# clementinboittiaux/sucre

Measured on AMD Instinct MI355X. Metric: restored Mpixels/sec/GPU at 1080p, 64 neighbour views; % HBM roofline, higher is better.
Workload: dtype f32

## Files before the change

### include/sucre_hip.h

```cpp
#ifndef SUCRE_HIP_H
#define SUCRE_HIP_H

#include <stddef.h>
#include <stdint.h>

#ifdef __cplusplus
extern "C" {
#endif

#define SUCRE_ABI_VERSION 2

#define SUCRE_OK 0
#define SUCRE_ERR_ARG (-1)
#define SUCRE_ERR_RANGE (-2)
#define SUCRE_ERR_LAUNCH (-3)

#define SUCRE_FIT_CLOSED_FORM 1u
#define SUCRE_FIT_OBS_U16MM 2u
#define SUCRE_FIT_KEEP_J 8u

#define SUCRE_OBS_F32 0
#define SUCRE_OBS_U16MM 1
#define SUCRE_OBS_F32_PLAIN 2
#define SUCRE_OBS_F32_Z26 3

#define SUCRE_EXT_POINTS 1
#define SUCRE_EXT_COLOUR 2
#define SUCRE_EXT_POINTS_COLOUR 3
#define SUCRE_FIT_EXT_COLOUR 4u
#define SUCRE_FIT_EXT_BOTH 16u

typedef struct sucre_view {
    const float *depth;
    const uint8_t *rgb;
    int32_t H, W;
    float K[9];
    float Kinv[9];
    float R[9];
    float t[3];
    float Rinv[9];
    float tinv[3];
} sucre_view_t;

enum {
    SUCRE_WS_VIEW_COUNT = 0,
    SUCRE_WS_VIEW_KEEP = 1,
    SUCRE_WS_N_OBS = 2,
    SUCRE_WS_PARAMS = 3,
    SUCRE_WS_SUMS = 4,
    SUCRE_WS_N_OBS_TOTAL = 5,
    SUCRE_WS_STORE_FORMAT = 6
};

int sucre_version(void);
const char *sucre_last_error(void);

size_t sucre_workspace_bytes(int H, int W, int n_views);
int64_t sucre_ws_offset(int H, int W, int n_views, int region);

int sucre_match_views(void *ws, int H, int W, int n_views, const sucre_view_t *target,
                      const sucre_view_t *views_dev, int k0, int k1, void *stream);

int sucre_match_map(int H, int W, int n_views, const sucre_view_t *target, const sucre_view_t *views_dev, int k,
                    int32_t *map_dev, void *stream);

int sucre_pack_view(const float *depth_dev, const uint8_t *rgb_dev, int H, int W, void *packed_dev, void *stream);
int sucre_pack_views(const float *const *depth_dev, const uint8_t *const *rgb_dev, void *const *packed_dev, int n, int H, int W,
                     void *stream);

int sucre_project_points(const sucre_view_t *view, const float *wP_dev, int64_t n, int32_t *pix_dev, void *stream);

int sucre_import_view(void *ws, int H, int W, int n_views, int k, const int16_t *u1_dev, const int16_t *v1_dev,
                      const float *z_dev, const uint8_t *rgb_dev, int64_t n, void *stream);

int sucre_finalize_matches(void *ws, int H, int W, int n_views, double min_cover, void *stream);
int sucre_finalize_matches_fmt(void *ws, int H, int W, int n_views, double min_cover, int obs_format, void *stream);

int sucre_fit_init(void *ws, int H, int W, int n_views, const uint8_t *rgb1_dev, const float *depth1_dev,
                   const float *params0, const float *J0_dev, void *stream);

int sucre_fit_run(void *ws, int H, int W, int n_views, int t0, int T, double lr, double beta1, double beta2,
                  double eps, unsigned flags, double *trace_dev, void *stream);

int sucre_fit_grad(void *ws, int H, int W, int n_views, int step, double lr, double beta1, double beta2,
                   double eps, unsigned flags, void *stream);
int sucre_fit_step(void *ws, int H, int W, int n_views, int step, double lr, double beta1, double beta2,
                   double eps, double *trace_row_dev, void *stream);
int sucre_set_n_obs_total(void *ws, int H, int W, int n_views, uint64_t n_obs_total, void *stream);

typedef struct sucre_group_image {
    void *ws;
    int32_t H, W, n_views;
    int32_t reserved;
} sucre_group_image_t;
size_t sucre_group_bytes(int n_images);
int64_t sucre_group_sums_offset(void);
int sucre_group_init(void *group_dev, int n_images, const sucre_group_image_t *images, const float *params0, void *stream);
int sucre_group_iter(void *group_dev, int n_images, int step, double lr, double beta1, double beta2, double eps, unsigned flags,
                     uint64_t n_obs_total, double *trace_dev, void *stream);
int sucre_group_finish(void *group_dev, int n_images, int step, double lr, double beta1, double beta2, double eps,
                       uint64_t n_obs_total, double *trace_dev, void *stream);

size_t sucre_batch_bytes(int n_images);
int sucre_fit_run_batch(void *batch_dev, int n_images, void *const *ws, double *const *trace_dev, int H, int W, const int *n_views,
                        int t0, int T, double lr, double beta1, double beta2, double eps, unsigned flags, void *stream);

int sucre_update_J(void *ws, int H, int W, int n_views, void *stream);
int sucre_update_J_fmt(void *ws, int H, int W, int n_views, int obs_format, void *stream);

int sucre_export_J(const void *ws, int H, int W, int n_views, float *J_dev, void *stream);

size_t sucre_select_scratch_bytes(void);
int sucre_select_ranks(const float *J_dev, int H, int W, int n_ranks, const uint64_t *ranks, float *out_dev, void *scratch_dev,
                       void *stream);

int sucre_count_valid(const float *J_dev, int H, int W, uint64_t *count_dev, void *stream);

int sucre_plot_stretch(const float *J_dev, int H, int W, const float *lo, const float *hi, uint8_t *out_dev, void *stream);

typedef struct sucre_pool_image {
    const float *J;
    int64_t n_px;
} sucre_pool_image_t;
size_t sucre_pool_select_bytes(void);
size_t sucre_pool_table_bytes(int n_images);
int sucre_pool_select_begin(void *state_dev, void *stream);
int sucre_pool_select_pass(void *state_dev, int pass, void *table_dev, int n_images, const sucre_pool_image_t *images, int n_ranks,
                           void *stream);
int sucre_pool_select_locate(void *state_dev, int pass, int n_ranks, const uint64_t *ranks, float *out_dev, void *stream);

int sucre_check_store(const void *ws, int H, int W, int n_views, uint32_t *verdict_dev, uint64_t *scratch_dev,
                      void *stream);

int sucre_export_view(const void *ws, int H, int W, int n_views, int k, float *z_dev, uint8_t *rgb_dev,
                      void *stream);

size_t sucre_light_workspace_bytes(int H, int W, int n_views);
int64_t sucre_light_params_offset(int H, int W, int n_views);
int sucre_match_views_light(void *ws, void *lws, int H, int W, int n_views, const sucre_view_t *target,
                            const sucre_view_t *views_dev, int k0, int k1, void *stream);
int sucre_match_views_fcolour(void *ws, void *lws, int H, int W, int n_views, const sucre_view_t *target,
                              const sucre_view_t *views_dev, int k0, int k1, void *stream);
size_t sucre_light_workspace_bytes_ext(int H, int W, int n_views, int ext_mode);
int sucre_match_views_light_fcolour(void *ws, void *lws, int H, int W, int n_views, const sucre_view_t *target,
                                    const sucre_view_t *views_dev, int k0, int k1, void *stream);
int sucre_finalize_matches_ext(void *ws, void *lws, int H, int W, int n_views, double min_cover, int ext_mode, void *stream);
int sucre_import_view_ext(void *ws, void *lws, int H, int W, int n_views, int k, const int16_t *u1_dev, const int16_t *v1_dev,
                          const float *z_dev, const uint8_t *rgb_dev, const float *ext_dev, int64_t n, int ext_mode, void *stream);
int sucre_export_view_ext(const void *ws, const void *lws, int H, int W, int n_views, int k, float *planes_dev, void *stream);
int sucre_export_view_ext2(const void *ws, const void *lws, int H, int W, int n_views, int k, float *planes_dev, void *stream);
int sucre_finalize_matches_light(void *ws, void *lws, int H, int W, int n_views, double min_cover, void *stream);
int sucre_fit_init_light(void *ws, void *lws, int H, int W, int n_views, const uint8_t *rgb1_dev, const float *depth1_dev,
                         const float *params0, const float *J0_dev, void *stream);
int sucre_update_J_light(void *ws, void *lws, int H, int W, int n_views, void *stream);
int sucre_update_J_ext(void *ws, void *lws, int H, int W, int n_views, unsigned flags, void *stream);
int sucre_fit_run_light(void *ws, void *lws, int H, int W, int n_views, int t0, int T, double lr, double beta1,
                        double beta2, double eps, unsigned flags , double *trace_dev,
                        void *stream);

size_t sucre_residual_scratch_bytes(int H, int W, int n_views);
int sucre_fit_residuals(const void *ws, int H, int W, int n_views, int obs_format, int32_t *count_dev, float *ssr_dev,
                        double *view_stats_dev, void *scratch_dev, void *stream);
int sucre_fit_residuals_ext(const void *ws, const void *lws, int H, int W, int n_views, unsigned flags ,
                            int32_t *count_dev, float *ssr_dev, double *view_stats_dev, void *scratch_dev, void *stream);

size_t sucre_trim_scratch_bytes(int H, int W, int n_views);
int sucre_trim_outliers(void *ws, int H, int W, int n_views, int obs_format, double k_sigma, const double *view_stats_dev,
                        int32_t *dropped_dev, int64_t *view_dropped_dev, float *thresholds_dev, void *scratch_dev, void *stream);
int sucre_trim_outliers_ext(void *ws, const void *lws, int H, int W, int n_views, unsigned flags ,
                            double k_sigma, const double *view_stats_dev, int32_t *dropped_dev, int64_t *view_dropped_dev,
                            float *thresholds_dev, void *scratch_dev, void *stream);

size_t sucre_gain_scratch_bytes(int H, int W, int n_views);
int sucre_view_gains(const void *ws, int H, int W, int n_views, int obs_format, double limit, double *gains_dev, float *inv_dev,
                     double *sums_dev, void *scratch_dev, void *stream);
int sucre_view_gains_ext(const void *ws, const void *lws, int H, int W, int n_views, unsigned flags ,
                         double limit, double *gains_dev, float *inv_dev, double *sums_dev, void *scratch_dev, void *stream);
int sucre_apply_view_gains(void *ws, int H, int W, int n_views, const float *inv_dev, int64_t *view_clipped_dev, void *scratch_dev,
                           void *stream);
int sucre_apply_view_gains_ext(void *ws, void *lws, int H, int W, int n_views, unsigned flags ,
                               const float *inv_dev, int64_t *view_clipped_dev, void *scratch_dev, void *stream);

#define SUCRE_INVERT_LIGHT 1u
#define SUCRE_INVERT_FLOAT_COLOUR 2u
typedef struct sucre_invert_image {
    const float *depth;
    const void *rgb;
    float *J;
    int32_t H, W;
    float Kinv[9];
    int32_t reserved;
} sucre_invert_image_t;
size_t sucre_invert_bytes(int n_images);
int sucre_invert_images(void *table_dev, int n_images, const sucre_invert_image_t *images, const float *params, unsigned flags,
                        void *stream);

typedef struct sucre_light_group_image {
    void *ws;
    void *lws;
    int32_t H, W, n_views;
    int32_t reserved;
} sucre_light_group_image_t;
size_t sucre_light_group_bytes(int n_images);
int64_t sucre_light_group_sums_offset(void);
// ... 12 lines not shown
```

### sucre_amd/_lib.py

```python
from __future__ import annotations

import ctypes as C
import os
from pathlib import Path

ABI_VERSION = 2
LIB_PATH = Path(os.environ.get('SUCRE_HIP_LIB', Path(__file__).resolve().parent / 'libsucre_hip.so'))

FIT_CLOSED_FORM = 1
FIT_OBS_U16MM = 2
FIT_EXT_COLOUR = 4
FIT_EXT_BOTH = 16
FIT_KEEP_J = 8
OBS_F32, OBS_U16MM, OBS_F32_PLAIN, OBS_F32_Z26 = 0, 1, 2, 3
EXT_POINTS, EXT_COLOUR, EXT_POINTS_COLOUR = 1, 2, 3
OBS_FORMATS = {'f32': OBS_F32, 'u16mm': OBS_U16MM, 'f32plain': OBS_F32_PLAIN, 'f32z26': OBS_F32_Z26}
WS_VIEW_COUNT, WS_VIEW_KEEP, WS_N_OBS, WS_PARAMS, WS_SUMS, WS_N_OBS_TOTAL, WS_STORE_FORMAT = range(7)
INVERT_LIGHT, INVERT_FLOAT_COLOUR = 1, 2
INVERT_MAX_IMAGES = 4096
POOL_MAX_IMAGES = 4096
POOL_MAX_RANKS = 8
POOL_HIST_WORDS = 3 * 8 * 256
STORE_F32, STORE_U16MM, STORE_Z24, STORE_Z26 = 0, 1, 2, 3


class SucreView(C.Structure):
    _fields_ = [('depth', C.c_void_p), ('rgb', C.c_void_p), ('H', C.c_int32), ('W', C.c_int32),
                ('K', C.c_float * 9), ('Kinv', C.c_float * 9), ('R', C.c_float * 9), ('t', C.c_float * 3),
                ('Rinv', C.c_float * 9), ('tinv', C.c_float * 3)]


assert C.sizeof(SucreView) == 192


class GroupImage(C.Structure):
    _fields_ = [('ws', C.c_void_p), ('H', C.c_int32), ('W', C.c_int32), ('n_views', C.c_int32), ('reserved', C.c_int32)]

class LightGroupImage(C.Structure):
    _fields_ = [('ws', C.c_void_p), ('lws', C.c_void_p), ('H', C.c_int32), ('W', C.c_int32), ('n_views', C.c_int32),
                ('reserved', C.c_int32)]


class InvertImage(C.Structure):
    _fields_ = [('depth', C.c_void_p), ('rgb', C.c_void_p), ('J', C.c_void_p), ('H', C.c_int32), ('W', C.c_int32),
                ('Kinv', C.c_float * 9), ('reserved', C.c_int32)]


assert C.sizeof(InvertImage) == 72


class PoolImage(C.Structure):
    _fields_ = [('J', C.c_void_p), ('n_px', C.c_int64)]


assert C.sizeof(PoolImage) == 16


_i, _vp, _d, _u64 = C.c_int, C.c_void_p, C.c_double, C.c_uint64
SIGNATURES = {
    'sucre_version': (_i, []),
    'sucre_last_error': (C.c_char_p, []),
    'sucre_workspace_bytes': (C.c_size_t, [_i, _i, _i]),
    'sucre_ws_offset': (C.c_int64, [_i, _i, _i, _i]),
    'sucre_match_views': (_i, [_vp, _i, _i, _i, C.POINTER(SucreView), _vp, _i, _i, _vp]),
    'sucre_match_map': (_i, [_i, _i, _i, C.POINTER(SucreView), _vp, _i, _vp, _vp]),
    'sucre_pack_view': (_i, [_vp, _vp, _i, _i, _vp, _vp]),
    'sucre_pack_views': (_i, [C.POINTER(_vp), C.POINTER(_vp), C.POINTER(_vp), _i, _i, _i, _vp]),
    'sucre_project_points': (_i, [C.POINTER(SucreView), _vp, C.c_int64, _vp, _vp]),
    'sucre_import_view': (_i, [_vp, _i, _i, _i, _i, _vp, _vp, _vp, _vp, C.c_int64, _vp]),
    'sucre_finalize_matches': (_i, [_vp, _i, _i, _i, _d, _vp]),
    'sucre_finalize_matches_fmt': (_i, [_vp, _i, _i, _i, _d, _i, _vp]),
    'sucre_fit_init': (_i, [_vp, _i, _i, _i, _vp, _vp, C.POINTER(C.c_float), _vp, _vp]),
    'sucre_fit_run': (_i, [_vp, _i, _i, _i, _i, _i, _d, _d, _d, _d, C.c_uint, _vp, _vp]),
    'sucre_fit_grad': (_i, [_vp, _i, _i, _i, _i, _d, _d, _d, _d, C.c_uint, _vp]),
    'sucre_fit_step': (_i, [_vp, _i, _i, _i, _i, _d, _d, _d, _d, _vp, _vp]),
    'sucre_set_n_obs_total': (_i, [_vp, _i, _i, _i, _u64, _vp]),
    'sucre_group_bytes': (C.c_size_t, [_i]),
    'sucre_group_sums_offset': (C.c_int64, []),
    'sucre_group_init': (_i, [_vp, _i, C.POINTER(GroupImage), C.POINTER(C.c_float), _vp]),
    'sucre_group_iter': (_i, [_vp, _i, _i, _d, _d, _d, _d, C.c_uint, _u64, _vp, _vp]),
    'sucre_group_finish': (_i, [_vp, _i, _i, _d, _d, _d, _d, _u64, _vp, _vp]),
    'sucre_batch_bytes': (C.c_size_t, [_i]),
    'sucre_fit_run_batch': (_i, [_vp, _i, C.POINTER(_vp), C.POINTER(_vp), _i, _i, C.POINTER(_i), _i, _i, _d, _d, _d, _d, C.c_uint, _vp]),
    'sucre_update_J': (_i, [_vp, _i, _i, _i, _vp]),
    'sucre_update_J_fmt': (_i, [_vp, _i, _i, _i, _i, _vp]),
    'sucre_export_J': (_i, [_vp, _i, _i, _i, _vp, _vp]),
    'sucre_select_scratch_bytes': (C.c_size_t, []),
    'sucre_select_ranks': (_i, [_vp, _i, _i, _i, C.POINTER(C.c_uint64), _vp, _vp, _vp]),
    'sucre_count_valid': (_i, [_vp, _i, _i, _vp, _vp]),
    'sucre_plot_stretch': (_i, [_vp, _i, _i, C.POINTER(C.c_float), C.POINTER(C.c_float), _vp, _vp]),
    'sucre_pool_select_bytes': (C.c_size_t, []),
    'sucre_pool_table_bytes': (C.c_size_t, [_i]),
    'sucre_pool_select_begin': (_i, [_vp, _vp]),
    'sucre_pool_select_pass': (_i, [_vp, _i, _vp, _i, C.POINTER(PoolImage), _i, _vp]),
    'sucre_pool_select_locate': (_i, [_vp, _i, _i, C.POINTER(C.c_uint64), _vp, _vp]),
    'sucre_check_store': (_i, [_vp, _i, _i, _i, _vp, _vp, _vp]),
    'sucre_export_view': (_i, [_vp, _i, _i, _i, _i, _vp, _vp, _vp]),
    'sucre_light_workspace_bytes': (C.c_size_t, [_i, _i, _i]),
    'sucre_light_params_offset': (C.c_int64, [_i, _i, _i]),
    'sucre_match_views_light': (_i, [_vp, _vp, _i, _i, _i, C.POINTER(SucreView), _vp, _i, _i, _vp]),
    'sucre_match_views_fcolour': (_i, [_vp, _vp, _i, _i, _i, C.POINTER(SucreView), _vp, _i, _i, _vp]),
    'sucre_light_workspace_bytes_ext': (C.c_size_t, [_i, _i, _i, _i]),
    'sucre_match_views_light_fcolour': (_i, [_vp, _vp, _i, _i, _i, C.POINTER(SucreView), _vp, _i, _i, _vp]),
    'sucre_finalize_matches_ext': (_i, [_vp, _vp, _i, _i, _i, _d, _i, _vp]),
    'sucre_import_view_ext': (_i, [_vp, _vp, _i, _i, _i, _i, _vp, _vp, _vp, _vp, _vp, C.c_int64, _i, _vp]),
    'sucre_export_view_ext': (_i, [_vp, _vp, _i, _i, _i, _i, _vp, _vp]),
    'sucre_export_view_ext2': (_i, [_vp, _vp, _i, _i, _i, _i, _vp, _vp]),
    'sucre_finalize_matches_light': (_i, [_vp, _vp, _i, _i, _i, _d, _vp]),
    'sucre_fit_init_light': (_i, [_vp, _vp, _i, _i, _i, _vp, _vp, C.POINTER(C.c_float), _vp, _vp]),
    'sucre_update_J_light': (_i, [_vp, _vp, _i, _i, _i, _vp]),
    'sucre_update_J_ext': (_i, [_vp, _vp, _i, _i, _i, C.c_uint, _vp]),
    'sucre_fit_run_light': (_i, [_vp, _vp, _i, _i, _i, _i, _i, _d, _d, _d, _d, C.c_uint, _vp, _vp]),
    'sucre_residual_scratch_bytes': (C.c_size_t, [_i, _i, _i]),
    'sucre_fit_residuals': (_i, [_vp, _i, _i, _i, _i, _vp, _vp, _vp, _vp, _vp]),
    'sucre_fit_residuals_ext': (_i, [_vp, _vp, _i, _i, _i, C.c_uint, _vp, _vp, _vp, _vp, _vp]),
    'sucre_trim_scratch_bytes': (C.c_size_t, [_i, _i, _i]),
    'sucre_trim_outliers': (_i, [_vp, _i, _i, _i, _i, _d, _vp, _vp, _vp, _vp, _vp, _vp]),
    'sucre_trim_outliers_ext': (_i, [_vp, _vp, _i, _i, _i, C.c_uint, _d, _vp, _vp, _vp, _vp, _vp, _vp]),
    'sucre_gain_scratch_bytes': (C.c_size_t, [_i, _i, _i]),
    'sucre_view_gains': (_i, [_vp, _i, _i, _i, _i, _d, _vp, _vp, _vp, _vp, _vp]),
    'sucre_view_gains_ext': (_i, [_vp, _vp, _i, _i, _i, C.c_uint, _d, _vp, _vp, _vp, _vp, _vp]),
    'sucre_apply_view_gains': (_i, [_vp, _i, _i, _i, _vp, _vp, _vp, _vp]),
    'sucre_apply_view_gains_ext': (_i, [_vp, _vp, _i, _i, _i, C.c_uint, _vp, _vp, _vp, _vp]),
    'sucre_invert_bytes': (C.c_size_t, [_i]),
    'sucre_invert_images': (_i, [_vp, _i, C.POINTER(InvertImage), C.POINTER(C.c_float), C.c_uint, _vp]),
    'sucre_light_group_bytes': (C.c_size_t, [_i]),
    'sucre_light_group_sums_offset': (C.c_int64, []),
    'sucre_light_group_init': (_i, [_vp, _i, C.POINTER(LightGroupImage), C.POINTER(C.c_float), _vp]),
    'sucre_light_group_iter': (_i, [_vp, _i, _i, _d, _d, _d, _d, C.c_uint, _u64, _vp, _vp]),
    'sucre_light_group_finish': (_i, [_vp, _i, _i, _d, _d, _d, _d, C.c_uint, _u64, _vp, _vp]),
}

_lib = None


class SucreError(RuntimeError):
    pass


def load() -> C.CDLL:
    global _lib
    if _lib is not None:
        return _lib
    if not LIB_PATH.exists():
        raise SucreError(f'{LIB_PATH} is missing: build the gfx950 HIP library first '
                         f'(make -C {LIB_PATH.parent / "csrc"}); there is no fallback path')
    import torch
    lib = C.CDLL(str(LIB_PATH))
    for name, (res, args) in SIGNATURES.items():
        fn = getattr(lib, name)
        fn.restype, fn.argtypes = res, args
    if lib.sucre_version() != ABI_VERSION:
        raise SucreError(f'libsucre_hip.so has ABI {lib.sucre_version()}, expected {ABI_VERSION}: rebuild it')
    _lib = lib
    return lib


def check(rc: int) -> None:
    if rc != 0:
        raise SucreError(f'libsucre_hip error {rc}: {load().sucre_last_error().decode()}')
```

### sucre_amd/csrc/abi.hip

```cpp
#include <cmath>
#include <cstdarg>
#include <cstdio>
#include <map>
#include <mutex>
#include <vector>

#include "invert.h"
#include "launch.h"
#include "pool.h"

namespace sucre {

static thread_local char g_err[512] = "";

static int fail(int code, const char *fmt, ...) {
    va_list ap;
    va_start(ap, fmt);
    vsnprintf(g_err, sizeof(g_err), fmt, ap);
    va_end(ap);
    return code;
}

static int check_hip(hipError_t e, const char *what) {
    if (e == hipSuccess) return SUCRE_OK;
    return fail(SUCRE_ERR_LAUNCH, "%s: %s", what, hipGetErrorString(e));
}

static bool aligned(const void *p, size_t a) { return (reinterpret_cast<uintptr_t>(p) % a) == 0; }

static int check_ws(const void *ws, int H, int W, int n_views, Layout *L) {
    if (!make_layout(H, W, n_views, L))
        return fail(SUCRE_ERR_ARG, "invalid geometry H=%d W=%d n_views=%d (need 1..32767, 1..%d views)", H, W, n_views,
                    kMaxViews);
    if (!ws) return fail(SUCRE_ERR_ARG, "workspace is NULL");
    if (!aligned(ws, 256)) return fail(SUCRE_ERR_ARG, "workspace must be 256-byte aligned");
    return SUCRE_OK;
}

AdamCoef adam_coef(int step, double lr, double beta1, double beta2, double eps) {
    AdamCoef c;
    const double bc1 = 1.0 - std::pow(beta1, (double)step);
    const double bc2 = 1.0 - std::pow(beta2, (double)step);
    c.w1 = (float)(1.0 - beta1);
    c.beta2 = (float)beta2;
    c.w2 = (float)(1.0 - beta2);
    c.step_size_neg = (float)(-(lr / bc1));
    c.bc2_sqrt = (float)std::sqrt(bc2);
    c.eps = (float)eps;
    return c;
}

static int check_adam(int step, double lr, double beta1, double beta2, double eps) {
    if (step < 1) return fail(SUCRE_ERR_RANGE, "Adam step must be >= 1 (got %d)", step);
    if (!(lr >= 0.0) || !(beta1 >= 0.0 && beta1 < 1.0) || !(beta2 >= 0.0 && beta2 < 1.0) || !(eps >= 0.0))
        return fail(SUCRE_ERR_ARG, "invalid Adam hyper-parameters lr=%g betas=(%g,%g) eps=%g", lr, beta1, beta2, eps);
    return SUCRE_OK;
}

}

using namespace sucre;

extern "C" {

int sucre_version(void) { return SUCRE_ABI_VERSION; }

const char *sucre_last_error(void) { return g_err; }

size_t sucre_workspace_bytes(int H, int W, int n_views) {
    Layout L;
    if (!make_layout(H, W, n_views, &L)) {
        fail(SUCRE_ERR_ARG, "invalid geometry H=%d W=%d n_views=%d", H, W, n_views);
        return 0;
    }
    return L.total;
}

int64_t sucre_ws_offset(int H, int W, int n_views, int region) {
    Layout L;
    if (!make_layout(H, W, n_views, &L)) return fail(SUCRE_ERR_ARG, "invalid geometry H=%d W=%d n_views=%d", H, W, n_views);
    switch (region) {
        case SUCRE_WS_VIEW_COUNT: return (int64_t)L.off_view_count;
        case SUCRE_WS_VIEW_KEEP: return (int64_t)L.off_view_keep;
        case SUCRE_WS_N_OBS: return (int64_t)L.off_n_obs;
        case SUCRE_WS_PARAMS: return (int64_t)L.off_params;
        case SUCRE_WS_SUMS: return (int64_t)L.off_sums;
        case SUCRE_WS_N_OBS_TOTAL: return (int64_t)L.off_n_obs_total;
        case SUCRE_WS_STORE_FORMAT: return (int64_t)off_store_format(L);
        default: return fail(SUCRE_ERR_RANGE, "unknown workspace region %d", region);
    }
}

int sucre_match_views(void *ws, int H, int W, int n_views, const sucre_view_t *target,
                      const sucre_view_t *views_dev, int k0, int k1, void *stream) {
    Layout L;
    if (int rc = check_ws(ws, H, W, n_views, &L)) return rc;
    if (!target || !views_dev) return fail(SUCRE_ERR_ARG, "target / views_dev is NULL");
    if (!target->depth) return fail(SUCRE_ERR_ARG, "target depth map is NULL");
    if (target->H != H || target->W != W)
        return fail(SUCRE_ERR_ARG, "target is %dx%d but the workspace is laid out for %dx%d", target->W, target->H, W, H);
    if (!aligned(views_dev, 8)) return fail(SUCRE_ERR_ARG, "views_dev must be 8-byte aligned");
    if (k0 < 0 || k1 > n_views || k0 >= k1) return fail(SUCRE_ERR_RANGE, "view range [%d,%d) outside [0,%d)", k0, k1, n_views);
    return check_hip(launch_match(L, static_cast<uint8_t *>(ws), *target, views_dev, k0, k1,
                                  static_cast<hipStream_t>(stream)), "sucre_match_views");
}

int sucre_match_map(int H, int W, int n_views, const sucre_view_t *target, const sucre_view_t *views_dev, int k,
                    int32_t *map_dev, void *stream) {
    Layout L;
    if (!make_layout(H, W, n_views, &L)) return fail(SUCRE_ERR_ARG, "invalid geometry H=%d W=%d n_views=%d", H, W, n_views);
    if (!target || !views_dev || !map_dev) return fail(SUCRE_ERR_ARG, "target / views_dev / map_dev is NULL");
    if (!target->depth) return fail(SUCRE_ERR_ARG, "target depth map is NULL");
    if (target->H != H || target->W != W) return fail(SUCRE_ERR_ARG, "target is %dx%d, expected %dx%d", target->W, target->H, W, H);
    if (k < 0 || k >= n_views) return fail(SUCRE_ERR_RANGE, "view %d outside [0,%d)", k, n_views);
    return check_hip(launch_match_map(L, *target, views_dev, k, map_dev, static_cast<hipStream_t>(stream)), "sucre_match_map");
}

int sucre_pack_view(const float *depth_dev, const uint8_t *rgb_dev, int H, int W, void *packed_dev, void *stream) {
    if (H <= 0 || W <= 0 || H > 32767 || W > 32767) return fail(SUCRE_ERR_ARG, "invalid image size %dx%d", W, H);
    if (!depth_dev || !rgb_dev || !packed_dev) return fail(SUCRE_ERR_ARG, "depth_dev / rgb_dev / packed_dev is NULL");
    if (!aligned(packed_dev, 8)) return fail(SUCRE_ERR_ARG, "packed_dev must be 8-byte aligned");
    return check_hip(launch_pack_view(depth_dev, rgb_dev, H, W, packed_dev, static_cast<hipStream_t>(stream)), "sucre_pack_view");
}

int sucre_pack_views(const float *const *depth_dev, const uint8_t *const *rgb_dev, void *const *packed_dev, int n, int H, int W,
                     void *stream) {
    if (H <= 0 || W <= 0 || H > 32767 || W > 32767) return fail(SUCRE_ERR_ARG, "invalid image size %dx%d", W, H);
    if (n < 0) return fail(SUCRE_ERR_RANGE, "negative view count %d", n);
    if (n == 0) return SUCRE_OK;
    if (!depth_dev || !rgb_dev || !packed_dev) return fail(SUCRE_ERR_ARG, "depth_dev / rgb_dev / packed_dev is NULL");
    for (int k = 0; k < n; ++k) {
        if (!depth_dev[k] || !rgb_dev[k] || !packed_dev[k]) return fail(SUCRE_ERR_ARG, "view %d: depth / rgb / packed pointer is NULL", k);
        if (!aligned(packed_dev[k], 8)) return fail(SUCRE_ERR_ARG, "view %d: packed_dev must be 8-byte aligned", k);
    }
    return check_hip(launch_pack_views(depth_dev, rgb_dev, packed_dev, n, H, W, static_cast<hipStream_t>(stream)), "sucre_pack_views");
}

int sucre_project_points(const sucre_view_t *view, const float *wP_dev, int64_t n, int32_t *pix_dev, void *stream) {
    if (!view) return fail(SUCRE_ERR_ARG, "view is NULL");
    if (view->H <= 0 || view->W <= 0 || view->H > 32767 || view->W > 32767)
        return fail(SUCRE_ERR_ARG, "invalid sensor size %dx%d", view->W, view->H);
    if (n < 0) return fail(SUCRE_ERR_RANGE, "negative point count %lld", (long long)n);
    if (n == 0) return SUCRE_OK;
    if (!wP_dev || !pix_dev) return fail(SUCRE_ERR_ARG, "wP_dev / pix_dev is NULL");
    return check_hip(launch_project_points(*view, wP_dev, (long long)n, pix_dev, static_cast<hipStream_t>(stream)),
                     "sucre_project_points");
}

int sucre_import_view(void *ws, int H, int W, int n_views, int k, const int16_t *u1_dev, const int16_t *v1_dev,
                      const float *z_dev, const uint8_t *rgb_dev, int64_t n, void *stream) {
    Layout L;
    if (int rc = check_ws(ws, H, W, n_views, &L)) return rc;
    if (k < 0 || k >= n_views) return fail(SUCRE_ERR_RANGE, "view %d outside [0,%d)", k, n_views);
    if (n < 0) return fail(SUCRE_ERR_RANGE, "negative observation count %lld", (long long)n);
    if (n > 0 && (!u1_dev || !v1_dev || !z_dev || !rgb_dev)) return fail(SUCRE_ERR_ARG, "NULL match list");
    return check_hip(launch_import_view(L, static_cast<uint8_t *>(ws), k, u1_dev, v1_dev, z_dev, rgb_dev, (long long)n,
                                        static_cast<hipStream_t>(stream)), "sucre_import_view");
}

int sucre_finalize_matches(void *ws, int H, int W, int n_views, double min_cover, void *stream) {
    Layout L;
    if (int rc = check_ws(ws, H, W, n_views, &L)) return rc;
    if (std::isnan(min_cover)) return fail(SUCRE_ERR_ARG, "min_cover is NaN");
    return check_hip(launch_finalize(L, static_cast<uint8_t *>(ws), min_cover, static_cast<hipStream_t>(stream)),
                     "sucre_finalize_matches");
}

int sucre_finalize_matches_fmt(void *ws, int H, int W, int n_views, double min_cover, int obs_format, void *stream) {
    Layout L;
    if (int rc = check_ws(ws, H, W, n_views, &L)) return rc;
    if (std::isnan(min_cover)) return fail(SUCRE_ERR_ARG, "min_cover is NaN");
    if (obs_format != SUCRE_OBS_F32 && obs_format != SUCRE_OBS_U16MM && obs_format != SUCRE_OBS_F32_PLAIN && obs_format != SUCRE_OBS_F32_Z26)
        return fail(SUCRE_ERR_ARG, "unknown observation format %d", obs_format);
    return check_hip(launch_finalize(L, static_cast<uint8_t *>(ws), min_cover, static_cast<hipStream_t>(stream),
                                     nullptr, nullptr, obs_format), "sucre_finalize_matches_fmt");
}

int sucre_fit_init(void *ws, int H, int W, int n_views, const uint8_t *rgb1_dev, const float *depth1_dev,
                   const float *params0, const float *J0_dev, void *stream) {
    Layout L;
    if (int rc = check_ws(ws, H, W, n_views, &L)) return rc;
    if (!depth1_dev || !params0) return fail(SUCRE_ERR_ARG, "depth1_dev / params0 is NULL");
    if (!rgb1_dev && !J0_dev) return fail(SUCRE_ERR_ARG, "need rgb1_dev or J0_dev");
    return check_hip(launch_fit_init(L, static_cast<uint8_t *>(ws), rgb1_dev, depth1_dev, params0, J0_dev,
                                     static_cast<hipStream_t>(stream)), "sucre_fit_init");
}

int sucre_fit_grad(void *ws, int H, int W, int n_views, int step, double lr, double beta1, double beta2,
                   double eps, unsigned flags, void *stream) {
    Layout L;
    if (int rc = check_ws(ws, H, W, n_views, &L)) return rc;
    if (int rc = check_adam(step, lr, beta1, beta2, eps)) return rc;
    if (flags & ~(SUCRE_FIT_CLOSED_FORM | SUCRE_FIT_OBS_U16MM)) return fail(SUCRE_ERR_ARG, "unknown fit flags 0x%x", flags);
    if ((flags & SUCRE_FIT_CLOSED_FORM) && step == 1)
        if (int rc = check_hip(launch_update_J(L, static_cast<uint8_t *>(ws), (flags & SUCRE_FIT_OBS_U16MM) ? SUCRE_OBS_U16MM : SUCRE_OBS_F32,
                                               static_cast<hipStream_t>(stream)), "sucre_fit_grad/update_J")) return rc;
    return check_hip(launch_fit_grad(L, static_cast<uint8_t *>(ws), adam_coef(step, lr, beta1, beta2, eps), flags,
                                     static_cast<hipStream_t>(stream)), "sucre_fit_grad");
}

int sucre_fit_step(void *ws, int H, int W, int n_views, int step, double lr, double beta1, double beta2,
                   double eps, double *trace_row_dev, void *stream) {
    Layout L;
    if (int rc = check_ws(ws, H, W, n_views, &L)) return rc;
    if (int rc = check_adam(step, lr, beta1, beta2, eps)) return rc;
    if (trace_row_dev && !aligned(trace_row_dev, 8)) return fail(SUCRE_ERR_ARG, "trace must be 8-byte aligned");
    return check_hip(launch_fit_step(L, static_cast<uint8_t *>(ws), adam_coef(step, lr, beta1, beta2, eps),
                                     trace_row_dev, static_cast<hipStream_t>(stream)), "sucre_fit_step");
}

int sucre_fit_run(void *ws, int H, int W, int n_views, int t0, int T, double lr, double beta1, double beta2,
                  double eps, unsigned flags, double *trace_dev, void *stream) {
    Layout L;
    if (int rc = check_ws(ws, H, W, n_views, &L)) return rc;
    if (t0 < 0 || T < 0) return fail(SUCRE_ERR_RANGE, "t0=%d T=%d must be >= 0", t0, T);
    if (int rc = check_adam(t0 + 1, lr, beta1, beta2, eps)) return rc;
    if (flags & ~(SUCRE_FIT_CLOSED_FORM | SUCRE_FIT_OBS_U16MM | SUCRE_FIT_KEEP_J)) return fail(SUCRE_ERR_ARG, "unknown fit flags 0x%x", flags);
    if (trace_dev && !aligned(trace_dev, 8)) return fail(SUCRE_ERR_ARG, "trace must be 8-byte aligned");
    auto *w = static_cast<uint8_t *>(ws);
    auto s = static_cast<hipStream_t>(stream);
    const int fmt = (flags & SUCRE_FIT_OBS_U16MM) ? SUCRE_OBS_U16MM : SUCRE_OBS_F32;
    if ((flags & SUCRE_FIT_CLOSED_FORM) && t0 == 0 && T > 0)
        if (int rc = check_hip(launch_update_J(L, w, fmt, s), "sucre_fit_run/initial update_J")) return rc;
    for (int it = 0; it < T; ++it) {
        const AdamCoef co = adam_coef(t0 + it + 1, lr, beta1, beta2, eps);
        if (int rc = check_hip(launch_fit_iter_fused(L, w, co, flags, trace_dev ? trace_dev + (size_t)it * 10 : nullptr, s),
                               "sucre_fit_run")) return rc;
    }
    if ((flags & SUCRE_FIT_CLOSED_FORM) && !(flags & SUCRE_FIT_KEEP_J))
        return check_hip(launch_update_J(L, w, fmt, s), "sucre_fit_run/update_J");
    return SUCRE_OK;
}

int sucre_set_n_obs_total(void *ws, int H, int W, int n_views, uint64_t n_obs_total, void *stream) {
    Layout L;
    if (int rc = check_ws(ws, H, W, n_views, &L)) return rc;
    if (n_obs_total == 0) return fail(SUCRE_ERR_RANGE, "n_obs_total must be > 0");
    return check_hip(launch_set_n_obs_total(L, static_cast<uint8_t *>(ws), n_obs_total,
                                            static_cast<hipStream_t>(stream)), "sucre_set_n_obs_total");
}

int sucre_update_J(void *ws, int H, int W, int n_views, void *stream) {
    return sucre_update_J_fmt(ws, H, W, n_views, SUCRE_OBS_F32, stream);
}

int sucre_update_J_fmt(void *ws, int H, int W, int n_views, int obs_format, void *stream) {
    Layout L;
    if (int rc = check_ws(ws, H, W, n_views, &L)) return rc;
    if (obs_format != SUCRE_OBS_F32 && obs_format != SUCRE_OBS_U16MM && obs_format != SUCRE_OBS_F32_PLAIN && obs_format != SUCRE_OBS_F32_Z26)
        return fail(SUCRE_ERR_ARG, "unknown observation format %d", obs_format);
    return check_hip(launch_update_J(L, static_cast<uint8_t *>(ws), obs_format == SUCRE_OBS_U16MM ? SUCRE_OBS_U16MM : SUCRE_OBS_F32,
                                     static_cast<hipStream_t>(stream)),
                     "sucre_update_J");
}

int sucre_export_J(const void *ws, int H, int W, int n_views, float *J_dev, void *stream) {
    Layout L;
    if (int rc = check_ws(ws, H, W, n_views, &L)) return rc;
    if (!J_dev) return fail(SUCRE_ERR_ARG, "J_dev is NULL");
    return check_hip(launch_export_J(L, static_cast<const uint8_t *>(ws), J_dev, static_cast<hipStream_t>(stream)),
                     "sucre_export_J");
}

int sucre_export_view(const void *ws, int H, int W, int n_views, int k, float *z_dev, uint8_t *rgb_dev,
                      void *stream) {
    Layout L;
    if (int rc = check_ws(ws, H, W, n_views, &L)) return rc;
    if (k < 0 || k >= n_views) return fail(SUCRE_ERR_RANGE, "view %d outside [0,%d)", k, n_views);
    if (!z_dev && !rgb_dev) return fail(SUCRE_ERR_ARG, "both outputs are NULL");
    return check_hip(launch_export_view(L, static_cast<const uint8_t *>(ws), k, z_dev, rgb_dev,
                                        static_cast<hipStream_t>(stream)), "sucre_export_view");
}

int sucre_check_store(const void *ws, int H, int W, int n_views, uint32_t *verdict_dev, uint64_t *scratch_dev,
                      void *stream) {
    Layout L;
    if (int rc = check_ws(ws, H, W, n_views, &L)) return rc;
    if (!verdict_dev || !scratch_dev) return fail(SUCRE_ERR_ARG, "verdict_dev / scratch_dev is NULL");
    if (!aligned(verdict_dev, 4) || !aligned(scratch_dev, 8)) return fail(SUCRE_ERR_ARG, "outputs must be 4 / 8-byte aligned");
    return check_hip(launch_check_store(L, static_cast<const uint8_t *>(ws), verdict_dev, scratch_dev,
                                        static_cast<hipStream_t>(stream)), "sucre_check_store");
}


size_t sucre_group_bytes(int n_images) { return n_images > 0 ? group_bytes(n_images) : 0; }

int64_t sucre_group_sums_offset(void) { return group_sums_offset(); }

int sucre_group_init(void *group_dev, int n_images, const sucre_group_image_t *images, const float *params0, void *stream) {
    if (!group_dev || !aligned(group_dev, 256)) return fail(SUCRE_ERR_ARG, "group buffer is NULL or not 256-byte aligned");
    if (n_images < 1 || !images || !params0) return fail(SUCRE_ERR_ARG, "need at least one image and params0");
    auto s = static_cast<hipStream_t>(stream);
    if (int rc = check_hip(launch_group_init(group_dev, params0, s), "sucre_group_init")) return rc;
    for (int i = 0; i < n_images; ++i) {
        Layout L;
        if (int rc = check_ws(images[i].ws, images[i].H, images[i].W, images[i].n_views, &L)) return rc;
        if (int rc = check_hip(launch_group_set_image(group_dev, i, L, static_cast<uint8_t *>(images[i].ws), s), "sucre_group_init")) return rc;
    }
    return SUCRE_OK;
}

int sucre_group_iter(void *group_dev, int n_images, int step, double lr, double beta1, double beta2, double eps, unsigned flags,
                     uint64_t n_obs_total, double *trace_dev, void *stream) {
    if (!group_dev || n_images < 1) return fail(SUCRE_ERR_ARG, "group buffer is NULL / no image");
    if (int rc = check_adam(step, lr, beta1, beta2, eps)) return rc;
    if (flags & ~(SUCRE_FIT_CLOSED_FORM | SUCRE_FIT_OBS_U16MM)) return fail(SUCRE_ERR_ARG, "unknown fit flags 0x%x", flags);
    if (n_obs_total == 0) return fail(SUCRE_ERR_RANGE, "n_obs_total must be > 0");
    if (trace_dev && !aligned(trace_dev, 8)) return fail(SUCRE_ERR_ARG, "trace must be 8-byte aligned");
    const AdamCoef co_prev = adam_coef(step > 1 ? step - 1 : 1, lr, beta1, beta2, eps);
    double *row = (trace_dev && step > 1) ? trace_dev + (size_t)(step - 2) * 10 : nullptr;
    return check_hip(launch_group_iter(group_dev, n_images, step, co_prev, adam_coef(step, lr, beta1, beta2, eps), flags, n_obs_total,
                                       row, static_cast<hipStream_t>(stream)), "sucre_group_iter");
}

int sucre_group_finish(void *group_dev, int n_images, int step, double lr, double beta1, double beta2, double eps,
                       uint64_t n_obs_total, double *trace_dev, void *stream) {
    if (!group_dev || n_images < 1) return fail(SUCRE_ERR_ARG, "group buffer is NULL / no image");
    if (step < 0) return fail(SUCRE_ERR_RANGE, "step=%d must be >= 0", step);
    if (step >= 1) if (int rc = check_adam(step, lr, beta1, beta2, eps)) return rc;
    if (n_obs_total == 0) return fail(SUCRE_ERR_RANGE, "n_obs_total must be > 0");
    double *row = (trace_dev && step >= 1) ? trace_dev + (size_t)(step - 1) * 10 : nullptr;
    return check_hip(launch_group_finish(group_dev, n_images, step, adam_coef(step >= 1 ? step : 1, lr, beta1, beta2, eps), n_obs_total,
                                         row, static_cast<hipStream_t>(stream)), "sucre_group_finish");
}


size_t sucre_batch_bytes(int n_images) { return n_images > 0 ? batch_bytes(n_images) : 0; }

int sucre_fit_run_batch(void *batch_dev, int n_images, void *const *ws, double *const *trace_dev, int H, int W, const int *n_views,
                        int t0, int T, double lr, double beta1, double beta2, double eps, unsigned flags, void *stream) {
    if (!batch_dev || !aligned(batch_dev, 256)) return fail(SUCRE_ERR_ARG, "batch buffer is NULL or not 256-byte aligned");
    if (n_images < 1 || !ws || !n_views) return fail(SUCRE_ERR_ARG, "need at least one image (ws and n_views arrays)");
    if (n_images > 4096) return fail(SUCRE_ERR_RANGE, "n_images=%d: at most 4096 images per batch", n_images);
    std::vector<Layout> layouts((size_t)n_images);
    for (int i = 0; i < n_images; ++i) {
        if (int rc = check_ws(ws[i], H, W, n_views[i], &layouts[(size_t)i])) return rc;
        for (int j = 0; j < i; ++j)
            if (ws[j] == ws[i]) return fail(SUCRE_ERR_ARG, "images %d and %d share a workspace", j, i);
        if (trace_dev && trace_dev[i] && !aligned(trace_dev[i], 8)) return fail(SUCRE_ERR_ARG, "trace of image %d must be 8-byte aligned", i);
    }
    if (t0 < 0 || T < 0) return fail(SUCRE_ERR_RANGE, "t0=%d T=%d must be >= 0", t0, T);
    if (int rc = check_adam(t0 + 1, lr, beta1, beta2, eps)) return rc;
    if (flags & ~(SUCRE_FIT_CLOSED_FORM | SUCRE_FIT_OBS_U16MM | SUCRE_FIT_KEEP_J)) return fail(SUCRE_ERR_ARG, "unknown fit flags 0x%x", flags);
    auto s = static_cast<hipStream_t>(stream);
    const int fmt = (flags & SUCRE_FIT_OBS_U16MM) ? SUCRE_OBS_U16MM : SUCRE_OBS_F32;
    if (int rc = check_hip(launch_batch_set(batch_dev, n_images, reinterpret_cast<uint8_t *const *>(ws), trace_dev, layouts.data(), flags, s),
                           "sucre_fit_run_batch/table")) return rc;
    if ((flags & SUCRE_FIT_CLOSED_FORM) && t0 == 0 && T > 0)
        for (int i = 0; i < n_images; ++i)
            if (int rc = check_hip(launch_update_J(layouts[(size_t)i], static_cast<uint8_t *>(ws[i]), fmt, s), "sucre_fit_run_batch/initial update_J")) return rc;
    for (int it = 0; it < T; ++it)
        if (int rc = check_hip(launch_batch_iter(layouts[0], batch_dev, n_images, adam_coef(t0 + it + 1, lr, beta1, beta2, eps), flags, it, s),
                               "sucre_fit_run_batch")) return rc;
    if ((flags & SUCRE_FIT_CLOSED_FORM) && !(flags & SUCRE_FIT_KEEP_J))
        for (int i = 0; i < n_images; ++i)
            if (int rc = check_hip(launch_update_J(layouts[(size_t)i], static_cast<uint8_t *>(ws[i]), fmt, s), "sucre_fit_run_batch/update_J")) return rc;
    return SUCRE_OK;
}

size_t sucre_select_scratch_bytes(void) { return select_scratch_bytes(); }

int sucre_select_ranks(const float *J_dev, int H, int W, int n_ranks, const uint64_t *ranks, float *out_dev, void *scratch_dev,
                       void *stream) {
    if (H <= 0 || W <= 0) return fail(SUCRE_ERR_ARG, "invalid image size %dx%d", W, H);
    if (!J_dev || !ranks || !out_dev || !scratch_dev) return fail(SUCRE_ERR_ARG, "J_dev / ranks / out_dev / scratch_dev is NULL");
    if (n_ranks < 1 || n_ranks > 8) return fail(SUCRE_ERR_RANGE, "n_ranks=%d outside [1,8]", n_ranks);
    if (!aligned(scratch_dev, 8) || !aligned(J_dev, 4) || !aligned(out_dev, 4)) return fail(SUCRE_ERR_ARG, "misaligned pointer");
    return check_hip(launch_select_ranks(J_dev, H, W, n_ranks, ranks, out_dev, scratch_dev, static_cast<hipStream_t>(stream)),
                     "sucre_select_ranks");
}

int sucre_count_valid(const float *J_dev, int H, int W, uint64_t *count_dev, void *stream) {
    if (H <= 0 || W <= 0) return fail(SUCRE_ERR_ARG, "invalid image size %dx%d", W, H);
    if (!J_dev || !count_dev) return fail(SUCRE_ERR_ARG, "J_dev / count_dev is NULL");
    if (!aligned(J_dev, 4) || !aligned(count_dev, 8)) return fail(SUCRE_ERR_ARG, "misaligned pointer");
    return check_hip(launch_count_valid(J_dev, H, W, count_dev, static_cast<hipStream_t>(stream)), "sucre_count_valid");
}
// ... 550 lines not shown
```

### sucre_amd/csrc/experiment.h

```cpp
#pragma once

#ifdef SUCRE_EXP_NOCOMPUTE
constexpr bool kExpNoCompute = true;
#else
constexpr bool kExpNoCompute = false;
#endif
#ifdef SUCRE_EXP_NOLOAD
constexpr bool kExpNoLoad = true;
#else
constexpr bool kExpNoLoad = false;
#endif
#ifdef SUCRE_EXP_NOSTORE
constexpr bool kExpNoStore = true;
#else
constexpr bool kExpNoStore = false;
#endif
#ifndef SUCRE_STORE_NT
#define SUCRE_STORE_NT 2
#endif
constexpr int kStoreNt = SUCRE_STORE_NT;

#ifndef SUCRE_FIT_WAVES
#define SUCRE_FIT_WAVES 5
#endif
#ifndef SUCRE_CLOSED_WAVES
#define SUCRE_CLOSED_WAVES 4
#endif

#ifndef SUCRE_MIN_STRIPS
#define SUCRE_MIN_STRIPS 4
#endif

#ifndef SUCRE_RING
#define SUCRE_RING 3
#endif
#ifndef SUCRE_DMA_POLICY
#define SUCRE_DMA_POLICY " nt"
#endif

#ifndef SUCRE_EXACT_DIV
#define SUCRE_EXACT_DIV 0
#endif
constexpr bool kExactDiv = SUCRE_EXACT_DIV != 0;

#ifndef SUCRE_EXACT_J_ADAM
#define SUCRE_EXACT_J_ADAM 0
#endif
constexpr bool kExactJAdam = SUCRE_EXACT_J_ADAM != 0;

#if !defined(SUCRE_SCALED_B)
#define SUCRE_SCALED_B 1
#endif
constexpr bool kScaledBBuilt = SUCRE_SCALED_B != 0;

#ifdef SUCRE_EXP_WAVE_TIMES
constexpr bool kExpWaveTimes = true;
#define SUCRE_EXP_EXPORT extern "C" __attribute__((visibility("default")))
#else
constexpr bool kExpWaveTimes = false;
#define SUCRE_EXP_EXPORT [[maybe_unused]] static
#endif

#ifndef SUCRE_DEAL_FIT
#define SUCRE_DEAL_FIT 64, 50, 38, 28, 20
#endif
#ifndef SUCRE_DEAL_CLOSED
#define SUCRE_DEAL_CLOSED 64, 48, 32, 20
#endif
```

### sucre_amd/csrc/fit.hip

```cpp
#include <cstddef>
#include <type_traits>

#include "experiment.h"
#include "fit_math.h"
#include "handoff.h"

namespace sucre {

struct Water {
    float B[3], nb[3], ng[3];
};

template <class ParamAt>
__device__ __forceinline__ Water water_from(ParamAt param_at) {
    Water w;
#pragma unroll
    for (int c = 0; c < 3; ++c) {
        w.B[c] = param_at(c);
        w.nb[c] = -param_at(3 + c) * kLog2e;
        w.ng[c] = -param_at(6 + c) * kLog2e;
    }
    return w;
}
__device__ __forceinline__ Water load_water(const float *__restrict__ params) {
// ... 5 lines not shown
    Water w = load_water(params);
#pragma unroll
    for (int c = 0; c < 3; ++c) { w.B[c] = uniform_f(w.B[c]); w.nb[c] = uniform_f(w.nb[c]); w.ng[c] = uniform_f(w.ng[c]); }
    return w;
}

constexpr float kInv255 = (float)(1.0 / 255.0);

struct Acc {
    float pa[3];
    float pb[3];
    float sB[3];
    float sGZ[3];
    float cost;
};

__device__ __forceinline__ void pack_sums(float (&s)[kNumSums], const float (&sB)[3], const float (&sGZ)[3], const float (&sBeta)[3], float cost) {
#pragma unroll
    for (int c = 0; c < 3; ++c) { s[c] = sB[c]; s[3 + c] = sGZ[c]; s[6 + c] = sBeta[c]; }
    s[9] = cost;
}

struct Exps { float a[kGroupLv][3], g[kGroupLv][3]; };

__device__ __forceinline__ void chunk_exps(const float (&zz)[kGroupLv], const Water &w, Exps &e) {
#pragma unroll
    for (int j = 0; j < kGroupLv; ++j)
#pragma unroll
        for (int c = 0; c < 3; ++c) { e.a[j][c] = zz[j] * w.nb[c]; e.g[j][c] = zz[j] * w.ng[c]; }
    __builtin_amdgcn_sched_barrier(0);
#pragma unroll
    for (int j = 0; j < kGroupLv; ++j)
#pragma unroll
        for (int c = 0; c < 3; ++c) { e.a[j][c] = fast_exp2(e.a[j][c]); e.g[j][c] = fast_exp2(e.g[j][c]); }
    __builtin_amdgcn_sched_barrier(0);
}

template <bool kScaledB>
__device__ __forceinline__ void grad_terms(float z, float a, float g, uint32_t k, bool valid, float Bc, float Jc, int c, Acc &acc) {
    const float omg = kScaledB ? __builtin_fmaf(-Bc, g, Bc) : 1.0f - g;
    const float Ihat = __builtin_fmaf(Jc, a, kScaledB ? omg : Bc * omg);
    float r = __builtin_fmaf((float)k, kInv255, -Ihat);
    r = valid ? r : 0.0f;
    const float rz = r * z;
    acc.cost = __builtin_fmaf(r, r, acc.cost);
    acc.pa[c] = __builtin_fmaf(r, a, acc.pa[c]);
    acc.pb[c] = __builtin_fmaf(rz, a, acc.pb[c]);
    acc.sB[c] = __builtin_fmaf(r, omg, acc.sB[c]);
    acc.sGZ[c] = __builtin_fmaf(rz, g, acc.sGZ[c]);
}

template <bool kMasked, bool kScaledB>
__device__ __forceinline__ void accumulate_chunk(const float (&zz)[kGroupLv], const uint32_t (&cc)[3], const Water &w,
                                                 const float (&J)[3], Acc &acc) {
    if (kExpNoCompute) {
        acc.cost += (zz[0] + zz[1]) + (zz[2] + zz[3]) + (float)(cc[0] ^ cc[1] ^ cc[2]);
        return;
    }
    Exps e;
    chunk_exps(zz, w, e);
#pragma unroll
    for (int j = 0; j < kGroupLv; ++j) {
        const float z = zz[j];
        const bool valid = !kMasked || z > 0.0f;
#pragma unroll
        for (int c = 0; c < 3; ++c) grad_terms<kScaledB>(z, e.a[j][c], e.g[j][c], (cc[c] >> (8 * j)) & 255u, valid, w.B[c], J[c], c, acc);
    }
}

template <bool kScaledB>
__device__ __forceinline__ void accumulate_level(float z, const uint32_t (&k)[3], const Water &w, const float (&J)[3],
                                                 Acc &acc) {
    const bool valid = z > 0.0f;
#pragma unroll
    for (int c = 0; c < 3; ++c) grad_terms<kScaledB>(z, fast_exp2(z * w.nb[c]), fast_exp2(z * w.ng[c]), k[c], valid, w.B[c], J[c], c, acc);
}

__device__ __forceinline__ float finite_or_zero(float x) { return __builtin_isfinite(x) ? x : 0.0f; }

struct AccOne {
    float q[9][3];
};

template <bool kScaledB>
__device__ __forceinline__ void closed_terms(float z, float a, float g, uint32_t k, bool valid, float Bc, float Jp,
                                             float &q0, float &q1, float &q2, float &q3, float &q4, float &q5,
                                             float &q6, float &q7, float &q8) {
    const float omg = kScaledB ? __builtin_fmaf(-Bc, g, Bc) : 1.0f - g;
    const float y = __builtin_fmaf((float)k, kInv255, -(kScaledB ? omg : Bc * omg));
    float p = __builtin_fmaf(-Jp, a, y);
    p = valid ? p : 0.0f;
    const float za = z * a, zg = z * g;
    q0 = __builtin_fmaf(p, a, q0);
    q1 = __builtin_fmaf(a, valid ? a : 0.0f, q1);
    q2 = __builtin_fmaf(p, omg, q2);
    q3 = __builtin_fmaf(a, omg, q3);
    q4 = __builtin_fmaf(p, za, q4);
    q5 = __builtin_fmaf(a, za, q5);
    q6 = __builtin_fmaf(p, zg, q6);
    q7 = __builtin_fmaf(a, zg, q7);
    q8 = __builtin_fmaf(p, p, q8);
}

template <bool kMasked, bool kScaledB>
__device__ __forceinline__ void accumulate_chunk(const float (&zz)[kGroupLv], const uint32_t (&cc)[3], const Water &w,
                                                 const float (&Jp)[3], AccOne &acc) {
    if (kExpNoCompute) {
        acc.q[8][0] += (zz[0] + zz[1]) + (zz[2] + zz[3]) + (float)(cc[0] ^ cc[1] ^ cc[2]);
        return;
    }
    Exps e;
    chunk_exps(zz, w, e);
#pragma unroll
    for (int j = 0; j < kGroupLv; ++j) {
        const float z = zz[j];
        const bool valid = !kMasked || z > 0.0f;
#pragma unroll
        for (int c = 0; c < 3; ++c)
            closed_terms<kScaledB>(z, e.a[j][c], e.g[j][c], (cc[c] >> (8 * j)) & 255u, valid, w.B[c], Jp[c], acc.q[0][c], acc.q[1][c],
                                   acc.q[2][c], acc.q[3][c], acc.q[4][c], acc.q[5][c], acc.q[6][c], acc.q[7][c], acc.q[8][c]);
    }
}

template <bool kScaledB>
__device__ __forceinline__ void accumulate_level(float z, const uint32_t (&k)[3], const Water &w, const float (&Jp)[3],
                                                 AccOne &acc) {
    if (kExpNoCompute) {
        acc.q[8][0] += z + (float)(k[0] ^ k[1] ^ k[2]);
        return;
    }
    const bool valid = z > 0.0f;
#pragma unroll
    for (int c = 0; c < 3; ++c)
        closed_terms<kScaledB>(z, fast_exp2(z * w.nb[c]), fast_exp2(z * w.ng[c]), k[c], valid, w.B[c], Jp[c], acc.q[0][c], acc.q[1][c],
                               acc.q[2][c], acc.q[3][c], acc.q[4][c], acc.q[5][c], acc.q[6][c], acc.q[7][c], acc.q[8][c]);
}

constexpr int kRing = SUCRE_RING;
constexpr int kAhead = kRing - 1;
constexpr int kSlot = 2048;

struct __attribute__((aligned(16))) FitLds {
    uint8_t ring[4][kRing][kSlot];
    double stot[kSumsPad];
    float wsum[4][kNumSums];
    double wtotal[4][kNumSums];
    int is_last, is_last_total;
};

__device__ __forceinline__ uint32_t lds_addr(const void *p) {
    return static_cast<uint32_t>(reinterpret_cast<uintptr_t>(p));
}

constexpr uint32_t kShapeFull = 1u << 31;
constexpr uint32_t kShapeTrail = 1u << 30;
__host__ __device__ constexpr uint32_t full_chunk_b(int fmt) { return (uint32_t)(chunk_bytes(fmt) - 1024) / 16u; }
__host__ __device__ __forceinline__ uint32_t item_shape(uint32_t bytes, bool full_chunk) {
    const uint32_t pieces = bytes / 16u;
    const uint32_t nA = pieces < 64u ? pieces : 64u, nB = pieces - nA;
    return (nA - 1u) | ((nB ? nB - 1u : 0u) << 8) | ((nB ? nA : nA - 1u) << 16) | (full_chunk ? kShapeFull : 0u);
}
static_assert(level_bytes(0) % 16 == 0 && level_bytes(1) % 16 == 0 && level_bytes(2) % 16 == 0 && level_bytes(3) % 16 == 0 && kChunk % 16 == 0 && kChunk16 % 16 == 0 && kChunk24 % 16 == 0 && kChunk26 % 16 == 0, "items are copied in 16-byte pieces");
static_assert(kChunk <= 2048 && kChunk >= 1024 && kChunk16 >= 1024 && kChunk24 >= 1024 && kChunk26 >= 1024 && kChunk26 <= kChunk, "a full chunk is one whole DMA + a partial one");
static_assert(level_bytes(0) % 64 == 0 && level_bytes(1) % 64 == 0 && level_bytes(2) % 64 == 0 && (kGroupLv * level_bytes(3)) % 64 == 0, "items start on 64-byte units (PlanItem.src64; a kStoreZ26 strip starts on a whole chunk)");

__device__ __forceinline__ void dma_item(const uint8_t *src, uint32_t slotA, uint32_t slotB, uint32_t voffA, uint32_t voffB) {
    if (kExpNoLoad) return;
    unsigned keep;
    asm volatile(
        "s_nop 4\n\t"
        "s_mov_b32 %0, m0\n\t"
        "s_mov_b32 m0, %3\n\t"
        "s_nop 0\n\t"
        "global_load_lds_dwordx4 %1, %2" SUCRE_DMA_POLICY "\n\t"
        "s_mov_b32 m0, %4\n\t"
        "s_nop 0\n\t"
        "global_load_lds_dwordx4 %5, %2" SUCRE_DMA_POLICY "\n\t"
        "s_mov_b32 m0, %0"
        : "=&s"(keep)
        : "v"(voffA), "s"(src), "s"(slotA), "s"(slotB), "v"(voffB)
        : "memory");
}

__device__ __forceinline__ void wait_vm(uint32_t n) {
#define SUCRE_W(N) case N: asm volatile("s_waitcnt vmcnt(" #N ")" ::: "memory"); break;
    switch (n) {
        SUCRE_W(0) SUCRE_W(1) SUCRE_W(2) SUCRE_W(3) SUCRE_W(4) SUCRE_W(5) SUCRE_W(6) SUCRE_W(7) SUCRE_W(8) SUCRE_W(9)
        SUCRE_W(10) SUCRE_W(11) SUCRE_W(12) SUCRE_W(13) SUCRE_W(14) SUCRE_W(15) SUCRE_W(16) SUCRE_W(17) SUCRE_W(18)
        SUCRE_W(19) SUCRE_W(20) SUCRE_W(21)
        default: asm volatile("s_waitcnt vmcnt(0)" ::: "memory"); break;
    }
#undef SUCRE_W
}
static_assert(2 * kAhead + 9 <= 63, "s_waitcnt vmcnt takes six bits");

__device__ __forceinline__ uint32_t strip_items(uint32_t levels, int mode) { return 1u + ((levels + 3u) >> 2) + (mode == 0 ? 1u : 0u); }

__global__ __launch_bounds__(256) void plan_kernel(const StripMeta *__restrict__ meta, int n_strips, const uint32_t *__restrict__ store_fmt, uint32_t W0, uint32_t W1,
                                                   uint32_t Kmax, uint32_t stride0, uint32_t stride1, uint32_t kmax0, uint32_t kmax1,
                                                   PlanItem *__restrict__ plan0, PlanItem *__restrict__ plan1,
                                                   StripEntry *__restrict__ strips0, StripEntry *__restrict__ strips1,
                                                   uint32_t *__restrict__ count0, uint32_t *__restrict__ count1, uint64_t comp_off,
                                                   uint64_t state_off) {
    const int mode = blockIdx.y;
    const int fmt = (int)store_fmt[0];
    const uint32_t W = mode ? W1 : W0, stride = mode ? stride1 : stride0, kmax = mode ? kmax1 : kmax0;
    PlanItem *plan = mode ? plan1 : plan0;
    StripEntry *strips = mode ? strips1 : strips0;
    uint32_t *count = mode ? count1 : count0;
    const uint32_t idx = blockIdx.x * 256u + threadIdx.x;
    const uint32_t wid = idx / Kmax, k = idx - wid * Kmax;
    if (wid >= W) return;
    const DealShares sh = deal_shares(mode, W / 4u);
    uint32_t start = 0u, strip = 0u, strip0 = 0u;
    const uint32_t K = deal_walk(wid, W, (uint32_t)n_strips, sh, [&](uint32_t s) { return meta[s].levels; }, [&](uint32_t kk, uint32_t s) {
        if (kk == 0u) strip0 = s;
        if (kk < k) start += strip_items(meta[s].levels, mode);
        if (kk == k) strip = s;
    });
    if (k == 0u) count[wid] = K;
    if (k >= K) return;
    const StripMeta m = meta[strip];
    const uint32_t nfull = m.levels >> 2, r = m.levels & 3u;
    const uint32_t nu = min(nfull, m.full >> 2);
    const uint32_t lb = (uint32_t)level_bytes(fmt);
    const uint64_t st = state_off + (uint64_t)strip * (kStateFloats * 4);
    PlanItem *out = plan + (size_t)wid * stride + start;
    strips[(size_t)wid * kmax + k] = StripEntry{strip, strip_counts(nu, nfull - nu, r)};
    *out++ = PlanItem{(uint32_t)(st >> 6), item_shape(3u * kStripPx * 4u, false)};
    for (uint32_t g = 0; g < nfull; ++g)
        *out++ = PlanItem{(uint32_t)((comp_off + (m.lvoff + (uint64_t)g * kGroupLv) * lb) >> 6), item_shape((uint32_t)chunk_bytes(fmt), true)};
    if (r) *out++ = PlanItem{(uint32_t)((comp_off + (m.lvoff + (uint64_t)nfull * kGroupLv) * lb) >> 6), item_shape(r * lb, false)};
    if (mode == 0) *out++ = PlanItem{(uint32_t)((st + 3 * kStripPx * 4) >> 6), item_shape(6u * kStripPx * 4u, false)};
    if (k + 1u == K) {
        const uint64_t st0 = state_off + (uint64_t)strip0 * (kStateFloats * 4);
        for (int j = 0; j < kAhead + 1; ++j) *out++ = PlanItem{(uint32_t)(st0 >> 6), item_shape(3u * kStripPx * 4u, false) | kShapeTrail};
    }
}

typedef uint32_t ItemRegs __attribute__((ext_vector_type(2)));
typedef const __attribute__((address_space(4))) ItemRegs *ConstItems;

template <class T>
__device__ __forceinline__ T *uniform_ptr(T *p) {
    const uint64_t u = reinterpret_cast<uint64_t>(p);
    const uint32_t lo = __builtin_amdgcn_readfirstlane((uint32_t)u), hi = __builtin_amdgcn_readfirstlane((uint32_t)(u >> 32));
    return reinterpret_cast<T *>(((uint64_t)hi << 32) | lo);
}

template <class T>
__device__ __forceinline__ ConstItems const_items(const T *p) {
    static_assert(sizeof(T) == 8, "two dwords per entry");
    return (ConstItems)(reinterpret_cast<uintptr_t>(uniform_ptr(p)));
}

struct RangeCodes { bool z24, z26; uint32_t zoff, fullB; };

template <int kFmt>
__device__ __forceinline__ RangeCodes range_codes_of(uint32_t f0, uint32_t f1) {
    RangeCodes rc;
    rc.z24 = kFmt == 0 && f0 == (uint32_t)kStoreZ24;
    rc.z26 = kFmt == 0 && f0 == (uint32_t)kStoreZ26;
    rc.zoff = f1;
    rc.fullB = rc.z24 ? full_chunk_b(kStoreZ24) : rc.z26 ? full_chunk_b(kStoreZ26) : full_chunk_b(kFmt);
    return rc;
}

template <int kFmt>
__device__ __forceinline__ RangeCodes range_codes(const uint32_t *__restrict__ store_fmt) {
    return range_codes_of<kFmt>(__builtin_amdgcn_readfirstlane(store_fmt[0]), __builtin_amdgcn_readfirstlane(store_fmt[1]));
}

__host__ __device__ constexpr bool format_readable(int kFmt, uint32_t f) {
    return kFmt == kStoreU16 ? f == (uint32_t)kStoreU16 : (f == (uint32_t)kStoreF32 || f == (uint32_t)kStoreZ24 || f == (uint32_t)kStoreZ26);
}
template <int kFmt>
__device__ __forceinline__ bool store_matches(const uint32_t *__restrict__ store_fmt) {
    return format_readable(kFmt, __builtin_amdgcn_readfirstlane(store_fmt[0]));
}

template <int kFmt>
__device__ __forceinline__ void read_chunk(const uint8_t *sp, int lane, float (&zz)[kGroupLv], uint32_t (&cc)[3], const RangeCodes &rc, bool masked) {
    auto read_codes = [&](auto z26) {
        constexpr bool kZ26 = decltype(z26)::value;
        const uint2 a = *reinterpret_cast<const uint2 *>(sp + lane * 24), b = *reinterpret_cast<const uint2 *>(sp + lane * 24 + 8),
                    c = *reinterpret_cast<const uint2 *>(sp + lane * 24 + 16);
        const uint32_t h = kZ26 ? sp[kChunk24 + lane] : 0u;
        const uint32_t w[4] = {a.x, a.y, b.x, b.y};
#pragma unroll
        for (int j = 0; j < kGroupLv; ++j) {
            uint32_t bits;
            asm("v_mad_u32_u24 %0, %1, 1, %2" : "=v"(bits) : "v"(w[j]), "s"(rc.zoff));
            if (kZ26) bits += ((h >> (2 * j)) & 3u) << 24;
            zz[j] = __uint_as_float(bits);
            if (masked) zz[j] = (kZ26 ? bits != rc.zoff : (w[j] & 0xffffffu) != 0u) ? zz[j] : 0.0f;
        }
        cc[0] = __builtin_amdgcn_perm(a.y, a.x, 0x0c0c0703u) | __builtin_amdgcn_perm(b.y, b.x, 0x07030c0cu);
        cc[1] = c.x; cc[2] = c.y;
    };
    if (kFmt == 0 && rc.z26) return read_codes(std::true_type{});
    if (kFmt == 0 && rc.z24) return read_codes(std::false_type{});
    if (kFmt == 0) {
        const float4 z4 = *reinterpret_cast<const float4 *>(sp + lane * 16);
        zz[0] = z4.x; zz[1] = z4.y; zz[2] = z4.z; zz[3] = z4.w;
    } else {
        const uint2 q = *reinterpret_cast<const uint2 *>(sp + lane * 8);
        zz[0] = (float)(q.x & 0xffffu) * kMPerMm; zz[1] = (float)(q.x >> 16) * kMPerMm;
        zz[2] = (float)(q.y & 0xffffu) * kMPerMm; zz[3] = (float)(q.y >> 16) * kMPerMm;
    }
    const uint32_t *cp = reinterpret_cast<const uint32_t *>(sp + (kFmt ? 2 : 4) * kStripPx * kGroupLv) + 3 * lane;
    cc[0] = cp[0]; cc[1] = cp[1]; cc[2] = cp[2];
}

template <int kFmt>
__device__ __forceinline__ void read_level(const uint8_t *sp, int lane, uint32_t r, uint32_t j, float &z, uint32_t (&k)[3], const RangeCodes &rc) {
    const bool z24 = kFmt == 0 && (rc.z24 || rc.z26);
    if (z24) {
        const uint8_t *zp = sp + (lane * r + j) * 3u;
        uint32_t code = (uint32_t)zp[0] | ((uint32_t)zp[1] << 8) | ((uint32_t)zp[2] << 16);
        if (rc.z26) {
            const uint32_t f = (uint32_t)lane * r + j;
            code |= ((reinterpret_cast<const uint32_t *>(sp + 6u * kStripPx * r)[f >> 4] >> (2u * (f & 15u))) & 3u) << 24;
        }
        z = code ? __uint_as_float(code + rc.zoff) : 0.0f;
    } else if (kFmt == 0) z = reinterpret_cast<const float *>(sp)[lane * r + j];
    else z = (float)reinterpret_cast<const uint16_t *>(sp)[lane * r + j] * kMPerMm;
    const uint8_t *cb = sp + (z24 ? 3 : kFmt ? 2 : 4) * kStripPx * r;
#pragma unroll
    for (int c = 0; c < 3; ++c) k[c] = cb[c * kStripPx * r + lane * r + j];
}

template <int kFmt>
__device__ __forceinline__ void issue_item(const ItemRegs it, uint32_t ring0, uint32_t slot_off, const uint8_t *__restrict__ ws, int lane, uint32_t fullB) {
    const uint32_t lane16 = (uint32_t)lane * 16u;
    const uint32_t voffB_full = (64u + min((uint32_t)lane, fullB - 1u)) * 16u;
    const uint8_t *src = ws + ((uint64_t)it.x << 6);
    const uint32_t slot = ring0 + slot_off;
    if (it.y & kShapeFull) {
        dma_item(src, slot, slot + 1024u, lane16, voffB_full);
    } else {
        const uint32_t a_last = it.y & 127u, b_last = (it.y >> 8) & 127u, b_base = (it.y >> 16) & 127u;
        dma_item(src, slot, slot + ((a_last + 1u) << 4), min((uint32_t)lane, a_last) << 4, (b_base + min((uint32_t)lane, b_last)) << 4);
    }
}

struct NoChain { static constexpr bool kOn = false; };
struct StreamChain {
    static constexpr bool kOn = true;
    ItemRegs head[kAhead + 1], se0;
    bool next_on;
    ItemRegs next_head[kAhead];
    const uint8_t *next_ws;
    uint32_t next_fullB;
    uint32_t cs, behind;
};

template <int kFmt, int kStores, bool kMoments, bool kPrimed = false, class Chain = NoChain, class OnJ, class OnChunk, class OnTail, class OnEnd>
__device__ __forceinline__ void stream_strips(FitLds &lds, const PlanItem *__restrict__ plan, const StripEntry *__restrict__ strip_list,
                                              uint32_t K, const uint8_t *__restrict__ ws, int wave, int lane, uint32_t fullB, OnJ on_J,
                                              OnChunk on_chunk, OnTail on_tail, OnEnd on_end, Chain *chain = nullptr) {
    if (K == 0) return;
    constexpr bool kChain = Chain::kOn;
    static_assert(!kChain || kPrimed, "a chained stream's first items are in flight when it starts");
    const uint32_t ring0 = lds_addr(&lds.ring[wave][0][0]);
    const uint8_t *ringp = &lds.ring[wave][0][0];
    const ConstItems items = const_items(plan);
    const ConstItems strips = const_items(strip_list);
    uint32_t trail = 0u;
    auto issue = [&](const ItemRegs it, uint32_t slot_off) {
        if constexpr (kChain) {
            if (chain->next_on && (it.y & kShapeTrail)) {
                ItemRegs f = chain->next_head[0];
#pragma unroll
                for (int q = 1; q < kAhead; ++q) f = trail == (uint32_t)q ? chain->next_head[q] : f;
                ++trail;
                issue_item<kFmt>(f, ring0, slot_off, chain->next_ws, lane, chain->next_fullB);
                return;
            }
        }
        issue_item<kFmt>(it, ring0, slot_off, ws, lane, fullB);
    };
    if (!kPrimed) {
#pragma unroll
        for (int q = 0; q < kAhead; ++q) issue(items[q], (uint32_t)(q * kSlot));
    }
    ItemRegs nxt;
    if constexpr (kChain) nxt = chain->head[kAhead]; else nxt = items[kAhead];
    uint32_t i = 0;
    uint32_t cs = 0u;
    uint32_t behind = 0u;
    if constexpr (kChain) { cs = chain->cs; behind = chain->behind; }
    auto step = [&]() -> const uint8_t * {
        asm volatile("s_waitcnt lgkmcnt(0)" ::: "memory");
        const uint32_t is = cs == 0u ? (uint32_t)((kRing - 1) * kSlot) : cs - (uint32_t)kSlot;
        issue(nxt, is);
        nxt = items[i + (uint32_t)kAhead + 1u];
        if (behind) {
            asm volatile("s_waitcnt vmcnt(%0)" ::"n"(2 * kAhead + kStores) : "memory");
            --behind;
        } else {
            asm volatile("s_waitcnt vmcnt(%0)" ::"n"(2 * kAhead) : "memory");
        }
        const uint8_t *sp = ringp + cs;
        cs = cs == (uint32_t)((kRing - 1) * kSlot) ? 0u : cs + (uint32_t)kSlot;
        ++i;
        return sp;
    };
    ItemRegs se;
    if constexpr (kChain) se = chain->se0; else se = strips[0];
    for (uint32_t k = 0; k < K; ++k) {
        const uint32_t strip = se.x, counts = se.y;
        if (k + 1u < K) se = strips[k + 1u];
        const uint32_t nu = counts_unmasked(counts), nm = counts_masked(counts), r = counts_tail(counts);
        on_J(step());
        for (uint32_t g = 0; g < nu; ++g) on_chunk(step(), false);
        for (uint32_t g = 0; g < nm; ++g) on_chunk(step(), true);
        if (r) on_tail(step(), r);
        if (kMoments) on_end(strip, step());
        else on_end(strip, (const uint8_t *)nullptr);
        behind = (uint32_t)kAhead;
    }
    if constexpr (kChain) {
        if (chain->next_on) {
            chain->cs = cs;
            chain->behind = (uint32_t)kAhead;
            return;
        }
        chain->cs = 0u;
        chain->behind = 0u;
    }
    asm volatile("s_waitcnt vmcnt(0)" ::: "memory");
}

__device__ __forceinline__ double wave_sum_fixed(double x) {
    return wave_sum_lane0(x);
}

__device__ __forceinline__ void reduce_group(const float *partials, int n_blocks, int g, double *gpart, int n_groups) {
    const int lane = threadIdx.x & 63, wave = threadIdx.x >> 6;
    const int b = g * kGroup + lane;
    for (int q = wave; q < kNumSums; q += 4) {
        double x = 0.0;
        if (lane < kGroup && b < n_blocks)
            x = (double)__hip_atomic_load(partials + (size_t)q * n_blocks + b, __ATOMIC_RELAXED, __HIP_MEMORY_SCOPE_AGENT);
        x = wave_sum_fixed(x);
        if (lane == 0) __hip_atomic_store(gpart + (size_t)q * n_groups + g, x, __ATOMIC_RELAXED, __HIP_MEMORY_SCOPE_AGENT);
    }
}

__device__ __forceinline__ double unscale_sum(double x, int q, bool scaled, float Bq) {
    return (kScaledBBuilt && scaled && q < 3) ? x / (double)Bq : x;
}

__device__ __forceinline__ void reduce_total(const double *gpart, int n_groups, double *stot, double *__restrict__ sums, const float *Bpass) {
    const int lane = threadIdx.x & 63, wave = threadIdx.x >> 6;
    const bool scaled = scaled_b_ok(Bpass[0], Bpass[1], Bpass[2]);
    for (int q = wave; q < kNumSums; q += 4) {
        double x = 0.0;
        for (int g = lane; g < n_groups; g += 64)
            x += __hip_atomic_load(gpart + (size_t)q * n_groups + g, __ATOMIC_RELAXED, __HIP_MEMORY_SCOPE_AGENT);
        x = unscale_sum(wave_sum_fixed(x), q, scaled, Bpass[q < 3 ? q : 0]);
        if (lane == 0) {
            __hip_atomic_store(sums + q, x, __ATOMIC_RELAXED, __HIP_MEMORY_SCOPE_AGENT);
            stot[q] = x;
        }
    }
    __syncthreads();
}

__device__ __forceinline__ void water_step(const double *__restrict__ sums, float *__restrict__ pstate,
                                           const uint64_t *__restrict__ n_obs_total, const AdamCoef &co,
                                           double *__restrict__ trace_row) {
    const int q = threadIdx.x & 63;
    const float scale = (1.0f / 3.0f) / (float)(*n_obs_total);
    float p = 0.f, m = 0.f, v = 0.f;
    double g = 0.0;
    if (q < 9) {
        g = water_grad(q, scale, [&](int i) { return sums[i]; }, [&](int c) { return pstate[c]; });
        p = pstate[q];
        m = pstate[9 + q];
        v = pstate[18 + q];
    }
    __builtin_amdgcn_wave_barrier();
    if (q < 9) {
        adam_update(p, m, v, (float)g, co);
        pstate[q] = p;
        pstate[9 + q] = m;
        pstate[18 + q] = v;
    }
    if (trace_row) {
        if (q < 9) trace_row[1 + q] = (double)p;
        if (q == 9) trace_row[0] = sums[9];
    }
}

__device__ __forceinline__ void wave_sums(float (&s)[kNumSums]) {
    static_assert(kNumSums == 10, "five pairs");
    float h[5];
#pragma unroll
    for (int q = 0; q < 5; ++q) {
        const auto r = __builtin_amdgcn_permlane32_swap(__float_as_uint(s[q]), __float_as_uint(s[q + 5]), false, false);
        h[q] = __uint_as_float(r[0]) + __uint_as_float(r[1]);
    }
    float R[3];
#pragma unroll
    for (int p = 0; p < 3; ++p) {
        const float a = h[2 * p], b = h[p < 2 ? 2 * p + 1 : 4];
        const auto r = __builtin_amdgcn_permlane16_swap(__float_as_uint(a), __float_as_uint(b), false, false);
        R[p] = __uint_as_float(r[0]) + __uint_as_float(r[1]);
        R[p] += lane_down<8>(R[p]);
        R[p] += lane_down<4>(R[p]);
        R[p] += lane_down<2>(R[p]);
        R[p] += lane_down<1>(R[p]);
    }
    auto at = [](float v, int lane) { return __uint_as_float(__builtin_amdgcn_readlane(__float_as_uint(v), lane)); };
    s[0] = at(R[0], 0); s[1] = at(R[0], 16); s[5] = at(R[0], 32); s[6] = at(R[0], 48);
    s[2] = at(R[1], 0); s[3] = at(R[1], 16); s[7] = at(R[1], 32); s[8] = at(R[1], 48);
    s[4] = at(R[2], 0); s[9] = at(R[2], 32);
}

template <bool kFused, bool kStep>
__device__ __forceinline__ void finish_from_wave_sums(FitLds &lds, float *partials, const AdamCoef &co, unsigned *ticket,
                                                      double *gpart, int n_groups, double *sums, float *pstate,
                                                      const uint64_t *__restrict__ n_obs_total, double *trace_row, const float *Bpass) {
    const int n_blocks = gridDim.x;
    const int t = threadIdx.x;
    __syncthreads();
    if (t < kNumSums)
        __hip_atomic_store(partials + (size_t)t * n_blocks + blockIdx.x,
                           ((lds.wsum[0][t] + lds.wsum[1][t]) + lds.wsum[2][t]) + lds.wsum[3][t], __ATOMIC_RELAXED,
                           __HIP_MEMORY_SCOPE_AGENT);

    if (kFused) {
        const int g = blockIdx.x / kGroup;
        const unsigned gsize = (unsigned)(min((g + 1) * kGroup, n_blocks) - g * kGroup);
        if (arrive_last(ticket + (size_t)(1 + g) * kTicketStride, gsize, &lds.is_last)) {
            reduce_group(partials, n_blocks, g, gpart, n_groups);
            if (arrive_last(ticket, (unsigned)n_groups, &lds.is_last_total)) {
                reduce_total(gpart, n_groups, lds.stot, sums, Bpass);
                if (kStep && t < 64) water_step(lds.stot, pstate, n_obs_total, co, trace_row);
            }
        }
    }
}

template <bool kFused, bool kStep = kFused>
__device__ __forceinline__ void finish_launch(FitLds &lds, float (&s)[kNumSums], float *partials, const AdamCoef &co,
                                              unsigned *ticket, double *gpart, int n_groups, double *sums,
                                              float *pstate, const uint64_t *__restrict__ n_obs_total,
                                              double *trace_row) {
    const int t = threadIdx.x;
    const int lane = t & 63;
    const int wave = __builtin_amdgcn_readfirstlane(t >> 6);
    wave_sums(s);
    if (lane == 0) {
#pragma unroll
        for (int q = 0; q < kNumSums; ++q) lds.wsum[wave][q] = s[q];
    }
    finish_from_wave_sums<kFused, kStep>(lds, partials, co, ticket, gpart, n_groups, sums, pstate, n_obs_total, trace_row, pstate);
}

template <class Chain>
__device__ __forceinline__ void store_stepped(float *p, float v) {
    if (kStoreNt == 1 || (kStoreNt == 2 && Chain::kOn)) __builtin_nontemporal_store(v, p);
    else *p = v;
}

template <int kFmt, bool kScaledB, bool kPrimed = false, class Chain = NoChain>
__device__ __forceinline__ void grad_pass(FitLds &lds, const PlanItem *__restrict__ plan, const StripEntry *__restrict__ strips, uint32_t n_strips_wave,
                                          const uint8_t *__restrict__ ws, float *__restrict__ state, int wave, int lane,
                                          const Water &w, float gscale, const AdamCoef &co, Acc &acc, float (&sBeta)[3], const RangeCodes &rc,
                                          Chain *chain = nullptr) {
    float J[3] = {0.f, 0.f, 0.f};
    stream_strips<kFmt, 9, true, kPrimed, Chain>(
        lds, plan, strips, n_strips_wave, ws, wave, lane, rc.fullB,
        [&](const uint8_t *sp) {
            const float *f = reinterpret_cast<const float *>(sp);
#pragma unroll
            for (int c = 0; c < 3; ++c) { J[c] = f[c * kStripPx + lane]; acc.pa[c] = 0.f; acc.pb[c] = 0.f; }
        },
        [&](const uint8_t *sp, bool masked) {
            float zz[kGroupLv];
            uint32_t cc[3];
            read_chunk<kFmt>(sp, lane, zz, cc, rc, masked);
            if (masked) accumulate_chunk<true, kScaledB>(zz, cc, w, J, acc);
            else accumulate_chunk<false, kScaledB>(zz, cc, w, J, acc);
        },
        [&](const uint8_t *sp, uint32_t r) {
            for (uint32_t j = 0; j < r; ++j) {
                float z;
                uint32_t k[3];
                read_level<kFmt>(sp, lane, r, j, z, k, rc);
                accumulate_level<kScaledB>(z, k, w, J, acc);
            }
        },
        [&](uint32_t strip, const uint8_t *sp) {
            const float *f = reinterpret_cast<const float *>(sp);
            float *st = state + (size_t)strip * kStateFloats;
#pragma unroll
            for (int c = 0; c < 3; ++c) {
                float Jc = J[c], m = f[c * kStripPx + lane], v = f[(3 + c) * kStripPx + lane];
                sBeta[c] += (acc.pb[c] == 0.0f) ? 0.0f : Jc * acc.pb[c];
                adam_update_J(Jc, m, v, gscale * acc.pa[c], co);
                if (kExpNoStore) {
                    asm volatile("" ::"v"(Jc), "v"(m), "v"(v));
                    continue;
                }
                store_stepped<Chain>(&st[c * kStripPx + lane], Jc);
                store_stepped<Chain>(&st[(3 + c) * kStripPx + lane], m);
                store_stepped<Chain>(&st[(6 + c) * kStripPx + lane], v);
            }
        },
        chain);
}

__device__ __forceinline__ bool pass_scaled_b(const Water &w) {
    return kScaledBBuilt && __builtin_amdgcn_readfirstlane((int)scaled_b_ok(w.B[0], w.B[1], w.B[2])) != 0;
}

template <int kFmt, bool kPrimed = false, class Chain = NoChain>
__device__ __forceinline__ void run_grad_pass(bool scaled, FitLds &lds, const PlanItem *__restrict__ plan, const StripEntry *__restrict__ strips,
                                              uint32_t n_strips_wave, const uint8_t *__restrict__ ws, float *__restrict__ state, int wave, int lane,
                                              const Water &w, float gscale, const AdamCoef &co, Acc &acc, float (&sBeta)[3], const RangeCodes &rc,
                                              Chain *chain = nullptr) {
    if (kScaledBBuilt && scaled) grad_pass<kFmt, true, kPrimed, Chain>(lds, plan, strips, n_strips_wave, ws, state, wave, lane, w, gscale, co, acc, sBeta, rc, chain);
    else grad_pass<kFmt, false, kPrimed, Chain>(lds, plan, strips, n_strips_wave, ws, state, wave, lane, w, gscale, co, acc, sBeta, rc, chain);
}

__device__ __forceinline__ void zero_acc(Acc &acc) {
#pragma unroll
    for (int c = 0; c < 3; ++c) { acc.pa[c] = 0.f; acc.pb[c] = 0.f; acc.sB[c] = 0.f; acc.sGZ[c] = 0.f; }
    acc.cost = 0.f;
}

constexpr uint32_t kExpWaveSlots = 8192;
__device__ unsigned long long g_exp_wave_times[5][kExpWaveTimes ? kExpWaveSlots : 1];
}
SUCRE_EXP_EXPORT int sucre_exp_wave_times(unsigned long long *out) {
    return (int)hipMemcpyFromSymbol(out, HIP_SYMBOL(sucre::g_exp_wave_times), sizeof(sucre::g_exp_wave_times));
}
namespace sucre {

template <bool kFused, int kFmt>
__global__ __launch_bounds__(256, kFitWaves) void fit_grad_kernel(const uint8_t *__restrict__ ws,
                                                       const PlanItem *__restrict__ plan, const StripEntry *__restrict__ plan_strips, const uint32_t *__restrict__ plan_count,
                                                       uint32_t plan_stride, uint32_t plan_kmax,
                                                       float *pstate, const uint64_t *__restrict__ n_obs_total,
                                                       float *__restrict__ state, float *partials, const AdamCoef co,
                                                       unsigned *ticket, double *gpart, int n_groups, double *sums,
                                                       double *trace_row, const uint32_t *__restrict__ obs_format) {
    __shared__ FitLds lds;
    const unsigned long long exp_t_in = kExpWaveTimes ? wall_clock64() : 0ull, exp_c_in = kExpWaveTimes ? clock64() : 0ull;
    const int t = threadIdx.x;
    const int lane = t & 63;
    const int wave = __builtin_amdgcn_readfirstlane(t >> 6);
    const Water w = load_water(pstate);
    const float gscale = -2.0f * ((1.0f / 3.0f) / (float)(*n_obs_total));
    const RangeCodes rc = range_codes<kFmt>(obs_format);
    const bool fmt_ok = store_matches<kFmt>(obs_format);
    const uint32_t wid = blockIdx.x * 4u + (uint32_t)wave;
    const uint32_t n_mine = fmt_ok ? plan_count[wid] : 0u;

    Acc acc;
    zero_acc(acc);
    if (!fmt_ok) acc.cost = __builtin_nanf("");
    float sBeta[3] = {0.f, 0.f, 0.f};
    if (kExpWaveTimes && lane == 0 && wid < kExpWaveSlots) g_exp_wave_times[0][wid] = wall_clock64();
    run_grad_pass<kFmt>(pass_scaled_b(w), lds, plan + (size_t)wid * plan_stride, plan_strips + (size_t)wid * plan_kmax, n_mine, ws, state, wave, lane, w, gscale, co, acc, sBeta, rc);
    if (kExpWaveTimes && lane == 0 && wid < kExpWaveSlots) g_exp_wave_times[1][wid] = wall_clock64();

    float s[kNumSums];
    pack_sums(s, acc.sB, acc.sGZ, sBeta, acc.cost);
    finish_launch<kFused>(lds, s, partials, co, ticket, gpart, n_groups, sums, pstate, n_obs_total, trace_row);
    if (kExpWaveTimes && lane == 0 && wid < kExpWaveSlots) { g_exp_wave_times[2][wid] = exp_t_in; g_exp_wave_times[3][wid] = wall_clock64(); g_exp_wave_times[4][wid] = clock64() - exp_c_in; }
}

struct ClosedSums { float sB[3], sGZ[3], sBeta[3], cost; };

template <int kFmt, bool kJOnly, bool kScaledB, bool kPrimed = false, class Chain = NoChain>
__device__ __forceinline__ void closed_pass(FitLds &lds, const PlanItem *__restrict__ plan, const StripEntry *__restrict__ strips, uint32_t n_strips_wave,
                                            const uint8_t *__restrict__ ws, float *__restrict__ state, int wave, int lane,
                                            const Water &w, bool fmt_ok, ClosedSums &cs, const RangeCodes &rc, Chain *chain = nullptr) {
    AccOne acc;
    float Jp[3] = {0.f, 0.f, 0.f};
    stream_strips<kFmt, 3, false, kPrimed, Chain>(
        lds, plan, strips, n_strips_wave, ws, wave, lane, rc.fullB,
        [&](const uint8_t *sp) {
            const float *f = reinterpret_cast<const float *>(sp);
#pragma unroll
            for (int c = 0; c < 3; ++c) {
                Jp[c] = kJOnly ? 0.0f : finite_or_zero(f[c * kStripPx + lane]);
            }
#pragma unroll
            for (int q = 0; q < 9; ++q)
#pragma unroll
                for (int c = 0; c < 3; ++c) acc.q[q][c] = 0.f;
        },
        [&](const uint8_t *sp, bool masked) {
            float zz[kGroupLv];
            uint32_t cc[3];
            read_chunk<kFmt>(sp, lane, zz, cc, rc, masked);
            if (masked) accumulate_chunk<true, kScaledB>(zz, cc, w, Jp, acc);
            else accumulate_chunk<false, kScaledB>(zz, cc, w, Jp, acc);
        },
        [&](const uint8_t *sp, uint32_t r) {
            for (uint32_t j = 0; j < r; ++j) {
                float z;
                uint32_t k[3];
                read_level<kFmt>(sp, lane, r, j, z, k, rc);
                accumulate_level<kScaledB>(z, k, w, Jp, acc);
            }
        },
        [&](uint32_t strip, const uint8_t *) {
            float *st = state + (size_t)strip * kStateFloats;
#pragma unroll
            for (int c = 0; c < 3; ++c) {
                const float N = acc.q[0][c], D = acc.q[1][c];
                const float dJ = N / D;
                const float Jc = fmt_ok ? Jp[c] + dJ : __builtin_nanf("");
                store_stepped<Chain>(&st[c * kStripPx + lane], Jc);
                if (!kJOnly && D != 0.0f) {
                    cs.sB[c] += __builtin_fmaf(-dJ, acc.q[3][c], acc.q[2][c]);
                    cs.sBeta[c] += Jc * __builtin_fmaf(-dJ, acc.q[5][c], acc.q[4][c]);
                    cs.sGZ[c] += __builtin_fmaf(-dJ, acc.q[7][c], acc.q[6][c]);
                    cs.cost += __builtin_fmaf(-dJ, N, acc.q[8][c]);
                } else if (!kJOnly && N != 0.0f) {
                    cs.sB[c] += kScaledB ? dJ * w.B[c] : dJ;
                    cs.sBeta[c] += dJ;
                    cs.sGZ[c] += dJ;
                    cs.cost += __builtin_inff();
                }
            }
        },
        chain);
}

template <int kFmt, bool kPrimed = false, class Chain = NoChain>
__device__ __forceinline__ void run_closed_pass(bool scaled, FitLds &lds, const PlanItem *__restrict__ plan, const StripEntry *__restrict__ strips,
                                                uint32_t n_strips_wave, const uint8_t *__restrict__ ws, float *__restrict__ state, int wave, int lane,
                                                const Water &w, bool fmt_ok, ClosedSums &cs, const RangeCodes &rc, Chain *chain = nullptr) {
    if (kScaledBBuilt && scaled) closed_pass<kFmt, false, true, kPrimed, Chain>(lds, plan, strips, n_strips_wave, ws, state, wave, lane, w, fmt_ok, cs, rc, chain);
    else closed_pass<kFmt, false, false, kPrimed, Chain>(lds, plan, strips, n_strips_wave, ws, state, wave, lane, w, fmt_ok, cs, rc, chain);
}

template <bool kFused, int kFmt, bool kJOnly>
__global__ __launch_bounds__(256, kClosedWaves) void fit_closed_kernel(const uint8_t *__restrict__ ws,
                                                         const PlanItem *__restrict__ plan, const StripEntry *__restrict__ plan_strips, const uint32_t *__restrict__ plan_count,
                                                       uint32_t plan_stride, uint32_t plan_kmax,
                                                         float *pstate, const uint64_t *__restrict__ n_obs_total,
                                                         float *__restrict__ state, float *partials, const AdamCoef co,
                                                         unsigned *ticket, double *gpart, int n_groups, double *sums,
                                                         double *trace_row, const uint32_t *__restrict__ obs_format) {
    __shared__ FitLds lds;
    const int t = threadIdx.x;
    const int lane = t & 63;
    const int wave = __builtin_amdgcn_readfirstlane(t >> 6);
    const Water w = load_water_uniform(pstate);
    const RangeCodes rc = range_codes<kFmt>(obs_format);
    const bool fmt_ok = store_matches<kFmt>(obs_format);
    const uint32_t wid = blockIdx.x * 4u + (uint32_t)wave;
    const uint32_t n_mine = (fmt_ok || kJOnly) ? plan_count[wid] : 0u;
    ClosedSums cs = {{0.f, 0.f, 0.f}, {0.f, 0.f, 0.f}, {0.f, 0.f, 0.f}, fmt_ok ? 0.f : __builtin_nanf("")};
    if (kExpWaveTimes && !kJOnly && lane == 0 && wid < kExpWaveSlots) g_exp_wave_times[0][wid] = wall_clock64();
    if (kJOnly) closed_pass<kFmt, true, false>(lds, plan + (size_t)wid * plan_stride, plan_strips + (size_t)wid * plan_kmax, n_mine, ws, state, wave, lane, w, fmt_ok, cs, rc);
    else run_closed_pass<kFmt>(pass_scaled_b(w), lds, plan + (size_t)wid * plan_stride, plan_strips + (size_t)wid * plan_kmax, n_mine, ws, state, wave, lane, w, fmt_ok, cs, rc);
    if (kExpWaveTimes && !kJOnly && lane == 0 && wid < kExpWaveSlots) g_exp_wave_times[1][wid] = wall_clock64();
    if (kJOnly) return;
    float s[kNumSums];
    pack_sums(s, cs.sB, cs.sGZ, cs.sBeta, cs.cost);
    finish_launch<kFused>(lds, s, partials, co, ticket, gpart, n_groups, sums, pstate, n_obs_total, trace_row);
}

struct Params9 { float v[9]; };
static Params9 params9(const float *p) {
    Params9 q;
    for (int i = 0; i < 9; ++i) q.v[i] = p[i];
    return q;
}

constexpr int kGroupFitWaves = kFitWaves > 5 ? 5 : kFitWaves;

struct GroupImage {
    uint8_t *ws;
    uint64_t off_plan[2], off_strips[2], off_count[2], off_state, off_format, off_params;
    uint32_t stride[2], kmax[2], n_waves[2];
};

struct GroupHeader {
    float pstate[2][32];
    double sums[kSumsPad];
    unsigned ticket[(1 + (kFitGrid + kGroup - 1) / kGroup) * kTicketStride];
    double gpart[kNumSums * ((kFitGrid + kGroup - 1) / kGroup)];
    float partials[kNumSums * kFitGrid];
};

__host__ __device__ __forceinline__ GroupImage *group_images(GroupHeader *g) {
    return reinterpret_cast<GroupImage *>(reinterpret_cast<uint8_t *>(g) + align_up(sizeof(GroupHeader), 256));
}

__device__ __forceinline__ float ld_agent(const float *p) { return __hip_atomic_load(p, __ATOMIC_RELAXED, __HIP_MEMORY_SCOPE_AGENT); }
__device__ __forceinline__ double ld_agent(const double *p) { return __hip_atomic_load(p, __ATOMIC_RELAXED, __HIP_MEMORY_SCOPE_AGENT); }
__device__ __forceinline__ void st_agent(float *p, float v) { __hip_atomic_store(p, v, __ATOMIC_RELAXED, __HIP_MEMORY_SCOPE_AGENT); }

__device__ __forceinline__ void group_water_step(const double *__restrict__ sums, const float *__restrict__ in,
                                                 uint64_t n_obs_total, const AdamCoef &co, bool apply, float &p, float &m, float &v) {
    const int q = threadIdx.x & 63;
    p = m = v = 0.f;
    if (q < 9) {
        p = ld_agent(in + q); m = ld_agent(in + 9 + q); v = ld_agent(in + 18 + q);
        if (apply) {
            const float scale = (1.0f / 3.0f) / (float)n_obs_total;
            const double g = water_grad(q, scale, [&](int i) { return ld_agent(sums + i); }, [&](int c) { return ld_agent(in + c); });
            adam_update(p, m, v, (float)g, co);
        }
    }
}

template <int kMode, int kFmt>
__global__ __launch_bounds__(256, kMode ? kClosedWaves : kGroupFitWaves) void group_iter_kernel(GroupHeader *g, int n_images, uint64_t n_obs_total,
                                                                                           const AdamCoef co_prev, const AdamCoef co, int apply,
                                                                                           int in, int out, double *trace_prev, int n_groups,
// ... 219 lines not shown
            if (!v.fmt_ok) acc.cost = __builtin_nanf("");
            float sBeta[3] = {0.f, 0.f, 0.f};
            run_grad_pass<kFmt, true, StreamChain>(pass_scaled_b(v.w), lds, v.plan, v.strips, v.n_mine, v.ws, v.state, wave, lane, v.w, v.gscale, co, acc, sBeta, v.rc, &ch);
            const float q[kNumSums] = {acc.sB[0], acc.sB[1], acc.sB[2], acc.sGZ[0], acc.sGZ[1], acc.sGZ[2], sBeta[0], sBeta[1], sBeta[2], acc.cost};
#pragma unroll
            for (int j = 0; j < kNumSums; ++j) s[j] = q[j];
        } else {
            ClosedSums cs = {{0.f, 0.f, 0.f}, {0.f, 0.f, 0.f}, {0.f, 0.f, 0.f}, v.fmt_ok ? 0.f : __builtin_nanf("")};
            run_closed_pass<kFmt, true, StreamChain>(pass_scaled_b(v.w), lds, v.plan, v.strips, v.n_mine, v.ws, v.state, wave, lane, v.w, v.fmt_ok, cs, v.rc, &ch);
            const float q[kNumSums] = {cs.sB[0], cs.sB[1], cs.sB[2], cs.sGZ[0], cs.sGZ[1], cs.sGZ[2], cs.sBeta[0], cs.sBeta[1], cs.sBeta[2], cs.cost};
#pragma unroll
            for (int j = 0; j < kNumSums; ++j) s[j] = q[j];
        }
        if (more && !chained) {
            asm volatile("s_waitcnt lgkmcnt(0)" ::: "memory");
            prime(vn);
        }
        wave_sums(s);
        if (lane == 0) {
#pragma unroll
            for (int j = 0; j < kNumSums; ++j) blds.wsum[slot][wave][j] = s[j];
        }
        v = vn;
    }
    __syncthreads();
    for (int idx = t; idx < slot * kNumSums; idx += 256) {
        const int sl = idx / kNumSums, j = idx - sl * kNumSums;
        const uint32_t q = blockIdx.x + (uint32_t)sl * P, i = q / vblocks, vb = q - i * vblocks;
        float *partials = reinterpret_cast<float *>(images[i].ws + images[i].o.partials);
        __hip_atomic_store(partials + (size_t)j * vblocks + vb,
                           ((blds.wsum[sl][0][j] + blds.wsum[sl][1][j]) + blds.wsum[sl][2][j]) + blds.wsum[sl][3][j], __ATOMIC_RELAXED, __HIP_MEMORY_SCOPE_AGENT);
    }
}

constexpr int kTailThreads = 16 * kBatchMax;
__global__ __launch_bounds__(kTailThreads) void batch_tail_kernel(const BatchEntry *__restrict__ images, int n_images, int n_blocks, const AdamCoef co, int row) {
    __shared__ double stot[kBatchMax][kNumSums];
    __shared__ int is_last;
    const int t = threadIdx.x, g = blockIdx.x, n_groups = gridDim.x;
    const int i = t >> 4, q = t & 15;
    const bool mine = i < n_images && q < kNumSums;
    uint8_t *ws = mine ? images[i].ws : nullptr;
    if (mine)
        reduce_group_thread(reinterpret_cast<const float *>(ws + images[i].o.partials), n_blocks, g, q, reinterpret_cast<double *>(ws + images[i].o.gpart), n_groups);
    float p = 0.f, m = 0.f, v = 0.f, Bc = 0.f, scale = 0.f;
    float *pstate = nullptr;
    bool scaled = false;
    if (mine && q < 9) {
        pstate = reinterpret_cast<float *>(ws + images[i].o.params);
        scale = (1.0f / 3.0f) / (float)(*reinterpret_cast<const uint64_t *>(ws + images[i].o.n_obs_total));
        p = pstate[q]; m = pstate[9 + q]; v = pstate[18 + q];
        Bc = pstate[q % 3];
        scaled = scaled_b_ok(pstate[0], pstate[1], pstate[2]);
    }
    unsigned *ticket = reinterpret_cast<unsigned *>(images[0].ws + images[0].o.ticket);
    if (!arrive_last(ticket, (unsigned)n_groups, &is_last)) return;
    if (mine) {
        const double y = unscale_sum(reduce_total_thread(reinterpret_cast<const double *>(ws + images[i].o.gpart), n_groups, q), q, scaled, Bc);
        __hip_atomic_store(reinterpret_cast<double *>(ws + images[i].o.sums) + q, y, __ATOMIC_RELAXED, __HIP_MEMORY_SCOPE_AGENT);
        stot[i][q] = y;
    }
    __syncthreads();
    if (!mine) return;
    double *trace = images[i].trace;
    if (q < 9) {
        const double grad = water_grad(q, scale, [&](int j) { return stot[i][j]; }, [&](int) { return Bc; });
        adam_update(p, m, v, (float)grad, co);
        pstate[q] = p; pstate[9 + q] = m; pstate[18 + q] = v;
        if (trace) trace[(size_t)row * 10 + 1 + q] = (double)p;
    } else if (trace) {
        trace[(size_t)row * 10] = stot[i][9];
    }
}

constexpr uint32_t batch_full_grid(int mode) { return (uint32_t)(mode ? kClosedGrid : 256 * kGroupFitWaves); }
constexpr int batch_images(uint32_t vblocks, uint32_t full) { return vblocks <= full ? kBatchMax : (int)((uint64_t)kBatchMax * full / vblocks); }
static_assert(batch_images(kClosedGrid, batch_full_grid(1)) == kBatchMax && batch_images(kFitGrid, batch_full_grid(0)) >= 1, "a launch takes at least one image");
static_assert(SUCRE_FIT_WAVES > 5 || batch_images(kFitGrid, batch_full_grid(0)) == kBatchMax, "the product's launches take kBatchMax images");

constexpr int kBatchSet = 8;
struct BatchEntries { BatchEntry e[kBatchSet]; };
__global__ void batch_set_kernel(BatchEntry *dst, const BatchEntries src, int n) {
    if ((int)threadIdx.x < n) dst[threadIdx.x] = src.e[threadIdx.x];
}

__global__ __launch_bounds__(256) void reduce_groups_kernel(const float *partials, int n_blocks, double *gpart,
                                                            int n_groups) {
    reduce_group(partials, n_blocks, blockIdx.x, gpart, n_groups);
}

__global__ __launch_bounds__(256) void reduce_sums_kernel(const double *gpart, int n_groups, double *__restrict__ sums, const float *__restrict__ pstate) {
    __shared__ double stot[kSumsPad];
    reduce_total(gpart, n_groups, stot, sums, pstate);
}

__global__ __launch_bounds__(64) void param_step_kernel(const double *__restrict__ sums, float *__restrict__ pstate,
                                                        const uint64_t *__restrict__ n_obs_total, const AdamCoef co,
                                                        double *__restrict__ trace_row) {
    water_step(sums, pstate, n_obs_total, co, trace_row);
}

__global__ __launch_bounds__(256) void fit_init_kernel(const uint8_t *__restrict__ rgb1,
                                                       const float *__restrict__ depth1,
                                                       const float *__restrict__ J0, int H, int W, int tiles_x,
                                                       const uint32_t *__restrict__ perm, float *__restrict__ state,
                                                       float *__restrict__ pstate,
                                                       unsigned *__restrict__ ticket, int n_tickets,
                                                       const Params9 p0) {
    const int tile = blockIdx.x, t = threadIdx.x;
    const uint32_t src = perm[(size_t)tile * kTilePx + t];
    const int stile = src / kTilePx, sslot = src % kTilePx;
    const int ty = stile / tiles_x, tx = stile - ty * tiles_x;
    const int v = ty * kTile + (sslot >> 4), u = tx * kTile + (sslot & 15);
    const bool inside = v < H && u < W;
    const size_t o = inside ? (size_t)v * W + u : 0;
    const bool valid = inside && !(depth1[o] <= 0.0f);
    float *st = state + ((size_t)tile * kStripsPerTile + (t >> 6)) * kStateFloats + (t & 63);
#pragma unroll
    for (int c = 0; c < 3; ++c) {
        float Jc = __builtin_nanf("");
        if (valid) Jc = J0 ? J0[o * 3 + c] : unit_from_u8(rgb1[o * 3 + c]);
        st[c * kStripPx] = Jc;
        st[(3 + c) * kStripPx] = 0.f;
        st[(6 + c) * kStripPx] = 0.f;
    }
    if (tile == 0 && t < 27) pstate[t] = t < 9 ? p0.v[t] : 0.f;
    for (int i = tile * 256 + t; i < n_tickets; i += gridDim.x * 256) ticket[i] = 0u;
}

__global__ __launch_bounds__(256) void export_J_kernel(const float *__restrict__ state, int H, int W, int tiles_x,
                                                       const uint32_t *__restrict__ invperm, float *__restrict__ J) {
    const int tile = blockIdx.x, t = threadIdx.x;
    const int ty = tile / tiles_x, tx = tile - ty * tiles_x;
    const int v = ty * kTile + (t >> 4), u = tx * kTile + (t & 15);
    if (v >= H || u >= W) return;
    const uint32_t dst = invperm[(size_t)tile * kTilePx + t];
    const size_t o = ((size_t)v * W + u) * 3;
    const float *st = state + (size_t)(dst / kStripPx) * kStateFloats + dst % kStripPx;
#pragma unroll
    for (int c = 0; c < 3; ++c) J[o + c] = st[c * kStripPx];
}

__global__ void set_n_obs_total_kernel(uint64_t *dst, uint64_t v) { *dst = v; }

hipError_t launch_fit_init(const Layout &L, uint8_t *ws, const uint8_t *rgb1, const float *depth1,
                           const float *params0, const float *J0, hipStream_t s) {
    hipLaunchKernelGGL(fit_init_kernel, dim3(L.n_tiles), dim3(256), 0, s, rgb1, depth1, J0, L.H, L.W, L.tiles_x,
                       reinterpret_cast<const uint32_t *>(ws + L.off_perm), reinterpret_cast<float *>(ws + L.off_state),
                       reinterpret_cast<float *>(ws + L.off_params),
                       reinterpret_cast<unsigned *>(ws + L.off_ticket), (1 + L.n_groups) * kTicketStride, params9(params0));
    return hipGetLastError();
}

template <class Kernel>
static void launch_fit_kernel(Kernel kernel, int mode, const Layout &L, uint8_t *ws, const AdamCoef &co, double *trace_row,
                              hipStream_t s) {
    hipLaunchKernelGGL(kernel, dim3(L.fit_blocks[mode]), dim3(256), 0, s, ws,
                       reinterpret_cast<const PlanItem *>(ws + L.off_plan[mode]),
                       reinterpret_cast<const StripEntry *>(ws + L.off_plan_strips[mode]),
                       reinterpret_cast<const uint32_t *>(ws + L.off_plan_count[mode]), (uint32_t)L.plan_stride[mode], (uint32_t)L.plan_kmax[mode],
                       reinterpret_cast<float *>(ws + L.off_params),
                       reinterpret_cast<const uint64_t *>(ws + L.off_n_obs_total),
                       reinterpret_cast<float *>(ws + L.off_state), reinterpret_cast<float *>(ws + L.off_partials), co,
                       reinterpret_cast<unsigned *>(ws + L.off_ticket),
                       reinterpret_cast<double *>(ws + L.off_gpartials), L.fit_groups[mode],
                       reinterpret_cast<double *>(ws + L.off_sums), trace_row,
                       reinterpret_cast<const uint32_t *>(ws + off_store_format(L)));
}

template <class F>
static void dispatch_fit(int mode, bool u16, F f) {
    using Zero = std::integral_constant<int, 0>;
    using One = std::integral_constant<int, 1>;
    if (mode) { if (u16) f(One{}, One{}); else f(One{}, Zero{}); }
    else { if (u16) f(Zero{}, One{}); else f(Zero{}, Zero{}); }
}
static int fit_mode(unsigned flags) { return (flags & SUCRE_FIT_CLOSED_FORM) ? 1 : 0; }
static bool fit_u16(unsigned flags) { return (flags & SUCRE_FIT_OBS_U16MM) != 0; }

template <bool kFused>
static void launch_grad_variant(const Layout &L, uint8_t *ws, const AdamCoef &co, unsigned flags, double *trace_row,
                                hipStream_t s) {
    dispatch_fit(fit_mode(flags), fit_u16(flags), [&](auto mode, auto fmt) {
        if constexpr (mode.value) launch_fit_kernel(fit_closed_kernel<kFused, fmt.value, false>, 1, L, ws, co, trace_row, s);
        else launch_fit_kernel(fit_grad_kernel<kFused, fmt.value>, 0, L, ws, co, trace_row, s);
    });
}

hipError_t launch_fit_iter_fused(const Layout &L, uint8_t *ws, const AdamCoef &co, unsigned flags,
                                 double *trace_row, hipStream_t s) {
    launch_grad_variant<true>(L, ws, co, flags, trace_row, s);
    return hipGetLastError();
}

hipError_t launch_fit_grad(const Layout &L, uint8_t *ws, const AdamCoef &co, unsigned flags, hipStream_t s) {
    launch_grad_variant<false>(L, ws, co, flags, nullptr, s);
    const int mode = fit_mode(flags);
    hipLaunchKernelGGL(reduce_groups_kernel, dim3(L.fit_groups[mode]), dim3(256), 0, s,
                       reinterpret_cast<const float *>(ws + L.off_partials), L.fit_blocks[mode],
                       reinterpret_cast<double *>(ws + L.off_gpartials), L.fit_groups[mode]);
    hipLaunchKernelGGL(reduce_sums_kernel, dim3(1), dim3(256), 0, s,
                       reinterpret_cast<const double *>(ws + L.off_gpartials), L.fit_groups[mode],
                       reinterpret_cast<double *>(ws + L.off_sums), reinterpret_cast<const float *>(ws + L.off_params));
    return hipGetLastError();
}

hipError_t launch_fit_step(const Layout &L, uint8_t *ws, const AdamCoef &co, double *trace_row, hipStream_t s) {
    hipLaunchKernelGGL(param_step_kernel, dim3(1), dim3(64), 0, s, reinterpret_cast<const double *>(ws + L.off_sums),
                       reinterpret_cast<float *>(ws + L.off_params),
                       reinterpret_cast<const uint64_t *>(ws + L.off_n_obs_total), co, trace_row);
    return hipGetLastError();
}

hipError_t launch_update_J(const Layout &L, uint8_t *ws, int fmt, hipStream_t s) {
    dispatch_fit(1, fmt != 0, [&](auto, auto f) { launch_fit_kernel(fit_closed_kernel<false, f.value, true>, 1, L, ws, AdamCoef{}, nullptr, s); });
    return hipGetLastError();
}

hipError_t launch_plan(const Layout &L, uint8_t *ws, hipStream_t s) {
    auto *meta = reinterpret_cast<const StripMeta *>(ws + L.off_strip_meta);
    const uint32_t W0 = (uint32_t)L.fit_blocks[0] * 4u, W1 = (uint32_t)L.fit_blocks[1] * 4u;
    const uint32_t Wmax = W0 < W1 ? W1 : W0;
    uint32_t Kmax = (uint32_t)(L.plan_kmax[0] > L.plan_kmax[1] ? L.plan_kmax[0] : L.plan_kmax[1]);
    if (Kmax < 32u) Kmax = 32u;
    hipLaunchKernelGGL(plan_kernel, dim3((Wmax * Kmax + 255u) / 256u, 2), dim3(256), 0, s, meta, L.n_strips,
                       reinterpret_cast<const uint32_t *>(ws + off_store_format(L)), W0, W1, Kmax,
                       (uint32_t)L.plan_stride[0], (uint32_t)L.plan_stride[1], (uint32_t)L.plan_kmax[0], (uint32_t)L.plan_kmax[1],
                       reinterpret_cast<PlanItem *>(ws + L.off_plan[0]), reinterpret_cast<PlanItem *>(ws + L.off_plan[1]),
                       reinterpret_cast<StripEntry *>(ws + L.off_plan_strips[0]), reinterpret_cast<StripEntry *>(ws + L.off_plan_strips[1]),
                       reinterpret_cast<uint32_t *>(ws + L.off_plan_count[0]),
                       reinterpret_cast<uint32_t *>(ws + L.off_plan_count[1]), (uint64_t)L.off_comp, (uint64_t)L.off_state);
    return hipGetLastError();
}

hipError_t launch_export_J(const Layout &L, const uint8_t *ws, float *J, hipStream_t s) {
    hipLaunchKernelGGL(export_J_kernel, dim3(L.n_tiles), dim3(256), 0, s,
                       reinterpret_cast<const float *>(ws + L.off_state), L.H, L.W, L.tiles_x,
                       reinterpret_cast<const uint32_t *>(ws + L.off_invperm), J);
    return hipGetLastError();
}

struct ImageRef {
    uint64_t plan, strips, count, state, format, params;
    uint32_t stride, kmax, n_waves;
};
static ImageRef image_ref(const Layout &L, int mode) {
    return ImageRef{L.off_plan[mode], L.off_plan_strips[mode], L.off_plan_count[mode], L.off_state, off_store_format(L), L.off_params,
                    (uint32_t)L.plan_stride[mode], (uint32_t)L.plan_kmax[mode], (uint32_t)L.fit_blocks[mode] * 4u};
}

size_t batch_bytes(int n_images) { return align_up((size_t)n_images * sizeof(BatchEntry), 256); }

hipError_t launch_batch_set(void *batch, int n_images, uint8_t *const *ws, double *const *trace, const Layout *layouts, unsigned flags,
                            hipStream_t s) {
    const int mode = fit_mode(flags);
    for (int i0 = 0; i0 < n_images; i0 += kBatchSet) {
        BatchEntries src;
        const int n = n_images - i0 < kBatchSet ? n_images - i0 : kBatchSet;
        for (int j = 0; j < kBatchSet; ++j) {
            const Layout &L = layouts[j < n ? i0 + j : i0];
            const ImageRef r = image_ref(L, mode);
            const BatchOffsets o = {r.plan, r.strips, r.count, r.params, L.off_n_obs_total, r.state, L.off_partials, L.off_ticket,
                                    L.off_gpartials, L.off_sums, r.format, r.stride, r.kmax, L.fit_groups[mode]};
            src.e[j] = BatchEntry{j < n ? ws[i0 + j] : nullptr, (j < n && trace) ? trace[i0 + j] : nullptr, o};
        }
        hipLaunchKernelGGL(batch_set_kernel, dim3(1), dim3(64), 0, s, static_cast<BatchEntry *>(batch) + i0, src, n);
    }
    return hipGetLastError();
}

hipError_t launch_batch_iter(const Layout &L, void *batch, int n_images, const AdamCoef &co, unsigned flags, int row, hipStream_t s) {
    const int mode = fit_mode(flags);
    const uint32_t vblocks = (uint32_t)L.fit_blocks[mode];
    const uint32_t full = batch_full_grid(mode);
    const int per_launch = batch_images(vblocks, full);
    for (int i0 = 0; i0 < n_images; i0 += per_launch) {
        auto *b = static_cast<const BatchEntry *>(batch) + i0;
        const int n = n_images - i0 < per_launch ? n_images - i0 : per_launch;
        const uint32_t pairs = (uint32_t)n * vblocks;
        const dim3 grid(pairs < full ? pairs : full);
        dispatch_fit(mode, fit_u16(flags), [&](auto m, auto f) {
            hipLaunchKernelGGL((batch_iter_kernel<m.value, f.value>), grid, dim3(256), 0, s, b, n, co, row, vblocks);
        });
        hipLaunchKernelGGL(batch_tail_kernel, dim3(L.fit_groups[mode]), dim3(kTailThreads), 0, s, b, n, L.fit_blocks[mode], co, row);
    }
    return hipGetLastError();
}

size_t group_bytes(int n_images) { return align_up(sizeof(GroupHeader), 256) + (size_t)n_images * sizeof(GroupImage); }

int64_t group_sums_offset() { return (int64_t)offsetof(GroupHeader, sums); }

hipError_t launch_group_init(void *group, const float *params0, hipStream_t s) {
    hipLaunchKernelGGL(group_init_kernel, dim3(1), dim3(64), 0, s, static_cast<GroupHeader *>(group), params9(params0));
    return hipGetLastError();
}

hipError_t launch_group_set_image(void *group, int i, const Layout &L, uint8_t *ws, hipStream_t s) {
    GroupImage im;
    im.ws = ws;
    for (int m = 0; m < 2; ++m) {
        const ImageRef r = image_ref(L, m);
        im.off_plan[m] = r.plan; im.off_strips[m] = r.strips; im.off_count[m] = r.count;
        im.stride[m] = r.stride; im.kmax[m] = r.kmax; im.n_waves[m] = r.n_waves;
        im.off_state = r.state; im.off_format = r.format; im.off_params = r.params;
    }
    hipLaunchKernelGGL(group_set_image_kernel, dim3(1), dim3(1), 0, s, static_cast<GroupHeader *>(group), i, im);
    return hipGetLastError();
}

hipError_t launch_group_iter(void *group, int n_images, int step, const AdamCoef &co_prev, const AdamCoef &co, unsigned flags,
                             uint64_t n_obs_total, double *trace_prev, hipStream_t s) {
    auto *g = static_cast<GroupHeader *>(group);
    const int apply = step > 1 ? 1 : 0;
    const int in = apply ? (step - 2) & 1 : 0, out = apply ? (step - 1) & 1 : 0;
    dispatch_fit(fit_mode(flags), fit_u16(flags), [&](auto m, auto f) {
        constexpr int grid = m.value ? kClosedGrid : kFitGrid, ng = (grid + kGroup - 1) / kGroup;
        hipLaunchKernelGGL((group_iter_kernel<m.value, f.value>), dim3(grid), dim3(256), 0, s, g, n_images, n_obs_total, co_prev, co, apply, in, out,
                           trace_prev, ng, group_images(g));
    });
    return hipGetLastError();
}

hipError_t launch_group_finish(void *group, int n_images, int step, const AdamCoef &co_prev, uint64_t n_obs_total,
                               double *trace_prev, hipStream_t s) {
    const int apply = step >= 1 ? 1 : 0;
    const int in = apply ? (step - 1) & 1 : 0, out = apply ? step & 1 : 0;
    hipLaunchKernelGGL(group_finish_kernel, dim3(1), dim3(64), 0, s, static_cast<GroupHeader *>(group), n_images, n_obs_total, co_prev,
                       apply, in, out, trace_prev);
    return hipGetLastError();
}

hipError_t launch_set_n_obs_total(const Layout &L, uint8_t *ws, uint64_t n, hipStream_t s) {
    hipLaunchKernelGGL(set_n_obs_total_kernel, dim3(1), dim3(1), 0, s,
                       reinterpret_cast<uint64_t *>(ws + L.off_n_obs_total), n);
    return hipGetLastError();
}

}
```

### sucre_amd/csrc/launch.h

```cpp
#pragma once
#include <hip/hip_runtime.h>

#include "../../include/sucre_hip.h"
#include "layout.h"

namespace sucre {

struct CamDev {
    float K[9], Kinv[9], R[9], t[3], Rinv[9], tinv[3];
    int H, W;
};

struct AdamCoef {
    float w1;
    float beta2;
    float w2;
    float step_size_neg;
    float bc2_sqrt;
    float eps;
};

AdamCoef adam_coef(int step, double lr, double beta1, double beta2, double eps);

hipError_t launch_match(const Layout &L, uint8_t *ws, const sucre_view_t &target, const sucre_view_t *views_dev,
                        int k0, int k1, hipStream_t s, uint8_t *ext = nullptr, int ext_mode = SUCRE_EXT_POINTS,
                        uint8_t *ext2 = nullptr);
hipError_t launch_match_map(const Layout &L, const sucre_view_t &target, const sucre_view_t *views_dev, int k,
                            int32_t *map, hipStream_t s);
hipError_t launch_pack_view(const float *depth, const uint8_t *rgb, int H, int W, void *packed, hipStream_t s);
hipError_t launch_pack_views(const float *const *depth, const uint8_t *const *rgb, void *const *packed, int n, int H, int W, hipStream_t s);
hipError_t launch_project_points(const sucre_view_t &view, const float *wP, long long n, int32_t *pix, hipStream_t s);
hipError_t launch_import_view(const Layout &L, uint8_t *ws, int k, const int16_t *u1, const int16_t *v1, const float *z,
                              const uint8_t *rgb, long long n, hipStream_t s, uint8_t *ext_dense = nullptr,
                              const float *ext = nullptr, uint8_t *ext2_dense = nullptr);
hipError_t launch_export_view_ext(const Layout &L, const uint8_t *ws, const uint8_t *ext_dense, int k, float *out, hipStream_t s);
hipError_t launch_finalize(const Layout &L, uint8_t *ws, double min_cover, hipStream_t s,
                           const uint8_t *ext_dense = nullptr, uint8_t *ext_comp = nullptr, int fmt = SUCRE_OBS_F32,
                           const uint8_t *ext2_dense = nullptr, uint8_t *ext2_comp = nullptr);
hipError_t launch_compact(const Layout &L, uint8_t *ws, hipStream_t s, const uint8_t *ext_dense = nullptr,
                          uint8_t *ext_comp = nullptr, int fmt = SUCRE_OBS_F32, const uint8_t *ext2_dense = nullptr,
                          uint8_t *ext2_comp = nullptr);
hipError_t launch_check_store(const Layout &L, const uint8_t *ws, uint32_t *verdict, uint64_t *scratch, hipStream_t s);
hipError_t launch_export_view(const Layout &L, const uint8_t *ws, int k, float *z, uint8_t *rgb, hipStream_t s);

hipError_t launch_fit_init(const Layout &L, uint8_t *ws, const uint8_t *rgb1, const float *depth1,
                           const float *params0, const float *J0, hipStream_t s);
hipError_t launch_fit_iter_fused(const Layout &L, uint8_t *ws, const AdamCoef &co, unsigned flags, double *trace_row,
                                 hipStream_t s);
hipError_t launch_fit_grad(const Layout &L, uint8_t *ws, const AdamCoef &co, unsigned flags, hipStream_t s);
hipError_t launch_fit_step(const Layout &L, uint8_t *ws, const AdamCoef &co, double *trace_row, hipStream_t s);
hipError_t launch_update_J(const Layout &L, uint8_t *ws, int fmt, hipStream_t s);
hipError_t launch_plan(const Layout &L, uint8_t *ws, hipStream_t s);
hipError_t launch_export_J(const Layout &L, const uint8_t *ws, float *J, hipStream_t s);
hipError_t launch_set_n_obs_total(const Layout &L, uint8_t *ws, uint64_t n, hipStream_t s);
size_t group_bytes(int n_images);
int64_t group_sums_offset();
hipError_t launch_group_init(void *group, const float *params0, hipStream_t s);
hipError_t launch_group_set_image(void *group, int i, const Layout &L, uint8_t *ws, hipStream_t s);
hipError_t launch_group_iter(void *group, int n_images, int step, const AdamCoef &co_prev, const AdamCoef &co, unsigned flags,
                             uint64_t n_obs_total, double *trace_prev, hipStream_t s);
hipError_t launch_group_finish(void *group, int n_images, int step, const AdamCoef &co_prev, uint64_t n_obs_total,
                               double *trace_prev, hipStream_t s);

size_t batch_bytes(int n_images);
hipError_t launch_batch_set(void *batch, int n_images, uint8_t *const *ws, double *const *trace, const Layout *layouts, unsigned flags,
                            hipStream_t s);
hipError_t launch_batch_iter(const Layout &L, void *batch, int n_images, const AdamCoef &co, unsigned flags, int row, hipStream_t s);

size_t residual_scratch_bytes(const Layout &L);
hipError_t launch_residuals(const Layout &L, const uint8_t *ws, int fmt, int32_t *count, float *ssr, double *view_stats,
                            void *scratch, hipStream_t s);
hipError_t launch_residuals_ext(const Layout &L, const uint8_t *ws, const uint8_t *lws, unsigned flags, int32_t *count, float *ssr,
                                double *view_stats, void *scratch, hipStream_t s);

size_t trim_scratch_bytes(const Layout &L);
hipError_t launch_trim(const Layout &L, uint8_t *ws, int fmt, double k_sigma, const double *view_stats, int32_t *dropped,
                       int64_t *view_dropped, float *tau2, void *scratch, hipStream_t s);
hipError_t launch_trim_ext(const Layout &L, uint8_t *ws, const uint8_t *lws, unsigned flags, double k_sigma, const double *view_stats,
                           int32_t *dropped, int64_t *view_dropped, float *tau2, void *scratch, hipStream_t s);

size_t gain_scratch_bytes(const Layout &L);
hipError_t launch_view_gains(const Layout &L, const uint8_t *ws, int fmt, double limit, double *gains, float *inv, double *sums,
                             void *scratch, hipStream_t s);
hipError_t launch_view_gains_ext(const Layout &L, const uint8_t *ws, const uint8_t *lws, unsigned flags, double limit, double *gains,
                                 float *inv, double *sums, void *scratch, hipStream_t s);
hipError_t launch_apply_view_gains(const Layout &L, uint8_t *ws, const float *inv, int64_t *view_clipped, void *scratch, hipStream_t s);
hipError_t launch_apply_view_gains_ext(const Layout &L, uint8_t *ws, uint8_t *lws, unsigned flags, const float *inv,
                                       int64_t *view_clipped, void *scratch, hipStream_t s);

size_t invert_bytes(int n_images);
uint64_t invert_blocks(int H, int W);
hipError_t launch_invert(void *table, int n_images, const sucre_invert_image_t *images, const float *params, unsigned flags,
                         hipStream_t s);
hipError_t launch_invert_light(void *table, int n_images, uint32_t n_blocks, bool float_colour, hipStream_t s);

size_t select_scratch_bytes();
hipError_t launch_select_ranks(const float *J, int H, int W, int n_ranks, const uint64_t *ranks, float *out, void *scratch,
                               hipStream_t s);
hipError_t launch_plot_stretch(const float *J, int H, int W, const float *lo, const float *hi, uint8_t *out, hipStream_t s);
hipError_t launch_count_valid(const float *J, int H, int W, uint64_t *count, hipStream_t s);

size_t pool_state_bytes();
size_t pool_table_bytes(int n_images);
hipError_t launch_pool_begin(void *state, hipStream_t s);
hipError_t launch_pool_pass(void *state, int pass, void *table, int n_images, const sucre_pool_image_t *images, int n_ranks,
                            hipStream_t s);
hipError_t launch_pool_locate(void *state, int pass, int n_ranks, const uint64_t *ranks, float *out, hipStream_t s);

size_t light_workspace_bytes(const Layout &L, int ext_sets = 1);
uint8_t *light_ext2_dense(const Layout &L, uint8_t *lws);
uint8_t *light_ext2_comp(const Layout &L, uint8_t *lws);
int64_t light_params_offset(const Layout &L);
uint8_t *light_ext_dense(const Layout &L, uint8_t *lws);
uint8_t *light_ext_comp(const Layout &L, uint8_t *lws);
hipError_t launch_light_init(const Layout &L, uint8_t *lws, const float *params19, hipStream_t s);
hipError_t launch_light_deal(const Layout &L, uint8_t *ws, uint8_t *lws, unsigned flags, hipStream_t s);
hipError_t launch_light_iter(const Layout &L, uint8_t *ws, uint8_t *lws, const AdamCoef &co, unsigned flags,
                             double *trace_row, hipStream_t s);
hipError_t launch_light_update_J(const Layout &L, uint8_t *ws, uint8_t *lws, unsigned flags, hipStream_t s);
size_t light_group_bytes(int n_images);
int64_t light_group_sums_offset();
hipError_t launch_light_group_init(void *group, int n_images, const Layout *L, uint8_t *const *ws, uint8_t *const *lws,
                                   const float *params19, hipStream_t s);
hipError_t launch_light_group_iter(void *group, int n_images, const Layout *L, uint8_t *const *ws, uint8_t *const *lws, int step,
                                   const AdamCoef &co_prev, const AdamCoef &co, unsigned flags, uint64_t n_obs_total,
                                   double *trace_prev, bool write_deal, hipStream_t s);
hipError_t launch_light_group_finish(void *group, int n_images, const Layout *L, uint8_t *const *ws, uint8_t *const *lws, int step,
                                     const AdamCoef &co_prev, unsigned flags, uint64_t n_obs_total, double *trace_prev, hipStream_t s);

}
```

### sucre_amd/csrc/layout.h

```cpp
#pragma once
#include <stddef.h>
#include <stdint.h>

#include "experiment.h"

namespace sucre {

constexpr int kTile = 16;
constexpr int kTilePx = 256;
constexpr int kChunkZ = 1024;
constexpr int kChunkRGB = 768;
constexpr int kChunk = kChunkZ + kChunkRGB;
constexpr int kChunkZ16 = 512;
constexpr int kChunk16 = kChunkZ16 + kChunkRGB;
constexpr float kMmPerM = 1000.0f, kMPerMm = 0.001f;
constexpr int kStoreF32 = 0, kStoreU16 = 1, kStoreZ24 = 2, kStoreZ26 = 3;
constexpr int kChunk24 = 6 * 256;
constexpr int kChunk26 = kChunk24 + 64;
__host__ __device__ constexpr int chunk_bytes(int fmt) { return fmt == kStoreU16 ? kChunk16 : fmt == kStoreZ24 ? kChunk24 : fmt == kStoreZ26 ? kChunk26 : kChunk; }
__host__ __device__ constexpr uint32_t padded_levels(int fmt, uint32_t levels) { return fmt == kStoreZ26 ? (levels + 3u) & ~3u : levels; }
constexpr int kExtChunk = 3 * kChunkZ;
constexpr int kStripPx = 64;
constexpr int kStripsPerTile = kTilePx / kStripPx;
constexpr int kGroupLv = 4;
constexpr int kStateFloats = 9 * kStripPx;
__host__ __device__ constexpr int range_bytes(int fmt) { return fmt == kStoreU16 ? 2 : (fmt == kStoreZ24 || fmt == kStoreZ26) ? 3 : 4; }
__host__ __device__ constexpr int level_bytes(int fmt) { return (range_bytes(fmt) + 3) * kStripPx + (fmt == kStoreZ26 ? kStripPx / 4 : 0); }
static_assert(kGroupLv * level_bytes(kStoreZ26) == kChunk26 && kChunk26 % 64 == 0, "a 26-bit chunk is four levels and a whole number of 64-byte units");
constexpr int kExtLevelBytes = 3 * 4 * kStripPx;

struct StripMeta {
    uint64_t lvoff;
    uint32_t levels;
    uint32_t full;
};
constexpr int kNumSums = 10;
constexpr int kSumsPad = 12;
constexpr int kGroup = 32;
constexpr int kTicketStride = 16;
constexpr int kFitWaves = SUCRE_FIT_WAVES;
constexpr int kClosedWaves = SUCRE_CLOSED_WAVES;
constexpr int kFitGrid = 256 * kFitWaves;
constexpr int kClosedGrid = 256 * kClosedWaves;
constexpr int kMaxViews = 4096;
constexpr int kMinStripsPerWave = SUCRE_MIN_STRIPS;

constexpr uint32_t kDealDen = 64;
constexpr int kMaxGen = 8;
struct DealShares { uint32_t G; uint32_t p[kMaxGen]; };

__host__ __device__ inline DealShares deal_shares(int mode, uint32_t blocks) {
    const uint32_t fit[kMaxGen] = {SUCRE_DEAL_FIT}, closed[kMaxGen] = {SUCRE_DEAL_CLOSED};
    DealShares sh;
    const uint32_t G = (uint32_t)(mode ? kClosedWaves : kFitWaves);
    bool weighted = blocks == 256u * G && G <= (uint32_t)kMaxGen;
    for (uint32_t g = 0; weighted && g < G; ++g) weighted = (mode ? closed[g] : fit[g]) >= 1u && (mode ? closed[g] : fit[g]) <= kDealDen;
    weighted = weighted && (mode ? closed[0] : fit[0]) == kDealDen;
    bool all_equal = true;
    for (uint32_t g = 0; g < G && g < (uint32_t)kMaxGen; ++g) all_equal = all_equal && (mode ? closed[g] : fit[g]) == kDealDen;
    weighted = weighted && !all_equal;
    sh.G = weighted ? G : 1u;
    for (int g = 0; g < kMaxGen; ++g) sh.p[g] = weighted && (uint32_t)g < G ? (mode ? closed[g] : fit[g]) : kDealDen;
    return sh;
}

__host__ __device__ inline DealShares deal_shares_resident(uint32_t blocks) {
    const uint32_t four[kMaxGen] = {SUCRE_DEAL_CLOSED}, five[kMaxGen] = {SUCRE_DEAL_FIT};
    DealShares sh;
    const bool g4 = blocks == 1024u && kClosedWaves == 4, g5 = blocks == 1280u && kFitWaves == 5;
    sh.G = g4 ? 4u : g5 ? 5u : 1u;
    bool all_equal = true;
    for (int g = 0; g < kMaxGen; ++g) {
        sh.p[g] = (g4 && g < 4) ? four[g] : (g5 && g < 5) ? five[g] : kDealDen;
        all_equal = all_equal && sh.p[g] == kDealDen;
    }
    if (all_equal || sh.p[0] != kDealDen) { sh.G = 1u; for (int g = 0; g < kMaxGen; ++g) sh.p[g] = kDealDen; }
    return sh;
}

template <class L, class F>
__host__ __device__ inline uint32_t deal_walk(uint32_t wid, uint32_t W, uint32_t n_strips, const DealShares &sh, L &&levels, F &&f) {
    const uint32_t Wg = W / sh.G, g = wid / Wg, j = wid - g * Wg;
    uint32_t base = 0u, k = 0u;
    uint32_t work[kMaxGen] = {0u, 0u, 0u, 0u, 0u, 0u, 0u, 0u};
    for (uint32_t r = 0u; base < n_strips; ++r) {
        const uint32_t items = sh.G > 1u ? ((levels(base) + 3u) >> 2) + 2u : 0u;
        uint32_t below = 0u, total = 0u;
        bool mine = false;
        for (uint32_t q = 0u; q < sh.G; ++q) {
            if (q > 0u && (uint64_t)(2u * work[q] + items) * kDealDen > (uint64_t)2u * sh.p[q] * work[0]) continue;
            work[q] += items;
            ++total;
            below += q < g ? 1u : 0u;
            mine = mine || q == g;
        }
        const uint32_t n_r = total * Wg;
        if (mine) {
            const uint32_t rank = below * Wg + j, strip = base + ((r & 1u) ? n_r - 1u - rank : rank);
            if (strip < n_strips) { f(k, strip); ++k; }
        }
        base += n_r;
    }
    return k;
}

__host__ __device__ inline uint32_t deal_rounds(uint32_t W, uint32_t n_strips, const DealShares &sh) {
    const uint32_t per_round = sh.G > 1u ? W / sh.G : W;
    return (n_strips + per_round - 1u) / per_round;
}

struct PlanItem {
    uint32_t src64;
    uint32_t shape;
};
struct StripEntry {
    uint32_t strip;
    uint32_t counts;
};
constexpr uint32_t kCountBits = 12;
static_assert(kMaxViews / kGroupLv < (1 << kCountBits), "StripEntry.counts: a strip's full chunks must fit their field");
__host__ __device__ constexpr uint32_t strip_counts(uint32_t unmasked, uint32_t masked, uint32_t tail) { return unmasked | (masked << kCountBits) | (tail << (2 * kCountBits)); }
__host__ __device__ constexpr uint32_t counts_unmasked(uint32_t c) { return c & ((1u << kCountBits) - 1u); }
__host__ __device__ constexpr uint32_t counts_masked(uint32_t c) { return (c >> kCountBits) & ((1u << kCountBits) - 1u); }
__host__ __device__ constexpr uint32_t counts_tail(uint32_t c) { return (c >> (2 * kCountBits)) & 7u; }
static_assert(counts_unmasked(strip_counts(kMaxViews / kGroupLv, 0, 3)) == kMaxViews / kGroupLv && counts_masked(strip_counts(0, kMaxViews / kGroupLv, 3)) == kMaxViews / kGroupLv
              && counts_masked(strip_counts(kMaxViews / kGroupLv, 0, 3)) == 0 && counts_tail(strip_counts(1023, 1, 3)) == 3, "StripEntry.counts round trip at the largest strip");

struct Layout {
    int H, W, n_views, tiles_x, tiles_y, n_tiles;
    size_t off_obs;
    size_t obs_tile_stride, obs_view_stride;
    size_t off_cnt;
    size_t off_comp;
    size_t off_pcount;
    size_t off_pmask;
    int mask_words;
    size_t off_vbits;
    size_t off_blockhist;
    size_t off_bin_totals;
    size_t off_perm;
    size_t off_invperm;
    int n_strips;
    size_t off_strip_meta;
    size_t off_total_chunks;
    size_t off_zrange;
    size_t off_zpart;
    size_t off_view_count;
    size_t off_view_keep;
    size_t off_view_partial;
    size_t off_n_obs;
    size_t off_n_obs_total;
    size_t off_params;
    size_t off_sums;
    size_t off_ticket;
    size_t off_gpartials;
    int n_blocks, n_groups;
    int fit_blocks[2], fit_groups[2];
    size_t off_partials;
    size_t off_state;
    size_t off_plan[2];
    size_t off_plan_strips[2];
    size_t off_plan_count[2];
    size_t plan_stride[2];
    size_t plan_kmax[2];
    size_t total;
};

__host__ __device__ inline size_t align_up(size_t x, size_t a) { return (x + a - 1) / a * a; }

inline size_t off_store_format(const Layout &L) { return L.off_total_chunks + sizeof(uint64_t); }
inline size_t off_range_span(const Layout &L) { return off_store_format(L) + 2 * sizeof(uint32_t); }

inline bool make_layout(int H, int W, int n_views, Layout *L) {
    if (H <= 0 || W <= 0 || n_views <= 0 || n_views > kMaxViews || H > 32767 || W > 32767) return false;
    L->H = H; L->W = W; L->n_views = n_views;
    L->tiles_x = (W + kTile - 1) / kTile;
    L->tiles_y = (H + kTile - 1) / kTile;
    L->n_tiles = L->tiles_x * L->tiles_y;
    const size_t nt = (size_t)L->n_tiles, nv = (size_t)n_views;
    size_t o = 0;
    auto take = [&](size_t bytes) { size_t r = o; o = align_up(o + bytes, 256); return r; };
    L->off_obs = take(nt * nv * kChunk);
    L->obs_tile_stride = nv * kChunk; L->obs_view_stride = kChunk;
    L->off_cnt = take(nt * nv * sizeof(uint16_t));
    const size_t comp_f32 = nt * nv * kChunk, comp_z26 = nt * (nv + 3) * kChunk26;
    L->off_comp = take(comp_f32 > comp_z26 ? comp_f32 : comp_z26);
    L->off_pcount = take(nt * kTilePx * sizeof(uint16_t));
    L->mask_words = (n_views + 63) / 64;
    L->off_pmask = take(nt * kTilePx * (size_t)L->mask_words * sizeof(uint64_t));
    L->off_vbits = take(nt * nv * 4 * sizeof(uint64_t));
    L->off_blockhist = take(256 * nt * sizeof(uint32_t));
    L->off_bin_totals = take(512 * sizeof(uint32_t));
    L->off_perm = take(nt * kTilePx * sizeof(uint32_t));
    L->off_invperm = take(nt * kTilePx * sizeof(uint32_t));
    L->n_strips = L->n_tiles * kStripsPerTile;
    L->off_strip_meta = take((size_t)L->n_strips * sizeof(StripMeta));
    L->off_total_chunks = take(sizeof(uint64_t));
    L->off_zrange = take(nt * nv * 2 * sizeof(uint32_t));
    L->off_zpart = take((nt + 31) / 32 * 2 * sizeof(uint32_t));
    L->off_view_count = take(nv * sizeof(uint64_t));
    L->off_view_keep = take(nv * sizeof(uint32_t));
    L->off_view_partial = take((nt + 31) / 32 * nv * sizeof(uint32_t));
    L->off_n_obs = take(sizeof(uint64_t));
    L->off_n_obs_total = take(sizeof(uint64_t));
    L->off_params = take(27 * sizeof(float));
    L->off_sums = take(kSumsPad * sizeof(double));
    auto grid_of = [&](int full) { const int want = (L->n_tiles + kMinStripsPerWave - 1) / kMinStripsPerWave; return want < 1 ? 1 : (want < full ? want : full); };
    L->n_blocks = grid_of(kFitGrid);
    L->n_groups = (L->n_blocks + kGroup - 1) / kGroup;
    L->fit_blocks[0] = L->n_blocks;
    L->fit_blocks[1] = grid_of(kClosedGrid);
    for (int m = 0; m < 2; ++m) L->fit_groups[m] = (L->fit_blocks[m] + kGroup - 1) / kGroup;
    L->off_ticket = take((size_t)(1 + L->n_groups) * kTicketStride * sizeof(uint32_t));
    L->off_gpartials = take((size_t)kNumSums * L->n_groups * sizeof(double));
    L->off_partials = take(nt * kNumSums * sizeof(float));
    L->off_state = take((size_t)L->n_strips * kStateFloats * sizeof(float));
    {
        for (int m = 0; m < 2; ++m) {
            const size_t waves = (size_t)L->fit_blocks[m] * 4;
            L->plan_kmax[m] = deal_rounds((uint32_t)waves, (uint32_t)L->n_strips, deal_shares(m, (uint32_t)L->fit_blocks[m]));
            L->plan_stride[m] = L->plan_kmax[m] * (((size_t)n_views + kGroupLv - 1) / kGroupLv + 2) + SUCRE_RING;
            L->off_plan[m] = take(waves * L->plan_stride[m] * sizeof(PlanItem));
            L->off_plan_strips[m] = take(waves * L->plan_kmax[m] * sizeof(StripEntry));
            L->off_plan_count[m] = take(waves * sizeof(uint32_t));
        }
    }
    L->total = o;
    return true;
}

}
```

### sucre_amd/engine.py

```python
from __future__ import annotations

import contextlib
import ctypes as C
import os
import threading
from dataclasses import dataclass

import numpy as np
import torch

from . import _lib


@dataclass
class DeviceView:
    depth: torch.Tensor
    rgb: torch.Tensor
    K: torch.Tensor
    R: torch.Tensor
    t: torch.Tensor
    name: str = ''
    Kinv: torch.Tensor | None = None
    tinv: torch.Tensor | None = None

    def to_struct(self, packed: bool = False) -> _lib.SucreView:
        slot = '_struct_packed' if packed else '_struct'
        key = (self.depth.data_ptr(), self.rgb.data_ptr())
        if packed and self.__dict__.get('_packed') is not None:
            key = key + (self.__dict__['_packed'][1].data_ptr(),)
        cached = self.__dict__.get(slot)
        if cached is not None and cached[0] == key:
            return cached[1]
        if packed:
            H, W = self.depth.shape
            records = self.packed_records()
            key = key + (records.data_ptr(),)
            s = camera_struct(self.K, self.R, self.t, H, W, records.data_ptr(), 0, Kinv=self.Kinv, tinv=self.tinv)
        else:
            s = self._build_struct()
        self.__dict__[slot] = (key, s)
        return s

    def packed_records(self) -> torch.Tensor:
        key = (self.depth.data_ptr(), self.rgb.data_ptr())
        cached = self.__dict__.get('_packed')
        if cached is not None and cached[0] == key:
            return cached[1]
        assert self.rgb.dtype == torch.uint8, 'packed records hold uint8 colours'
        with _PACK_LOCK:
            cached = self.__dict__.get('_packed')
            if cached is not None and cached[0] == key:
                return cached[1]
            H, W = self.depth.shape
            dev = self.depth.device
            out = torch.empty(H * W * 8, dtype=torch.uint8, device=dev)
            with torch.cuda.device(dev):
                side = _pack_stream(dev)
                side.wait_stream(torch.cuda.current_stream(dev))
                with torch.cuda.stream(side):
                    _lib.check(_lib.load().sucre_pack_view(C.c_void_p(self.depth.data_ptr()), C.c_void_p(self.rgb.data_ptr()), H, W,
                                                           C.c_void_p(out.data_ptr()), _stream_ptr()))
                    done = torch.cuda.Event()
                    done.record()
            self.__dict__['_packed'] = [key, out, done, True]
            return out

    def repack(self) -> None:
        records = self.packed_records()
        self.wait_packed()
        H, W = self.depth.shape
        with torch.cuda.device(self.depth.device):
            _lib.check(_lib.load().sucre_pack_view(C.c_void_p(self.depth.data_ptr()), C.c_void_p(self.rgb.data_ptr()), H, W,
                                                   C.c_void_p(records.data_ptr()), _stream_ptr()))

    def twin(self) -> 'DeviceView':
        return DeviceView(depth=self.depth, rgb=self.rgb, K=self.K, R=self.R, t=self.t, name=self.name, Kinv=self.Kinv, tinv=self.tinv)

    def wait_packed(self) -> None:
        entry = self.__dict__.get('_packed')
        if entry is not None and entry[3]:
            if entry[2].query():
                entry[3] = False
            else:
                torch.cuda.current_stream(self.depth.device).wait_event(entry[2])

    def as_float_colour(self) -> 'DeviceView':
        if self.rgb.dtype == torch.float32:
            return self
        twin = self.__dict__.get('_float_twin')
        if twin is None:
            twin = DeviceView(depth=self.depth, rgb=(self.rgb.to(torch.float64) / 255).to(torch.float32).contiguous(),
                              K=self.K, R=self.R, t=self.t, name=self.name)
            self.__dict__['_float_twin'] = twin
        return twin

    def _build_struct(self) -> _lib.SucreView:
        H, W = self.depth.shape
        assert self.depth.dtype == torch.float32 and self.depth.is_contiguous() and self.depth.is_cuda
        assert self.rgb.dtype in (torch.uint8, torch.float32) and self.rgb.is_contiguous() and self.rgb.shape == (H, W, 3)
        return camera_struct(self.K, self.R, self.t, H, W, self.depth.data_ptr(), self.rgb.data_ptr(), Kinv=self.Kinv, tinv=self.tinv)


def repack_views(views: list) -> None:
    views = [v for v in views if v.rgb.dtype == torch.uint8]
    if not views:
        return
    H, W = views[0].depth.shape
    if any(tuple(v.depth.shape) != (H, W) for v in views):
        for v in views:
            v.repack()
        return
    recs = [v.packed_records() for v in views]
    for v in views:
        v.wait_packed()
    n = len(views)
    dp = (C.c_void_p * n)(*[v.depth.data_ptr() for v in views])
    cp = (C.c_void_p * n)(*[v.rgb.data_ptr() for v in views])
    op = (C.c_void_p * n)(*[r.data_ptr() for r in recs])
    with torch.cuda.device(views[0].depth.device):
        _lib.check(_lib.load().sucre_pack_views(dp, cp, op, n, H, W, _stream_ptr()))


def camera_struct(K: torch.Tensor, R: torch.Tensor, t: torch.Tensor, H: int, W: int, depth_ptr: int = 0,
                  rgb_ptr: int = 0, Kinv: torch.Tensor | None = None, tinv: torch.Tensor | None = None) -> _lib.SucreView:
    K = K.to(torch.float32).cpu()
    R = R.to(torch.float32).cpu()
    t = t.to(torch.float32).cpu().view(3, 1)
    Kinv = K.inverse() if Kinv is None else Kinv.to(torch.float32).cpu().view(3, 3)
    Rinv = R.T
    tinv = -R.T @ t if tinv is None else tinv.to(torch.float32).cpu().view(3, 1)
    s = _lib.SucreView()
    s.depth, s.rgb, s.H, s.W = depth_ptr or None, rgb_ptr or None, int(H), int(W)
    for name, val in (('K', K), ('Kinv', Kinv), ('R', R), ('t', t), ('Rinv', Rinv), ('tinv', tinv)):
        flat = val.contiguous().view(-1).tolist()
        setattr(s, name, (C.c_float * len(flat))(*flat))
    return s


def project_points(view: _lib.SucreView, wP: torch.Tensor) -> torch.Tensor:
    assert wP.is_cuda and wP.dtype == torch.float32 and wP.dim() == 2 and wP.shape[0] == 3
    wP = wP.contiguous()
    n = wP.shape[1]
    out = torch.empty(n, dtype=torch.int32, device=wP.device)
    with torch.cuda.device(wP.device):
        _lib.check(_lib.load().sucre_project_points(C.byref(view), C.c_void_p(wP.data_ptr()), n, C.c_void_p(out.data_ptr()),
                                                    _stream_ptr()))
    return out


_PACK_STREAMS: dict = {}
_PACK_LOCK = threading.Lock()


def _pack_stream(dev) -> 'torch.cuda.Stream':
    key = str(dev)
    if key not in _PACK_STREAMS:
        _PACK_STREAMS[key] = torch.cuda.Stream(dev)
    return _PACK_STREAMS[key]


PACKED_VIEWS = os.environ.get('SUCRE_PACKED_VIEWS', '1') != '0'

MAX_VIEWS = 4096


def _stream_ptr() -> C.c_void_p:
    return C.c_void_p(torch.cuda.current_stream().cuda_stream)


class Restoration:

    def __init__(self, height: int, width: int, n_views: int, device: str | torch.device = 'cuda', light: bool = False,
                 obs_format: str = 'f32', float_colour: bool = False):
        self.lib = _lib.load()
        self.light = bool(light)
        self.float_colour = bool(float_colour)
        self.both = self.light and self.float_colour
        if self.float_colour and obs_format != 'f32':
            raise NotImplementedError('float32 colours need the f32 store')
        if obs_format not in _lib.OBS_FORMATS:
            raise ValueError(f'obs_format must be one of {sorted(_lib.OBS_FORMATS)}, not {obs_format!r}')
        if self.light and obs_format != 'f32':
            raise NotImplementedError('the artificial-light model keeps float32 camera points: obs_format must be f32')
        self.obs_format = obs_format
        self._streams_used: dict = {}
        self._fmt = _lib.OBS_FORMATS[obs_format]
        self._fmt_flag = _lib.FIT_OBS_U16MM if self._fmt == _lib.OBS_U16MM else 0
        self.H, self.W, self.n_views = int(height), int(width), int(n_views)
        self.capacity = int(n_views)
        self.device = torch.device(device)
        if self.device.type != 'cuda':
            raise _lib.SucreError('the HIP engine needs a GPU device (there is no CPU fallback)')
        nbytes = self.lib.sucre_workspace_bytes(self.H, self.W, self.n_views)
        if nbytes == 0:
            raise _lib.SucreError(self.lib.sucre_last_error().decode())
        self.ws = torch.empty(nbytes, dtype=torch.uint8, device=self.device)
        assert self.ws.data_ptr() % 256 == 0
        self.lws = None
        if self.light or self.float_colour:
            lbytes = (self.lib.sucre_light_workspace_bytes_ext(self.H, self.W, self.n_views, _lib.EXT_POINTS_COLOUR) if self.both
                      else self.lib.sucre_light_workspace_bytes(self.H, self.W, self.n_views))
            self.lws = torch.empty(lbytes, dtype=torch.uint8, device=self.device)
            assert self.lws.data_ptr() % 256 == 0
        self._views_dev = None
        self._views_host = torch.empty(self.capacity * C.sizeof(_lib.SucreView), dtype=torch.uint8).pin_memory()
        self._views_buf = torch.empty(self.capacity * C.sizeof(_lib.SucreView), dtype=torch.uint8, device=self.device)
        self._views_copied = None
        self._keepalive = []
        self._batch_table = None
        self.trace = None
        self.steps_done = 0
        self.min_cover = None

    def _sp(self) -> C.c_void_p:
        st = torch.cuda.current_stream(self.device)
        self._streams_used[st.cuda_stream] = st
        return C.c_void_p(st.cuda_stream)

    @property
    def _ext_mode(self) -> int:
        return _lib.EXT_POINTS_COLOUR if self.both else _lib.EXT_COLOUR if self.float_colour else _lib.EXT_POINTS

    @property
    def _ext_flag(self) -> int:
        return _lib.FIT_EXT_BOTH if self.both else _lib.FIT_EXT_COLOUR if self.float_colour else 0

    @property
    def _geom(self):
        return C.c_void_p(self.ws.data_ptr()), self.H, self.W, self.n_views

    def _note_stream(self) -> None:
        if self.device.type == 'cuda':
            st = torch.cuda.current_stream(self.device)
            self._streams_used[st.cuda_stream] = st

    def _region(self, region: int, dtype: torch.dtype, count: int) -> torch.Tensor:
        self._note_stream()
        off = self.lib.sucre_ws_offset(self.H, self.W, self.n_views, region)
        if off < 0:
            raise _lib.SucreError(self.lib.sucre_last_error().decode())
        nbytes = count * torch.empty((), dtype=dtype).element_size()
        return self.ws[off:off + nbytes].view(dtype)

    def match(self, target: DeviceView, views: list[DeviceView], min_cover: float = 1e-6, packed: bool | None = None) -> None:
        assert 1 <= len(views) <= self.capacity, (len(views), self.capacity)
        self.min_cover = float(min_cover)
        self.n_views = len(views)
        tgt = target.to_struct()
        packed = (PACKED_VIEWS if packed is None else bool(packed)) and not self.float_colour
        table = (_lib.SucreView * self.n_views)(*[v.to_struct(packed) for v in views])
        if packed:
            with torch.cuda.device(self.device):
                for v in views:
                    v.wait_packed()
        nbytes = C.sizeof(table)
        if self._views_copied is not None:
            self._views_copied.synchronize()
        self._views_host[:nbytes].copy_(torch.frombuffer(bytearray(bytes(table)), dtype=torch.uint8))
        self._views_dev = self._views_buf[:nbytes]
        with torch.cuda.device(self.device):
            self._views_dev.copy_(self._views_host[:nbytes], non_blocking=True)
            self._views_copied = torch.cuda.Event()
            self._views_copied.record()
        self._keepalive = [target, views]
        ws, H, W, n = self._geom
        with torch.cuda.device(self.device):
            want = torch.float32 if self.float_colour else torch.uint8
            assert all(v.rgb.dtype == want for v in views), f'this restoration takes {want} colour images'
            if self.light or self.float_colour:
                lws = C.c_void_p(self.lws.data_ptr())
                fn = (self.lib.sucre_match_views_light_fcolour if self.both else
                      self.lib.sucre_match_views_fcolour if self.float_colour else self.lib.sucre_match_views_light)
                _lib.check(fn(ws, lws, H, W, n, C.byref(tgt), C.c_void_p(self._views_dev.data_ptr()), 0, n, self._sp()))
                _lib.check(self.lib.sucre_finalize_matches_ext(ws, lws, H, W, n, float(min_cover), self._ext_mode, self._sp()))
            else:
                _lib.check(self.lib.sucre_match_views(ws, H, W, n, C.byref(tgt), C.c_void_p(self._views_dev.data_ptr()),
                                                      0, n, self._sp()))
                _lib.check(self.lib.sucre_finalize_matches_fmt(ws, H, W, n, float(min_cover), self._fmt, self._sp()))

    def import_matches(self, target: DeviceView, lists: list, min_cover: float = -1.0) -> None:
        assert 1 <= len(lists) <= self.capacity, (len(lists), self.capacity)
        self.min_cover = float(min_cover)
        self.n_views = len(lists)
        self._keepalive = [target, lists]
        self._views_dev = None
        ws, H, W, n = self._geom
        ext_mode = self._ext_mode
        with torch.cuda.device(self.device):
            for k, item in enumerate(lists):
                u1, v1, z, rgb = item[:4]
                ext = item[4] if len(item) > 4 else None
                u1 = u1.to(self.device, torch.int16).contiguous(); v1 = v1.to(self.device, torch.int16).contiguous()
                z = z.to(self.device, torch.float32).contiguous()
                assert z.numel() == u1.numel() == v1.numel()
                if rgb is not None:
                    rgb = rgb.to(self.device, torch.uint8).contiguous()
                    assert rgb.shape == (u1.numel(), 3)
                self._keepalive.append((u1, v1, z, rgb))
                rgbp = C.c_void_p(rgb.data_ptr()) if rgb is not None else None
                if self.lws is not None:
                    planes = 6 if self.both else 3
                    assert ext is not None and ext.shape == (planes, u1.numel()), f'this restoration needs ({planes}, n) extension planes'
                    ext = ext.to(self.device, torch.float32).contiguous()
                    self._keepalive.append(ext)
                    _lib.check(self.lib.sucre_import_view_ext(ws, C.c_void_p(self.lws.data_ptr()), H, W, n, k,
                                                              C.c_void_p(u1.data_ptr()), C.c_void_p(v1.data_ptr()),
                                                              C.c_void_p(z.data_ptr()), rgbp, C.c_void_p(ext.data_ptr()),
                                                              u1.numel(), ext_mode, self._sp()))
                else:
                    _lib.check(self.lib.sucre_import_view(ws, H, W, n, k, C.c_void_p(u1.data_ptr()), C.c_void_p(v1.data_ptr()),
                                                          C.c_void_p(z.data_ptr()), rgbp, u1.numel(), self._sp()))
            if self.lws is not None:
                _lib.check(self.lib.sucre_finalize_matches_ext(ws, C.c_void_p(self.lws.data_ptr()), H, W, n,
                                                               float(min_cover), self._ext_mode, self._sp()))
            else:
                _lib.check(self.lib.sucre_finalize_matches_fmt(ws, H, W, n, float(min_cover), self._fmt, self._sp()))

    def match_map(self, k: int) -> torch.Tensor:
        assert self._views_dev is not None, 'call match() first'
        out = torch.empty((self.H, self.W), dtype=torch.int32, device=self.device)
        tgt = self._keepalive[0].to_struct()
        with torch.cuda.device(self.device):
            _lib.check(self.lib.sucre_match_map(self.H, self.W, self.n_views, C.byref(tgt),
                                                C.c_void_p(self._views_dev.data_ptr()), int(k),
                                                C.c_void_p(out.data_ptr()), self._sp()))
        return out

    def view_counts(self) -> torch.Tensor:
        return self._region(_lib.WS_VIEW_COUNT, torch.int64, self.n_views)

    def view_keep(self) -> torch.Tensor:
        return self._region(_lib.WS_VIEW_KEEP, torch.int32, self.n_views)

    def store_format(self) -> torch.Tensor:
        return self._region(_lib.WS_STORE_FORMAT, torch.int32, 4)

    def n_obs_device(self) -> torch.Tensor:
        return self._region(_lib.WS_N_OBS, torch.int64, 1)

    def n_obs(self) -> int:
        return int(self.n_obs_device().item())

    def export_view(self, k: int):
        z = torch.empty((self.H, self.W), dtype=torch.float32, device=self.device)
        rgb = torch.empty((self.H, self.W, 3), dtype=torch.uint8, device=self.device)
        ws, H, W, n = self._geom
        with torch.cuda.device(self.device):
            _lib.check(self.lib.sucre_export_view(ws, H, W, n, int(k), C.c_void_p(z.data_ptr()),
                                                  C.c_void_p(rgb.data_ptr()), self._sp()))
        return z, rgb

    def export_view_ext(self, k: int) -> torch.Tensor:
        assert self.lws is not None, 'this restoration keeps no extension planes'
        out = torch.empty((3, self.H, self.W), dtype=torch.float32, device=self.device)
        ws, H, W, n = self._geom
        with torch.cuda.device(self.device):
            _lib.check(self.lib.sucre_export_view_ext(ws, C.c_void_p(self.lws.data_ptr()), H, W, n, int(k),
                                                      C.c_void_p(out.data_ptr()), self._sp()))
        return out

    def export_view_colour(self, k: int) -> torch.Tensor:
        assert self.both, 'only a light restoration on float32 colours keeps a second set of extension planes'
        out = torch.empty((3, self.H, self.W), dtype=torch.float32, device=self.device)
        ws, H, W, n = self._geom
        with torch.cuda.device(self.device):
            _lib.check(self.lib.sucre_export_view_ext2(ws, C.c_void_p(self.lws.data_ptr()), H, W, n, int(k),
                                                       C.c_void_p(out.data_ptr()), self._sp()))
        return out

    def check_store(self) -> torch.Tensor:
        verdict = torch.empty(self.n_views, dtype=torch.int32, device=self.device)
        scratch = torch.empty(self.n_views, dtype=torch.int64, device=self.device)
        ws, H, W, n = self._geom
        with torch.cuda.device(self.device):
            _lib.check(self.lib.sucre_check_store(ws, H, W, n, C.c_void_p(verdict.data_ptr()),
                                                  C.c_void_p(scratch.data_ptr()), self._sp()))
        return verdict

    def fit_init(self, target: DeviceView, params0=None, J0: torch.Tensor | None = None) -> None:
        npar = 19 if (self.light or self.float_colour) else 9
        default = np.concatenate([np.full(9, 0.1), np.zeros(6), [1.0, 0.0, 0.0, 1.0]])
        p0 = default.copy() if params0 is None else np.asarray(params0, np.float64).reshape(-1)
        if self.float_colour and not self.light and p0.size == 9:
            p0 = np.concatenate([p0, default[9:]])
        p0 = p0.astype(np.float32).reshape(-1)[:npar] if params0 is None else p0.astype(np.float32).reshape(npar)
        p0c = (C.c_float * npar)(*p0.tolist())
        j0 = None
        if J0 is None and self.float_colour:
            J0 = target.rgb
        if J0 is not None:
            j0 = J0.to(self.device, torch.float32).contiguous()
            assert j0.shape == (self.H, self.W, 3)
            self._keepalive.append(j0)
        ws, H, W, n = self._geom
        with torch.cuda.device(self.device):
            j0p = C.c_void_p(j0.data_ptr()) if j0 is not None else None
            if self.light or self.float_colour:
                _lib.check(self.lib.sucre_fit_init_light(ws, C.c_void_p(self.lws.data_ptr()), H, W, n,
                                                         None if self.float_colour else C.c_void_p(target.rgb.data_ptr()),
                                                         C.c_void_p(target.depth.data_ptr()), p0c, j0p, self._sp()))
            else:
                _lib.check(self.lib.sucre_fit_init(ws, H, W, n, C.c_void_p(target.rgb.data_ptr()),
                                                   C.c_void_p(target.depth.data_ptr()), p0c, j0p, self._sp()))
        self.steps_done = 0

    def fit(self, num_iter: int = 200, lr: float = 0.05, use_closed_form: bool = False, betas=(0.9, 0.999),
            eps: float = 1e-8, record_trace: bool = True, keep_J: bool = False) -> torch.Tensor | None:
        ext = self.light or self.float_colour
        width = 20 if ext else 10
        trace = torch.zeros((num_iter, width), dtype=torch.float64, device=self.device) if record_trace else None
        flags = (_lib.FIT_CLOSED_FORM if use_closed_form else 0) | self._fmt_flag | self._ext_flag
        if keep_J and use_closed_form:
            flags |= _lib.FIT_KEEP_J
        ws, H, W, n = self._geom
        tp = C.c_void_p(trace.data_ptr()) if trace is not None else None
        with torch.cuda.device(self.device):
            if ext:
                _lib.check(self.lib.sucre_fit_run_light(ws, C.c_void_p(self.lws.data_ptr()), H, W, n, self.steps_done,
                                                        int(num_iter), float(lr), float(betas[0]), float(betas[1]),
                                                        float(eps), flags, tp, self._sp()))
            else:
                _lib.check(self.lib.sucre_fit_run(ws, H, W, n, self.steps_done, int(num_iter), float(lr),
                                                  float(betas[0]), float(betas[1]), float(eps), flags, tp,
                                                  self._sp()))
        self.steps_done += int(num_iter)
        if trace is not None and self.float_colour and not self.light:
            trace = trace[:, :10]
        self.trace = trace
        return trace

    def update_J(self) -> None:
        ws, H, W, n = self._geom
        with torch.cuda.device(self.device):
            if self.light or self.float_colour:
                _lib.check(self.lib.sucre_update_J_ext(ws, C.c_void_p(self.lws.data_ptr()), H, W, n, self._ext_flag, self._sp()))
            else:
                _lib.check(self.lib.sucre_update_J_fmt(ws, H, W, n, self._fmt, self._sp()))

    def residuals(self):
        count = torch.empty((self.H, self.W), dtype=torch.int32, device=self.device)
        ssr = torch.empty((self.H, self.W, 3), dtype=torch.float32, device=self.device)
        stats = torch.empty((self.n_views, 4), dtype=torch.float64, device=self.device)
        nbytes = self.lib.sucre_residual_scratch_bytes(self.H, self.W, self.n_views)
        if nbytes == 0:
            raise _lib.SucreError(self.lib.sucre_last_error().decode())
        scratch = torch.empty(nbytes, dtype=torch.uint8, device=self.device)
        ws, H, W, n = self._geom
        outs = (C.c_void_p(count.data_ptr()), C.c_void_p(ssr.data_ptr()), C.c_void_p(stats.data_ptr()), C.c_void_p(scratch.data_ptr()))
        with torch.cuda.device(self.device):
            if self.light or self.float_colour:
                _lib.check(self.lib.sucre_fit_residuals_ext(ws, C.c_void_p(self.lws.data_ptr()), H, W, n, self._ext_flag, *outs, self._sp()))
            else:
                _lib.check(self.lib.sucre_fit_residuals(ws, H, W, n, self._fmt, *outs, self._sp()))
        return count, ssr, stats

    def trim_outliers(self, k_sigma: float, residuals=None):
        k_sigma = float(k_sigma)
        if not (np.isfinite(k_sigma) and k_sigma > 0.0):
            raise ValueError(f'trim_outliers: k_sigma must be finite and > 0, not {k_sigma!r}')
        if self.min_cover is None:
            raise _lib.SucreError('trim_outliers: call match() or import_matches() first')
        stats = (self.residuals() if residuals is None else residuals)[2]
        assert stats.is_cuda and stats.dtype == torch.float64 and stats.is_contiguous() and stats.shape == (self.n_views, 4)
        dropped = torch.empty((self.H, self.W), dtype=torch.int32, device=self.device)
        view_dropped = torch.empty(self.n_views, dtype=torch.int64, device=self.device)
        thresholds = torch.empty(3, dtype=torch.float32, device=self.device)
        nbytes = self.lib.sucre_trim_scratch_bytes(self.H, self.W, self.n_views)
        if nbytes == 0:
            raise _lib.SucreError(self.lib.sucre_last_error().decode())
        scratch = torch.empty(nbytes, dtype=torch.uint8, device=self.device)
        ws, H, W, n = self._geom
        args = (k_sigma, C.c_void_p(stats.data_ptr()), C.c_void_p(dropped.data_ptr()), C.c_void_p(view_dropped.data_ptr()),
                C.c_void_p(thresholds.data_ptr()), C.c_void_p(scratch.data_ptr()))
        with torch.cuda.device(self.device):
            if self.lws is not None:
                lws = C.c_void_p(self.lws.data_ptr())
                _lib.check(self.lib.sucre_trim_outliers_ext(ws, lws, H, W, n, self._ext_flag, *args, self._sp()))
                _lib.check(self.lib.sucre_finalize_matches_ext(ws, lws, H, W, n, self.min_cover, self._ext_mode, self._sp()))
            else:
                _lib.check(self.lib.sucre_trim_outliers(ws, H, W, n, self._fmt, *args, self._sp()))
                _lib.check(self.lib.sucre_finalize_matches_fmt(ws, H, W, n, self.min_cover, self._fmt, self._sp()))
        self.steps_done = 0
        return dropped, view_dropped, thresholds

    def _gain_scratch(self) -> torch.Tensor:
        nbytes = self.lib.sucre_gain_scratch_bytes(self.H, self.W, self.n_views)
        if nbytes == 0:
            raise _lib.SucreError(self.lib.sucre_last_error().decode())
        return torch.empty(nbytes, dtype=torch.uint8, device=self.device)

    def view_gains(self, limit: float = 2.0):
        limit = float(limit)
        if not (np.isfinite(limit) and limit >= 1.0):
            raise ValueError(f'view_gains: limit must be finite and >= 1, not {limit!r}')
        gains = torch.empty((self.n_views, 3), dtype=torch.float64, device=self.device)
        inv = torch.empty((self.n_views, 3), dtype=torch.float32, device=self.device)
        sums = torch.empty((self.n_views, 7), dtype=torch.float64, device=self.device)
        scratch = self._gain_scratch()
        ws, H, W, n = self._geom
        outs = (limit, C.c_void_p(gains.data_ptr()), C.c_void_p(inv.data_ptr()), C.c_void_p(sums.data_ptr()), C.c_void_p(scratch.data_ptr()))
        with torch.cuda.device(self.device):
            if self.lws is not None:
                _lib.check(self.lib.sucre_view_gains_ext(ws, C.c_void_p(self.lws.data_ptr()), H, W, n, self._ext_flag, *outs, self._sp()))
            else:
                _lib.check(self.lib.sucre_view_gains(ws, H, W, n, self._fmt, *outs, self._sp()))
        return gains, inv, sums

    def apply_view_gains(self, inv: torch.Tensor) -> torch.Tensor:
        if self.min_cover is None:
            raise _lib.SucreError('apply_view_gains: call match() or import_matches() first')
        assert inv.is_cuda and inv.dtype == torch.float32 and inv.is_contiguous() and inv.shape == (self.n_views, 3)
        view_clipped = torch.empty(self.n_views, dtype=torch.int64, device=self.device)
        scratch = self._gain_scratch()
        ws, H, W, n = self._geom
        args = (C.c_void_p(inv.data_ptr()), C.c_void_p(view_clipped.data_ptr()), C.c_void_p(scratch.data_ptr()))
        with torch.cuda.device(self.device):
            if self.lws is not None:
                lws = C.c_void_p(self.lws.data_ptr())
                _lib.check(self.lib.sucre_apply_view_gains_ext(ws, lws, H, W, n, self._ext_flag, *args, self._sp()))
                _lib.check(self.lib.sucre_finalize_matches_ext(ws, lws, H, W, n, self.min_cover, self._ext_mode, self._sp()))
            else:
                _lib.check(self.lib.sucre_apply_view_gains(ws, H, W, n, *args, self._sp()))
                _lib.check(self.lib.sucre_finalize_matches_fmt(ws, H, W, n, self.min_cover, self._fmt, self._sp()))
        self.steps_done = 0
        return view_clipped

    def params(self) -> torch.Tensor:
        if self.light or self.float_colour:
            self._note_stream()
            off = self.lib.sucre_light_params_offset(self.H, self.W, self.n_views)
            return self.lws[off:off + (76 if self.light else 36)].view(torch.float32)
        return self._region(_lib.WS_PARAMS, torch.float32, 9)

    def J(self) -> torch.Tensor:
        out = torch.empty((self.H, self.W, 3), dtype=torch.float32, device=self.device)
        ws, H, W, n = self._geom
        with torch.cuda.device(self.device):
            _lib.check(self.lib.sucre_export_J(ws, H, W, n, C.c_void_p(out.data_ptr()), self._sp()))
        return out


def fit_batch(restorations: list, num_iter: int = 200, lr: float = 0.05, use_closed_form: bool = False, betas=(0.9, 0.999),
              eps: float = 1e-8, record_trace: bool = True, keep_J: bool = False) -> list:
    rs = list(restorations)
    if not rs:
        raise ValueError('fit_batch: no image')
    r0 = rs[0]
    for r in rs:
        if r.light or r.float_colour:
            raise NotImplementedError('fit_batch: the extension-plane modes (light model, float32 colours) are fitted one by one')
        if (r.H, r.W, str(r.device), r._fmt_flag, r.steps_done) != (r0.H, r0.W, str(r0.device), r0._fmt_flag, r0.steps_done):
            raise ValueError('fit_batch: one image size, device, observation format and Adam step per batch -- got '
                             f'{(r.H, r.W, str(r.device), r.obs_format, r.steps_done)} next to {(r0.H, r0.W, str(r0.device), r0.obs_format, r0.steps_done)}')
    if len({r.ws.data_ptr() for r in rs}) != len(rs):
        raise ValueError('fit_batch: every image needs its own workspace')
    n = len(rs)
    traces = [torch.zeros((num_iter, 10), dtype=torch.float64, device=r0.device) if record_trace else None for _ in rs]
    flags = (_lib.FIT_CLOSED_FORM if use_closed_form else 0) | r0._fmt_flag
    if keep_J and use_closed_form:
        flags |= _lib.FIT_KEEP_J
    lib = r0.lib
    table = torch.empty(lib.sucre_batch_bytes(n), dtype=torch.uint8, device=r0.device)
    ws = (C.c_void_p * n)(*[r.ws.data_ptr() for r in rs])
    tr = (C.c_void_p * n)(*[t.data_ptr() if t is not None else None for t in traces])
    nv = (C.c_int * n)(*[int(r.n_views) for r in rs])
    with torch.cuda.device(r0.device):
# ... 445 lines not shown
```

Measured before the change: 86.22.

## Fuse pairs of Adam fit iterations to avoid re-streaming J moments

Adds a paired fit path in which two consecutive Adam iterations are handled by an L pass and an F pass. The L pass writes only the gradient to a new gradient plane and skips loading and storing the moments. The F pass then applies the previous step's Adam update while it streams and computes the next gradient. This targets redundant state traffic in a bandwidth-bound loop, at the cost of an extra gradient-plane buffer, extra plan tables and more complex planning. It is on by default for the non-closed-form, non-extended fit and can be disabled with an env var or flag.

```diff
diff --git a/include/sucre_hip.h b/include/sucre_hip.h
--- a/include/sucre_hip.h
+++ b/include/sucre_hip.h
@@ -18,6 +18,7 @@
 #define SUCRE_FIT_CLOSED_FORM 1u
 #define SUCRE_FIT_OBS_U16MM 2u
 #define SUCRE_FIT_KEEP_J 8u
+#define SUCRE_FIT_UNPAIRED 32u
 
 #define SUCRE_OBS_F32 0
 #define SUCRE_OBS_U16MM 1
@@ -49,7 +50,9 @@
     SUCRE_WS_PARAMS = 3,
     SUCRE_WS_SUMS = 4,
     SUCRE_WS_N_OBS_TOTAL = 5,
-    SUCRE_WS_STORE_FORMAT = 6
+    SUCRE_WS_STORE_FORMAT = 6,
+    SUCRE_WS_STATE = 7,
+    SUCRE_WS_PAIR_GRADIENT = 8
 };
 
 int sucre_version(void);
diff --git a/sucre_amd/_lib.py b/sucre_amd/_lib.py
--- a/sucre_amd/_lib.py
+++ b/sucre_amd/_lib.py
@@ -12,10 +12,11 @@
 FIT_EXT_COLOUR = 4
 FIT_EXT_BOTH = 16
 FIT_KEEP_J = 8
+FIT_UNPAIRED = 32
 OBS_F32, OBS_U16MM, OBS_F32_PLAIN, OBS_F32_Z26 = 0, 1, 2, 3
 EXT_POINTS, EXT_COLOUR, EXT_POINTS_COLOUR = 1, 2, 3
 OBS_FORMATS = {'f32': OBS_F32, 'u16mm': OBS_U16MM, 'f32plain': OBS_F32_PLAIN, 'f32z26': OBS_F32_Z26}
-WS_VIEW_COUNT, WS_VIEW_KEEP, WS_N_OBS, WS_PARAMS, WS_SUMS, WS_N_OBS_TOTAL, WS_STORE_FORMAT = range(7)
+WS_VIEW_COUNT, WS_VIEW_KEEP, WS_N_OBS, WS_PARAMS, WS_SUMS, WS_N_OBS_TOTAL, WS_STORE_FORMAT, WS_STATE, WS_PAIR_GRADIENT = range(9)
 INVERT_LIGHT, INVERT_FLOAT_COLOUR = 1, 2
 INVERT_MAX_IMAGES = 4096
 POOL_MAX_IMAGES = 4096
diff --git a/sucre_amd/csrc/abi.hip b/sucre_amd/csrc/abi.hip
--- a/sucre_amd/csrc/abi.hip
+++ b/sucre_amd/csrc/abi.hip
@@ -87,6 +87,8 @@
         case SUCRE_WS_SUMS: return (int64_t)L.off_sums;
         case SUCRE_WS_N_OBS_TOTAL: return (int64_t)L.off_n_obs_total;
         case SUCRE_WS_STORE_FORMAT: return (int64_t)off_store_format(L);
+        case SUCRE_WS_STATE: return (int64_t)L.off_state;
+        case SUCRE_WS_PAIR_GRADIENT: return (int64_t)L.off_gplane;
         default: return fail(SUCRE_ERR_RANGE, "unknown workspace region %d", region);
     }
 }
@@ -215,14 +217,22 @@
     if (int rc = check_ws(ws, H, W, n_views, &L)) return rc;
     if (t0 < 0 || T < 0) return fail(SUCRE_ERR_RANGE, "t0=%d T=%d must be >= 0", t0, T);
     if (int rc = check_adam(t0 + 1, lr, beta1, beta2, eps)) return rc;
-    if (flags & ~(SUCRE_FIT_CLOSED_FORM | SUCRE_FIT_OBS_U16MM | SUCRE_FIT_KEEP_J)) return fail(SUCRE_ERR_ARG, "unknown fit flags 0x%x", flags);
+    if (flags & ~(SUCRE_FIT_CLOSED_FORM | SUCRE_FIT_OBS_U16MM | SUCRE_FIT_KEEP_J | SUCRE_FIT_UNPAIRED)) return fail(SUCRE_ERR_ARG, "unknown fit flags 0x%x", flags);
     if (trace_dev && !aligned(trace_dev, 8)) return fail(SUCRE_ERR_ARG, "trace must be 8-byte aligned");
     auto *w = static_cast<uint8_t *>(ws);
     auto s = static_cast<hipStream_t>(stream);
     const int fmt = (flags & SUCRE_FIT_OBS_U16MM) ? SUCRE_OBS_U16MM : SUCRE_OBS_F32;
+    const bool paired = fit_pair_built() && !(flags & (SUCRE_FIT_CLOSED_FORM | SUCRE_FIT_UNPAIRED));
+    flags &= ~SUCRE_FIT_UNPAIRED;
     if ((flags & SUCRE_FIT_CLOSED_FORM) && t0 == 0 && T > 0)
         if (int rc = check_hip(launch_update_J(L, w, fmt, s), "sucre_fit_run/initial update_J")) return rc;
-    for (int it = 0; it < T; ++it) {
+    int it = 0;
+    for (; paired && it + 1 < T; it += 2) {
+        const AdamCoef co0 = adam_coef(t0 + it + 1, lr, beta1, beta2, eps), co1 = adam_coef(t0 + it + 2, lr, beta1, beta2, eps);
+        if (int rc = check_hip(launch_fit_pair_fused(L, w, co0, co1, flags, trace_dev ? trace_dev + (size_t)it * 10 : nullptr,
+                                                     trace_dev ? trace_dev + (size_t)(it + 1) * 10 : nullptr, s), "sucre_fit_run")) return rc;
+    }
+    for (; it < T; ++it) {
         const AdamCoef co = adam_coef(t0 + it + 1, lr, beta1, beta2, eps);
         if (int rc = check_hip(launch_fit_iter_fused(L, w, co, flags, trace_dev ? trace_dev + (size_t)it * 10 : nullptr, s),
                                "sucre_fit_run")) return rc;
diff --git a/sucre_amd/csrc/experiment.h b/sucre_amd/csrc/experiment.h
--- a/sucre_amd/csrc/experiment.h
+++ b/sucre_amd/csrc/experiment.h
@@ -53,6 +53,11 @@
 #endif
 constexpr bool kScaledBBuilt = SUCRE_SCALED_B != 0;
 
+#if !defined(SUCRE_PAIRED_J)
+#define SUCRE_PAIRED_J 1
+#endif
+constexpr bool kPairedBuilt = SUCRE_PAIRED_J != 0;
+
 #ifdef SUCRE_EXP_WAVE_TIMES
 constexpr bool kExpWaveTimes = true;
 #define SUCRE_EXP_EXPORT extern "C" __attribute__((visibility("default")))
diff --git a/sucre_amd/csrc/fit.hip b/sucre_amd/csrc/fit.hip
--- a/sucre_amd/csrc/fit.hip
+++ b/sucre_amd/csrc/fit.hip
@@ -181,14 +181,6 @@
     return static_cast<uint32_t>(reinterpret_cast<uintptr_t>(p));
 }
 
-constexpr uint32_t kShapeFull = 1u << 31;
-constexpr uint32_t kShapeTrail = 1u << 30;
-__host__ __device__ constexpr uint32_t full_chunk_b(int fmt) { return (uint32_t)(chunk_bytes(fmt) - 1024) / 16u; }
-__host__ __device__ __forceinline__ uint32_t item_shape(uint32_t bytes, bool full_chunk) {
-    const uint32_t pieces = bytes / 16u;
-    const uint32_t nA = pieces < 64u ? pieces : 64u, nB = pieces - nA;
-    return (nA - 1u) | ((nB ? nB - 1u : 0u) << 8) | ((nB ? nA : nA - 1u) << 16) | (full_chunk ? kShapeFull : 0u);
-}
 static_assert(level_bytes(0) % 16 == 0 && level_bytes(1) % 16 == 0 && level_bytes(2) % 16 == 0 && level_bytes(3) % 16 == 0 && kChunk % 16 == 0 && kChunk16 % 16 == 0 && kChunk24 % 16 == 0 && kChunk26 % 16 == 0, "items are copied in 16-byte pieces");
 static_assert(kChunk <= 2048 && kChunk >= 1024 && kChunk16 >= 1024 && kChunk24 >= 1024 && kChunk26 >= 1024 && kChunk26 <= kChunk, "a full chunk is one whole DMA + a partial one");
 static_assert(level_bytes(0) % 64 == 0 && level_bytes(1) % 64 == 0 && level_bytes(2) % 64 == 0 && (kGroupLv * level_bytes(3)) % 64 == 0, "items start on 64-byte units (PlanItem.src64; a kStoreZ26 strip starts on a whole chunk)");
@@ -223,14 +215,13 @@
 }
 static_assert(2 * kAhead + 9 <= 63, "s_waitcnt vmcnt takes six bits");
 
-__device__ __forceinline__ uint32_t strip_items(uint32_t levels, int mode) { return 1u + ((levels + 3u) >> 2) + (mode == 0 ? 1u : 0u); }
-
 __global__ __launch_bounds__(256) void plan_kernel(const StripMeta *__restrict__ meta, int n_strips, const uint32_t *__restrict__ store_fmt, uint32_t W0, uint32_t W1,
                                                    uint32_t Kmax, uint32_t stride0, uint32_t stride1, uint32_t kmax0, uint32_t kmax1,
                                                    PlanItem *__restrict__ plan0, PlanItem *__restrict__ plan1,
                                                    StripEntry *__restrict__ strips0, StripEntry *__restrict__ strips1,
                                                    uint32_t *__restrict__ count0, uint32_t *__restrict__ count1, uint64_t comp_off,
-                                                   uint64_t state_off) {
+                                                   uint64_t state_off, uint32_t stride_pair, PlanItem *__restrict__ planL, PlanItem *__restrict__ planF,
+                                                   uint64_t gplane_off) {
     const int mode = blockIdx.y;
     const int fmt = (int)store_fmt[0];
     const uint32_t W = mode ? W1 : W0, stride = mode ? stride1 : stride0, kmax = mode ? kmax1 : kmax0;
@@ -240,31 +231,7 @@
     const uint32_t idx = blockIdx.x * 256u + threadIdx.x;
     const uint32_t wid = idx / Kmax, k = idx - wid * Kmax;
     if (wid >= W) return;
-    const DealShares sh = deal_shares(mode, W / 4u);
-    uint32_t start = 0u, strip = 0u, strip0 = 0u;
-    const uint32_t K = deal_walk(wid, W, (uint32_t)n_strips, sh, [&](uint32_t s) { return meta[s].levels; }, [&](uint32_t kk, uint32_t s) {
-        if (kk == 0u) strip0 = s;
-        if (kk < k) start += strip_items(meta[s].levels, mode);
-        if (kk == k) strip = s;
-    });
-    if (k == 0u) count[wid] = K;
-    if (k >= K) return;
-    const StripMeta m = meta[strip];
-    const uint32_t nfull = m.levels >> 2, r = m.levels & 3u;
-    const uint32_t nu = min(nfull, m.full >> 2);
-    const uint32_t lb = (uint32_t)level_bytes(fmt);
-    const uint64_t st = state_off + (uint64_t)strip * (kStateFloats * 4);
-    PlanItem *out = plan + (size_t)wid * stride + start;
-    strips[(size_t)wid * kmax + k] = StripEntry{strip, strip_counts(nu, nfull - nu, r)};
-    *out++ = PlanItem{(uint32_t)(st >> 6), item_shape(3u * kStripPx * 4u, false)};
-    for (uint32_t g = 0; g < nfull; ++g)
-        *out++ = PlanItem{(uint32_t)((comp_off + (m.lvoff + (uint64_t)g * kGroupLv) * lb) >> 6), item_shape((uint32_t)chunk_bytes(fmt), true)};
-    if (r) *out++ = PlanItem{(uint32_t)((comp_off + (m.lvoff + (uint64_t)nfull * kGroupLv) * lb) >> 6), item_shape(r * lb, false)};
-    if (mode == 0) *out++ = PlanItem{(uint32_t)((st + 3 * kStripPx * 4) >> 6), item_shape(6u * kStripPx * 4u, false)};
-    if (k + 1u == K) {
-        const uint64_t st0 = state_off + (uint64_t)strip0 * (kStateFloats * 4);
-        for (int j = 0; j < kAhead + 1; ++j) *out++ = PlanItem{(uint32_t)(st0 >> 6), item_shape(3u * kStripPx * 4u, false) | kShapeTrail};
-    }
+    plan_thread(mode, fmt, wid, k, W, (uint32_t)n_strips, meta, plan, strips, count, stride, kmax, comp_off, state_off, planL, planF, stride_pair, gplane_off);
 }
 
 typedef uint32_t ItemRegs __attribute__((ext_vector_type(2)));
@@ -384,7 +351,7 @@
     uint32_t cs, behind;
 };
 
-template <int kFmt, int kStores, bool kMoments, bool kPrimed = false, class Chain = NoChain, class OnJ, class OnChunk, class OnTail, class OnEnd>
+template <int kFmt, int kStores, bool kMoments, bool kPrimed = false, class Chain = NoChain, int kStart = 1, class OnJ, class OnChunk, class OnTail, class OnEnd>
 __device__ __forceinline__ void stream_strips(FitLds &lds, const PlanItem *__restrict__ plan, const StripEntry *__restrict__ strip_list,
                                               uint32_t K, const uint8_t *__restrict__ ws, int wave, int lane, uint32_t fullB, OnJ on_J,
                                               OnChunk on_chunk, OnTail on_tail, OnEnd on_end, Chain *chain = nullptr) {
@@ -441,7 +408,14 @@
         const uint32_t strip = se.x, counts = se.y;
         if (k + 1u < K) se = strips[k + 1u];
         const uint32_t nu = counts_unmasked(counts), nm = counts_masked(counts), r = counts_tail(counts);
-        on_J(step());
+        if constexpr (kStart == 3) {
+            static_assert(!kMoments, "the moments are among the start items");
+            on_J(step(), std::integral_constant<int, 0>{});
+            on_J(step(), std::integral_constant<int, 1>{});
+            on_J(step(), std::integral_constant<int, 2>{});
+        } else {
+            on_J(step());
+        }
         for (uint32_t g = 0; g < nu; ++g) on_chunk(step(), false);
         for (uint32_t g = 0; g < nm; ++g) on_chunk(step(), true);
         if (r) on_tail(step(), r);
@@ -656,6 +630,88 @@
     else grad_pass<kFmt, false, kPrimed, Chain>(lds, plan, strips, n_strips_wave, ws, state, wave, lane, w, gscale, co, acc, sBeta, rc, chain);
 }
 
+template <int kFmt, bool kScaledB, int kPair>
+__device__ __forceinline__ void pair_pass(FitLds &lds, const PlanItem *__restrict__ plan, const StripEntry *__restrict__ strips, uint32_t n_strips_wave,
+                                          const uint8_t *__restrict__ ws, float *__restrict__ state, float *__restrict__ gplane, int wave, int lane,
+                                          const Water &w, float gscale, const AdamCoef &co_prev, const AdamCoef &co, Acc &acc, float (&sBeta)[3],
+                                          const RangeCodes &rc) {
+    static_assert(kPair == 1 || kPair == 2, "L or F");
+    float J[3] = {0.f, 0.f, 0.f}, G[3] = {0.f, 0.f, 0.f}, M[3] = {0.f, 0.f, 0.f}, V[3] = {0.f, 0.f, 0.f};
+    auto begin = [&](const uint8_t *sp) {
+        const float *f = reinterpret_cast<const float *>(sp);
+#pragma unroll
+        for (int c = 0; c < 3; ++c) { J[c] = f[c * kStripPx + lane]; acc.pa[c] = 0.f; acc.pb[c] = 0.f; }
+    };
+    auto on_chunk = [&](const uint8_t *sp, bool masked) {
+        float zz[kGroupLv];
+        uint32_t cc[3];
+        read_chunk<kFmt>(sp, lane, zz, cc, rc, masked);
+        if (masked) accumulate_chunk<true, kScaledB>(zz, cc, w, J, acc);
+        else accumulate_chunk<false, kScaledB>(zz, cc, w, J, acc);
+    };
+    auto on_tail = [&](const uint8_t *sp, uint32_t r) {
+        for (uint32_t j = 0; j < r; ++j) {
+            float z;
+            uint32_t k[3];
+            read_level<kFmt>(sp, lane, r, j, z, k, rc);
+            accumulate_level<kScaledB>(z, k, w, J, acc);
+        }
+    };
+    if constexpr (kPair == 1) {
+        stream_strips<kFmt, 3, false>(
+            lds, plan, strips, n_strips_wave, ws, wave, lane, rc.fullB, begin, on_chunk, on_tail,
+            [&](uint32_t strip, const uint8_t *) {
+                float *gp = gplane + (size_t)strip * (3 * kStripPx);
+#pragma unroll
+                for (int c = 0; c < 3; ++c) {
+                    sBeta[c] += (acc.pb[c] == 0.0f) ? 0.0f : J[c] * acc.pb[c];
+                    const float g = gscale * acc.pa[c];
+                    if (kExpNoStore) {
+                        asm volatile("" ::"v"(g));
+                        continue;
+                    }
+                    store_stepped<NoChain>(&gp[c * kStripPx + lane], g);
+                }
+            });
+    } else {
+        stream_strips<kFmt, 9, false, false, NoChain, 3>(
+            lds, plan, strips, n_strips_wave, ws, wave, lane, rc.fullB,
+            [&](const uint8_t *sp, auto which) {
+                const float *f = reinterpret_cast<const float *>(sp);
+                if constexpr (which.value == 0) {
+                    begin(sp);
+                } else if constexpr (which.value == 1) {
+#pragma unroll
+                    for (int c = 0; c < 3; ++c) G[c] = f[c * kStripPx + lane];
+                } else {
+#pragma unroll
+                    for (int c = 0; c < 3; ++c) {
+                        M[c] = f[c * kStripPx + lane];
+                        V[c] = f[(3 + c) * kStripPx + lane];
+                        adam_update_J(J[c], M[c], V[c], G[c], co_prev);
+                    }
+                }
+            },
+            on_chunk, on_tail,
+            [&](uint32_t strip, const uint8_t *) {
+                float *st = state + (size_t)strip * kStateFloats;
+#pragma unroll
+                for (int c = 0; c < 3; ++c) {
+                    float Jc = J[c], m = M[c], v = V[c];
+                    sBeta[c] += (acc.pb[c] == 0.0f) ? 0.0f : Jc * acc.pb[c];
+                    adam_update_J(Jc, m, v, gscale * acc.pa[c], co);
+                    if (kExpNoStore) {
+                        asm volatile("" ::"v"(Jc), "v"(m), "v"(v));
+                        continue;
+                    }
+                    store_stepped<NoChain>(&st[c * kStripPx + lane], Jc);
+                    store_stepped<NoChain>(&st[(3 + c) * kStripPx + lane], m);
+                    store_stepped<NoChain>(&st[(6 + c) * kStripPx + lane], v);
+                }
+            });
+    }
+}
+
 __device__ __forceinline__ void zero_acc(Acc &acc) {
 #pragma unroll
     for (int c = 0; c < 3; ++c) { acc.pa[c] = 0.f; acc.pb[c] = 0.f; acc.sB[c] = 0.f; acc.sGZ[c] = 0.f; }
@@ -670,14 +726,15 @@
 }
 namespace sucre {
 
-template <bool kFused, int kFmt>
+template <bool kFused, int kFmt, int kPair = 0>
 __global__ __launch_bounds__(256, kFitWaves) void fit_grad_kernel(const uint8_t *__restrict__ ws,
                                                        const PlanItem *__restrict__ plan, const StripEntry *__restrict__ plan_strips, const uint32_t *__restrict__ plan_count,
                                                        uint32_t plan_stride, uint32_t plan_kmax,
                                                        float *pstate, const uint64_t *__restrict__ n_obs_total,
                                                        float *__restrict__ state, float *partials, const AdamCoef co,
                                                        unsigned *ticket, double *gpart, int n_groups, double *sums,
-                                                       double *trace_row, const uint32_t *__restrict__ obs_format) {
+                                                       double *trace_row, const uint32_t *__restrict__ obs_format,
+                                                       float *__restrict__ gplane, const AdamCoef co_prev) {
     __shared__ FitLds lds;
     const unsigned long long exp_t_in = kExpWaveTimes ? wall_clock64() : 0ull, exp_c_in = kExpWaveTimes ? clock64() : 0ull;
     const int t = threadIdx.x;
@@ -695,7 +752,12 @@
     if (!fmt_ok) acc.cost = __builtin_nanf("");
     float sBeta[3] = {0.f, 0.f, 0.f};
     if (kExpWaveTimes && lane == 0 && wid < kExpWaveSlots) g_exp_wave_times[0][wid] = wall_clock64();
-    run_grad_pass<kFmt>(pass_scaled_b(w), lds, plan + (size_t)wid * plan_stride, plan_strips + (size_t)wid * plan_kmax, n_mine, ws, state, wave, lane, w, gscale, co, acc, sBeta, rc);
+    if constexpr (kPair == 0) {
+        run_grad_pass<kFmt>(pass_scaled_b(w), lds, plan + (size_t)wid * plan_stride, plan_strips + (size_t)wid * plan_kmax, n_mine, ws, state, wave, lane, w, gscale, co, acc, sBeta, rc);
+    } else {
+        if (pass_scaled_b(w)) pair_pass<kFmt, true, kPair>(lds, plan + (size_t)wid * plan_stride, plan_strips + (size_t)wid * plan_kmax, n_mine, ws, state, gplane, wave, lane, w, gscale, co_prev, co, acc, sBeta, rc);
+        else pair_pass<kFmt, false, kPair>(lds, plan + (size_t)wid * plan_stride, plan_strips + (size_t)wid * plan_kmax, n_mine, ws, state, gplane, wave, lane, w, gscale, co_prev, co, acc, sBeta, rc);
+    }
     if (kExpWaveTimes && lane == 0 && wid < kExpWaveSlots) g_exp_wave_times[1][wid] = wall_clock64();
 
     float s[kNumSums];
@@ -1221,20 +1283,25 @@
     return hipGetLastError();
 }
 
-template <class Kernel>
-static void launch_fit_kernel(Kernel kernel, int mode, const Layout &L, uint8_t *ws, const AdamCoef &co, double *trace_row,
-                              hipStream_t s) {
+template <class Kernel, class... Extra>
+static void launch_fit_kernel_on(Kernel kernel, int mode, size_t plan_off, size_t plan_stride, const Layout &L, uint8_t *ws, const AdamCoef &co, double *trace_row,
+                                 hipStream_t s, Extra... extra) {
     hipLaunchKernelGGL(kernel, dim3(L.fit_blocks[mode]), dim3(256), 0, s, ws,
-                       reinterpret_cast<const PlanItem *>(ws + L.off_plan[mode]),
+                       reinterpret_cast<const PlanItem *>(ws + plan_off),
                        reinterpret_cast<const StripEntry *>(ws + L.off_plan_strips[mode]),
-                       reinterpret_cast<const uint32_t *>(ws + L.off_plan_count[mode]), (uint32_t)L.plan_stride[mode], (uint32_t)L.plan_kmax[mode],
+                       reinterpret_cast<const uint32_t *>(ws + L.off_plan_count[mode]), (uint32_t)plan_stride, (uint32_t)L.plan_kmax[mode],
                        reinterpret_cast<float *>(ws + L.off_params),
                        reinterpret_cast<const uint64_t *>(ws + L.off_n_obs_total),
                        reinterpret_cast<float *>(ws + L.off_state), reinterpret_cast<float *>(ws + L.off_partials), co,
                        reinterpret_cast<unsigned *>(ws + L.off_ticket),
                        reinterpret_cast<double *>(ws + L.off_gpartials), L.fit_groups[mode],
                        reinterpret_cast<double *>(ws + L.off_sums), trace_row,
-                       reinterpret_cast<const uint32_t *>(ws + off_store_format(L)));
+                       reinterpret_cast<const uint32_t *>(ws + off_store_format(L)), extra...);
+}
+template <class Kernel>
+static void launch_fit_kernel(Kernel kernel, int mode, const Layout &L, uint8_t *ws, const AdamCoef &co, double *trace_row,
+                              hipStream_t s) {
+    launch_fit_kernel_on(kernel, mode, L.off_plan[mode], L.plan_stride[mode], L, ws, co, trace_row, s);
 }
 
 template <class F>
@@ -1252,7 +1319,7 @@
                                 hipStream_t s) {
     dispatch_fit(fit_mode(flags), fit_u16(flags), [&](auto mode, auto fmt) {
         if constexpr (mode.value) launch_fit_kernel(fit_closed_kernel<kFused, fmt.value, false>, 1, L, ws, co, trace_row, s);
-        else launch_fit_kernel(fit_grad_kernel<kFused, fmt.value>, 0, L, ws, co, trace_row, s);
+        else launch_fit_kernel_on(fit_grad_kernel<kFused, fmt.value>, 0, L.off_plan[0], L.plan_stride[0], L, ws, co, trace_row, s, (float *)nullptr, co);
     });
 }
 
@@ -1260,6 +1327,21 @@
                                  double *trace_row, hipStream_t s) {
     launch_grad_variant<true>(L, ws, co, flags, trace_row, s);
     return hipGetLastError();
+}
+
+bool fit_pair_built() { return kPairedBuilt; }
+hipError_t launch_fit_pair_fused(const Layout &L, uint8_t *ws, const AdamCoef &co0, const AdamCoef &co1, unsigned flags,
+                                 double *trace_row0, double *trace_row1, hipStream_t s) {
+    if constexpr (kPairedBuilt) {
+        float *gplane = reinterpret_cast<float *>(ws + L.off_gplane);
+        dispatch_fit(0, fit_u16(flags), [&](auto, auto fmt) {
+            launch_fit_kernel_on(fit_grad_kernel<true, fmt.value, 1>, 0, L.off_plan_pair[0], L.plan_stride_pair, L, ws, co0, trace_row0, s, gplane, co0);
+            launch_fit_kernel_on(fit_grad_kernel<true, fmt.value, 2>, 0, L.off_plan_pair[1], L.plan_stride_pair, L, ws, co1, trace_row1, s, gplane, co0);
+        });
+        return hipGetLastError();
+    } else {
+        return hipErrorNotSupported;
+    }
 }
 
 hipError_t launch_fit_grad(const Layout &L, uint8_t *ws, const AdamCoef &co, unsigned flags, hipStream_t s) {
@@ -1298,7 +1380,9 @@
                        reinterpret_cast<PlanItem *>(ws + L.off_plan[0]), reinterpret_cast<PlanItem *>(ws + L.off_plan[1]),
                        reinterpret_cast<StripEntry *>(ws + L.off_plan_strips[0]), reinterpret_cast<StripEntry *>(ws + L.off_plan_strips[1]),
                        reinterpret_cast<uint32_t *>(ws + L.off_plan_count[0]),
-                       reinterpret_cast<uint32_t *>(ws + L.off_plan_count[1]), (uint64_t)L.off_comp, (uint64_t)L.off_state);
+                       reinterpret_cast<uint32_t *>(ws + L.off_plan_count[1]), (uint64_t)L.off_comp, (uint64_t)L.off_state,
+                       (uint32_t)L.plan_stride_pair, reinterpret_cast<PlanItem *>(ws + L.off_plan_pair[0]), reinterpret_cast<PlanItem *>(ws + L.off_plan_pair[1]),
+                       (uint64_t)L.off_gplane);
     return hipGetLastError();
 }
 
diff --git a/sucre_amd/csrc/launch.h b/sucre_amd/csrc/launch.h
--- a/sucre_amd/csrc/launch.h
+++ b/sucre_amd/csrc/launch.h
@@ -47,6 +47,9 @@
                            const float *params0, const float *J0, hipStream_t s);
 hipError_t launch_fit_iter_fused(const Layout &L, uint8_t *ws, const AdamCoef &co, unsigned flags, double *trace_row,
                                  hipStream_t s);
+bool fit_pair_built();
+hipError_t launch_fit_pair_fused(const Layout &L, uint8_t *ws, const AdamCoef &co0, const AdamCoef &co1, unsigned flags,
+                                 double *trace_row0, double *trace_row1, hipStream_t s);
 hipError_t launch_fit_grad(const Layout &L, uint8_t *ws, const AdamCoef &co, unsigned flags, hipStream_t s);
 hipError_t launch_fit_step(const Layout &L, uint8_t *ws, const AdamCoef &co, double *trace_row, hipStream_t s);
 hipError_t launch_update_J(const Layout &L, uint8_t *ws, int fmt, hipStream_t s);
diff --git a/sucre_amd/csrc/layout.h b/sucre_amd/csrc/layout.h
--- a/sucre_amd/csrc/layout.h
+++ b/sucre_amd/csrc/layout.h
@@ -125,6 +125,73 @@
 __host__ __device__ constexpr uint32_t counts_tail(uint32_t c) { return (c >> (2 * kCountBits)) & 7u; }
 static_assert(counts_unmasked(strip_counts(kMaxViews / kGroupLv, 0, 3)) == kMaxViews / kGroupLv && counts_masked(strip_counts(0, kMaxViews / kGroupLv, 3)) == kMaxViews / kGroupLv
               && counts_masked(strip_counts(kMaxViews / kGroupLv, 0, 3)) == 0 && counts_tail(strip_counts(1023, 1, 3)) == 3, "StripEntry.counts round trip at the largest strip");
+
+constexpr uint32_t kShapeFull = 1u << 31;
+constexpr uint32_t kShapeTrail = 1u << 30;
+__host__ __device__ constexpr uint32_t full_chunk_b(int fmt) { return (uint32_t)(chunk_bytes(fmt) - 1024) / 16u; }
+__host__ __device__ inline uint32_t item_shape(uint32_t bytes, bool full_chunk) {
+    const uint32_t pieces = bytes / 16u;
+    const uint32_t nA = pieces < 64u ? pieces : 64u, nB = pieces - nA;
+    return (nA - 1u) | ((nB ? nB - 1u : 0u) << 8) | ((nB ? nA : nA - 1u) << 16) | (full_chunk ? kShapeFull : 0u);
+}
+__host__ __device__ constexpr uint32_t shape_bytes(uint32_t shape, int fmt) {
+    const uint32_t a = (shape & 127u) + 1u, b = ((shape >> 16) & 127u) + ((shape >> 8) & 127u) + 1u;
+    return (shape & kShapeFull) ? (uint32_t)chunk_bytes(fmt) : (a > b ? a : b) * 16u;
+}
+
+constexpr int kStreamJ = 0, kStreamClosed = 1, kStreamL = 2, kStreamF = 3;
+__host__ __device__ constexpr uint32_t stream_strip_items(uint32_t levels, int stream) {
+    return ((levels + 3u) >> 2) + (stream == kStreamJ ? 2u : stream == kStreamF ? 3u : 1u);
+}
+__host__ __device__ inline uint32_t write_strip_items(int stream, const StripMeta &m, uint32_t strip, int fmt, uint64_t comp_off, uint64_t state_off,
+                                                      uint64_t gplane_off, PlanItem *out) {
+    const uint32_t nfull = m.levels >> 2, r = m.levels & 3u;
+    const uint32_t lb = (uint32_t)level_bytes(fmt);
+    const uint64_t st = state_off + (uint64_t)strip * (kStateFloats * 4);
+    const PlanItem moments = PlanItem{(uint32_t)((st + 3 * kStripPx * 4) >> 6), item_shape(6u * kStripPx * 4u, false)};
+    PlanItem *o = out;
+    *o++ = PlanItem{(uint32_t)(st >> 6), item_shape(3u * kStripPx * 4u, false)};
+    if (stream == kStreamF) {
+        *o++ = PlanItem{(uint32_t)((gplane_off + (uint64_t)strip * (3 * kStripPx * 4)) >> 6), item_shape(3u * kStripPx * 4u, false)};
+        *o++ = moments;
+    }
+    for (uint32_t g = 0; g < nfull; ++g)
+        *o++ = PlanItem{(uint32_t)((comp_off + (m.lvoff + (uint64_t)g * kGroupLv) * lb) >> 6), item_shape((uint32_t)chunk_bytes(fmt), true)};
+    if (r) *o++ = PlanItem{(uint32_t)((comp_off + (m.lvoff + (uint64_t)nfull * kGroupLv) * lb) >> 6), item_shape(r * lb, false)};
+    if (stream == kStreamJ) *o++ = moments;
+    return (uint32_t)(o - out);
+}
+__host__ __device__ inline void write_trailing_items(uint32_t strip0, uint64_t state_off, PlanItem *out) {
+    const uint64_t st0 = state_off + (uint64_t)strip0 * (kStateFloats * 4);
+    for (int j = 0; j < SUCRE_RING; ++j) out[j] = PlanItem{(uint32_t)(st0 >> 6), item_shape(3u * kStripPx * 4u, false) | kShapeTrail};
+}
+
+__host__ __device__ inline void plan_thread(int mode, int fmt, uint32_t wid, uint32_t k, uint32_t W, uint32_t n_strips, const StripMeta *meta,
+                                            PlanItem *plan, StripEntry *strips, uint32_t *count, uint32_t stride, uint32_t kmax, uint64_t comp_off,
+                                            uint64_t state_off, PlanItem *planL, PlanItem *planF, uint32_t stride_pair, uint64_t gplane_off) {
+    const DealShares sh = deal_shares(mode, W / 4u);
+    uint32_t start = 0u, strip = 0u, strip0 = 0u;
+    const uint32_t K = deal_walk(wid, W, n_strips, sh, [&](uint32_t s) { return meta[s].levels; }, [&](uint32_t kk, uint32_t s) {
+        if (kk == 0u) strip0 = s;
+        if (kk < k) start += stream_strip_items(meta[s].levels, mode);
+        if (kk == k) strip = s;
+    });
+    if (k == 0u) count[wid] = K;
+    if (k >= K) return;
+    const StripMeta m = meta[strip];
+    const uint32_t nfull = m.levels >> 2, r = m.levels & 3u;
+    const uint32_t nu = nfull < (m.full >> 2) ? nfull : (m.full >> 2);
+    strips[(size_t)wid * kmax + k] = StripEntry{strip, strip_counts(nu, nfull - nu, r)};
+    auto write = [&](int stream, PlanItem *out) {
+        out += write_strip_items(stream, m, strip, fmt, comp_off, state_off, gplane_off, out);
+        if (k + 1u == K) write_trailing_items(strip0, state_off, out);
+    };
+    write(mode, plan + (size_t)wid * stride + start);
+    if (kPairedBuilt && mode == 0) {
+        write(kStreamL, planL + (size_t)wid * stride_pair + (start - k));
+        write(kStreamF, planF + (size_t)wid * stride_pair + (start + k));
+    }
+}
 
 struct Layout {
     int H, W, n_views, tiles_x, tiles_y, n_tiles;
@@ -163,6 +230,9 @@
     size_t off_plan_count[2];
     size_t plan_stride[2];
     size_t plan_kmax[2];
+    size_t off_gplane;
+    size_t off_plan_pair[2];
+    size_t plan_stride_pair;
     size_t total;
 };
 
@@ -225,6 +295,9 @@
             L->off_plan_count[m] = take(waves * sizeof(uint32_t));
         }
     }
+    L->off_gplane = take((size_t)L->n_strips * 3 * kStripPx * sizeof(float));
+    L->plan_stride_pair = L->plan_stride[0] + L->plan_kmax[0];
+    for (int q = 0; q < 2; ++q) L->off_plan_pair[q] = take((size_t)L->fit_blocks[0] * 4 * L->plan_stride_pair * sizeof(PlanItem));
     L->total = o;
     return true;
 }
diff --git a/sucre_amd/engine.py b/sucre_amd/engine.py
--- a/sucre_amd/engine.py
+++ b/sucre_amd/engine.py
@@ -160,6 +160,8 @@
 
 
 PACKED_VIEWS = os.environ.get('SUCRE_PACKED_VIEWS', '1') != '0'
+
+PAIRED_FIT = os.environ.get('SUCRE_PAIRED_FIT', '1') != '0'
 
 MAX_VIEWS = 4096
 
@@ -405,13 +407,15 @@
         self.steps_done = 0
 
     def fit(self, num_iter: int = 200, lr: float = 0.05, use_closed_form: bool = False, betas=(0.9, 0.999),
-            eps: float = 1e-8, record_trace: bool = True, keep_J: bool = False) -> torch.Tensor | None:
+            eps: float = 1e-8, record_trace: bool = True, keep_J: bool = False, paired: bool | None = None) -> torch.Tensor | None:
         ext = self.light or self.float_colour
         width = 20 if ext else 10
         trace = torch.zeros((num_iter, width), dtype=torch.float64, device=self.device) if record_trace else None
         flags = (_lib.FIT_CLOSED_FORM if use_closed_form else 0) | self._fmt_flag | self._ext_flag
         if keep_J and use_closed_form:
             flags |= _lib.FIT_KEEP_J
+        if not ext and not use_closed_form and not (PAIRED_FIT if paired is None else paired):
+            flags |= _lib.FIT_UNPAIRED
         ws, H, W, n = self._geom
         tp = C.c_void_p(trace.data_ptr()) if trace is not None else None
         with torch.cuda.device(self.device):
```

Result: faster. 87.44, median of 6 (+1.4%).
